# anenbergb/Co-DETR-TensorRT

Measured on AMD Instinct MI355X. Metric: images/sec, Co-DINO Swin-L 1920x1280 fp16 (p50 ms/image alongside), higher is better.
Workload: dtype f16

## Files before the change

co-detr-tensorrt_amd/codetr/_cabi.py:

```python
import ctypes
import os

import torch

_HERE = os.path.dirname(os.path.abspath(__file__))
LIB_PATH = os.path.join(_HERE, "libcodetr_hip.so")
ABI_VERSION = 53

_i64, _i32, _vp, _cp = ctypes.c_int64, ctypes.c_int, ctypes.c_void_p, ctypes.c_char_p

_MSDA_ARGS = [_vp, _vp, _vp, _vp, _vp, _vp, _i64, _i64, _i32, _i32, _i32, _i64, _i32, _i64, _vp]
SIGNATURES = {
    "codetr_hip_abi_version": (_i32, []),
    "codetr_hip_strerror": (_cp, [_i32]),
    "codetr_msda_forward_f16": (_i32, _MSDA_ARGS),
    "codetr_msda_forward_bf16": (_i32, _MSDA_ARGS),
    "codetr_msda_forward_f32": (_i32, _MSDA_ARGS),
    "codetr_msda_forward_f64": (_i32, _MSDA_ARGS),
    "codetr_msda_backward_f16": (_i32, [_vp, _vp, _vp, _vp, _vp, _vp, _vp, _i64, _i64, _i32, _i32, _i32, _i64, _i32, _i64,
                                        _vp, _vp, _vp]),
    "codetr_msda_backward_f32": (_i32, [_vp, _vp, _vp, _vp, _vp, _vp, _vp, _i64, _i64, _i32, _i32, _i32, _i64, _i32, _i64,
                                        _vp, _vp, _vp]),
    "codetr_msda_backward_f64": (_i32, [_vp, _vp, _vp, _vp, _vp, _vp, _vp, _i64, _i64, _i32, _i32, _i32, _i64, _i32, _i64,
                                        _vp, _vp, _vp]),
    "codetr_msda_variant": (_cp, [_i32, _i32, _i32, _i32, _i32]),
    "codetr_msda_fused_forward_f16": (_i32, [_vp, _vp, _vp, _vp, _vp, _i64, _vp, _i64, _vp, _i32, _i32, _i64, _i64,
                                             _i32, _i32, _i32, _i64, _i32, _vp]),
    "codetr_msda_fused_forward_bf16": (_i32, [_vp, _vp, _vp, _vp, _vp, _i64, _vp, _i64, _vp, _i32, _i32, _i64, _i64,
                                              _i32, _i32, _i32, _i64, _i32, _vp]),
    "codetr_msda_fused_forward_ref32_f16": (_i32, [_vp, _vp, _vp, _vp, _vp, _i64, _vp, _i64, _vp, _i32, _i32, _i64, _i64,
                                                   _i32, _i32, _i32, _i64, _i32, _vp]),
    "codetr_msda_fused_forward_ref32_bf16": (_i32, [_vp, _vp, _vp, _vp, _vp, _i64, _vp, _i64, _vp, _i32, _i32, _i64, _i64,
                                                    _i32, _i32, _i32, _i64, _i32, _vp]),
    "codetr_msda_encoder_forward_packed_f16": (_i32, [_vp, _vp, _vp, _vp, _i64, _vp, _i64, _i64, _i32, _i32, _i32, _i32,
                                                      _vp, _i32, _i32, _i32, _i32, _vp]),
    "codetr_msda_encoder_forward_packed_bf16": (_i32, [_vp, _vp, _vp, _vp, _i64, _vp, _i64, _i64, _i32, _i32, _i32, _i32,
                                                       _vp, _i32, _i32, _i32, _i32, _vp]),
    "codetr_linear_bf16_f16out": (_i32, [_vp, _vp, _vp, _vp, _vp, _vp, _i64, _i64, _i64, _i64, _i32]),
    "codetr_encoder_projections_f16": (_i32, [_vp, _vp, _vp, _vp, _vp, _vp, _vp, _vp, _i64, _i64, _i64, _i64, _i64, _i32]),
    "codetr_encoder_projections_bf16": (_i32, [_vp, _vp, _vp, _vp, _vp, _vp, _vp, _vp, _i64, _i64, _i64, _i64, _i64, _i32]),
    "codetr_encoder_projections_posgen_f16": (_i32, [_vp, _vp] + [_vp] * 10 + [_vp, _i32, _vp, ctypes.c_float, ctypes.c_float, ctypes.c_float,
                                                              ctypes.c_float, _i32, _vp, _vp, _vp, _vp, _vp, _i64, _i64, _i64, _i64, _i64, _i64, _i32]),
    "codetr_encoder_projections_posgen_bf16": (_i32, [_vp, _vp] + [_vp] * 10 + [_vp, _i32, _vp, ctypes.c_float, ctypes.c_float, ctypes.c_float,
                                                              ctypes.c_float, _i32, _vp, _vp, _vp, _vp, _vp, _i64, _i64, _i64, _i64, _i64, _i64, _i32]),
    "codetr_msda_encoder_packed_lds_bytes": (_i64, [_vp, _i32, _i32, _i32, _vp, _i32, _i32, _i32]),
    "codetr_msda_pack_projection_index": (_i32, [_i32, _i32, _i32, _vp]),
    "codetr_mx_scale_bytes": (_i64, [_i64, _i64]),
    "codetr_linear_fp8mx": (_i32, [_vp, _vp, _vp, _vp, _vp, _vp, _vp, _vp, _vp, _i64, _i64, _i64, _i32]),
    "codetr_cast_fp8mx_f16": (_i32, [_vp, _vp, _vp, _vp, _i64, _i64]),
    "codetr_layernorm_fp8mx_f16": (_i32, [_vp, _vp, _vp, _vp, _vp, _vp, _i64, _i64, ctypes.c_float]),
    "codetr_window_attention_fp8mx_f16": (_i32, [_vp, _vp, _vp, _vp, _vp, _vp, _i64, _i64, _i64, _i32, _i32, _i32, _i32]),
    "codetr_mha_attention_f16": (_i32, [_vp, _vp, _vp, _vp, _vp, _i64, _i64, _i64, _i32, _i32, _i64, _i64, _i64, _i64]),
    "codetr_mha_attention_bf16": (_i32, [_vp, _vp, _vp, _vp, _vp, _i64, _i64, _i64, _i32, _i32, _i64, _i64, _i64, _i64]),
    "codetr_linear_ln_f16": (_i32, [_vp, _vp, _vp, _vp, ctypes.c_float, _vp, _vp, _vp, _i64, _i64, _i64, _i32]),
    "codetr_linear_ln_bf16": (_i32, [_vp, _vp, _vp, _vp, ctypes.c_float, _vp, _vp, _vp, _i64, _i64, _i64, _i32]),
    "codetr_linear_xadd_f16": (_i32, [_vp, _vp, _vp, _vp, _vp, _vp, _i64, _i64, _i64]),
    "codetr_linear_xadd_bf16": (_i32, [_vp, _vp, _vp, _vp, _vp, _vp, _i64, _i64, _i64]),
    "codetr_im2col_tokens_b16": (_i32, [_vp, _vp, _i64, _i64, _i64, _i64, _i32, _i32, _i32, _vp]),
    "codetr_conv_tokens_f16": (_i32, [_vp, _vp, _vp, _vp, _vp, _vp, _i64, _i64, _i64, _i64, _i64, _i32, _i32, _i32, _i32]),
    "codetr_conv_tokens_bf16": (_i32, [_vp, _vp, _vp, _vp, _vp, _vp, _i64, _i64, _i64, _i64, _i64, _i32, _i32, _i32, _i32]),
# ... 11 lines not shown
    "codetr_sigmoid_f16": (_i32, [_vp, _vp, _vp, _i64]),
    "codetr_sigmoid_bf16": (_i32, [_vp, _vp, _vp, _i64]),
    "codetr_gather_rows_b16": (_i32, [_vp, _vp, _vp, _vp, _i64, _i64, _i64, _i64]),
    "codetr_decode_boxes_f16": (_i32, [_vp, _vp, _vp, _vp, _vp, _i64, _i64, _i64, _i32, ctypes.c_float, ctypes.c_float]),
    "codetr_decode_boxes_bf16": (_i32, [_vp, _vp, _vp, _vp, _vp, _i64, _i64, _i64, _i32, ctypes.c_float, ctypes.c_float]),
    "codetr_valid_ratios_f16": (_i32, [_vp, _vp, _vp, _vp, _vp, _i64, _i32]),
    "codetr_valid_ratios_bf16": (_i32, [_vp, _vp, _vp, _vp, _vp, _i64, _i32]),
    "codetr_linear_fp8": (_i32, [_vp, _vp, _vp, _vp, ctypes.c_float, _vp, _vp, _vp, _i32, ctypes.c_float, _i64, _i64, _i64,
                                 _i32]),
    "codetr_cast_fp8_f16": (_i32, [_vp, _vp, _vp, _i64, ctypes.c_float]),
    "codetr_layernorm_fp8_f16": (_i32, [_vp, _vp, _vp, _vp, _vp, _i64, _i64, ctypes.c_float, ctypes.c_float]),
    "codetr_linear_f16": (_i32, [_vp, _vp, _vp, _vp, _vp, _vp, _vp, _i64, _i64, _i64, _i32, _i64, _i32]),
    "codetr_linear_bf16": (_i32, [_vp, _vp, _vp, _vp, _vp, _vp, _vp, _i64, _i64, _i64, _i32, _i64, _i32]),
    "codetr_query_sine_embed_f16": (_i32, [_vp, _vp, _vp, _vp, _i64, _i64, _i32, _i32, _i32, ctypes.c_float, _i32, _vp, _vp,
                                           _vp]),
    "codetr_query_sine_embed_bf16": (_i32, [_vp, _vp, _vp, _vp, _i64, _i64, _i32, _i32, _i32, ctypes.c_float, _i32, _vp, _vp,
                                           _vp]),
    "codetr_encoder_geometry_f16": (_i32, [_vp, _vp, _vp, _i64, _i32, _vp, _vp, _vp, _vp, _vp]),
    "codetr_encoder_geometry_bf16": (_i32, [_vp, _vp, _vp, _i64, _i32, _vp, _vp, _vp, _vp, _vp]),
    "codetr_row_max_f16": (_i32, [_vp, _vp, _vp, _i64, _i64]),
    "codetr_row_max_bf16": (_i32, [_vp, _vp, _vp, _i64, _i64]),
    "codetr_preprocess_u8_f16": (_i32, [_vp, _vp, _i64, _i64, _i64, _i64, _i64, _i64, _vp, _vp, _vp, _vp, _vp]),
    "codetr_preprocess_u8_f32": (_i32, [_vp, _vp, _i64, _i64, _i64, _i64, _i64, _i64, _vp, _vp, _vp, _vp, _vp]),
    "codetr_batched_nms_f32": (_i32, [_vp, _vp, _vp, _i64, ctypes.c_float, _vp]),
    "codetr_preprocess_batch_u8_f16": (_i32, [_vp, _vp, _i64, _i64, _vp, _i64, _i64, _vp, _vp, _vp, ctypes.c_float, _vp, _vp]),
    "codetr_preprocess_batch_u8_bf16": (_i32, [_vp, _vp, _i64, _i64, _vp, _i64, _i64, _vp, _vp, _vp, ctypes.c_float, _vp, _vp]),
    "codetr_preprocess_batch_u8_f32": (_i32, [_vp, _vp, _i64, _i64, _vp, _i64, _i64, _vp, _vp, _vp, ctypes.c_float, _vp, _vp]),
    "codetr_postprocess_detections_f16": (_i32, [_vp, _vp, _vp, _vp, _vp, _i64, _i64, _i32, ctypes.c_float, _i32,
                                                 ctypes.c_float, _vp, _vp, _vp, _vp]),
    "codetr_postprocess_detections_bf16": (_i32, [_vp, _vp, _vp, _vp, _vp, _i64, _i64, _i32, ctypes.c_float, _i32,
                                                  ctypes.c_float, _vp, _vp, _vp, _vp]),
    "codetr_postprocess_detections_f32": (_i32, [_vp, _vp, _vp, _vp, _vp, _i64, _i64, _i32, ctypes.c_float, _i32,
                                                 ctypes.c_float, _vp, _vp, _vp, _vp]),
    "codetr_patch_merge_layernorm_f16": (_i32, [_vp, _vp, _vp, _vp, _vp, _i64, _i64, _i64, _i64, ctypes.c_float]),
    "codetr_patch_merge_layernorm_bf16": (_i32, [_vp, _vp, _vp, _vp, _vp, _i64, _i64, _i64, _i64, ctypes.c_float]),
    "codetr_mask_pyramid": (_i32, [_vp, _vp, _i64, _i64, _i64, _i32, _vp, _vp, _vp, _vp, _vp, _i32]),
    "codetr_linear_splitk_plan": (_i32, [_i64, _i64, _i64, _vp]),
    "codetr_linear_splitk_f16": (_i32, [_vp, _vp, _vp, _vp, _vp, _vp, _vp, _i64, _i64, _i64, _i32, _i32, _vp, _i64]),
    "codetr_linear_splitk_bf16": (_i32, [_vp, _vp, _vp, _vp, _vp, _vp, _vp, _i64, _i64, _i64, _i32, _i32, _vp, _i64]),
    "codetr_linear_sk_workspace_bytes": (_i64, []),
    "codetr_linear_sk_supported": (_i32, [_i64, _i64, _i64]),
    "codetr_linear_sk_preferred": (_i32, [_i64, _i64, _i64, _i32, _i32]),
    "codetr_linear_sk_f16": (_i32, [_vp, _vp, _vp, _vp, _vp, _vp, _i64, _i64, _i64, _i32, _vp, _i64, _i32]),
    "codetr_msda_op4_supported": (_i32, [_i32, _i64, _i64, _i32, _i32, _i32, _i64, _i32]),
    "codetr_msda_op4_forward_f16": (_i32, [_vp, _vp, _vp, _vp, _vp, _vp, _i64, _i64, _i32, _i32, _i32, _i64, _i32, _vp]),
    "codetr_msda_op4_forward_bf16": (_i32, [_vp, _vp, _vp, _vp, _vp, _vp, _i64, _i64, _i32, _i32, _i32, _i64, _i32, _vp]),
    "codetr_swin_mlp_supported": (_i32, [_i64, _i64, _i64]),
    "codetr_swin_mlp_f16": (_i32, [_vp, _vp, _vp, _vp, ctypes.c_float, _vp, _vp, _vp, _vp, _vp, _i64, _i64]),
    "codetr_swin_mlp_bf16": (_i32, [_vp, _vp, _vp, _vp, ctypes.c_float, _vp, _vp, _vp, _vp, _vp, _i64, _i64]),
    "codetr_linear_pp_supported": (_i32, [_i64, _i64, _i64]),
    "codetr_linear_pp_preferred": (_i32, [_i64, _i64, _i64, _i32, _i32]),
    "codetr_linear_pp_f16": (_i32, [_vp, _vp, _vp, _vp, _vp, _vp, _i64, _i64, _i64, _i32, _i32]),
    "codetr_linear_pp_bf16": (_i32, [_vp, _vp, _vp, _vp, _vp, _vp, _i64, _i64, _i64, _i32, _i32]),
    "codetr_linear_sk_bf16": (_i32, [_vp, _vp, _vp, _vp, _vp, _vp, _i64, _i64, _i64, _i32, _vp, _i64, _i32]),
    "codetr_decoder_layer_supported": (_i32, [_i32] * 7),
    "codetr_decoder_layer_blob_halfs": (_i64, [_i32] * 4),
    "codetr_decoder_layer_f16": (_i32, [_vp] * 18 + [_i64, _i64, _i64, _i32, _i32, _i32, ctypes.c_float, ctypes.c_float]),
    "codetr_decoder_layer_bf16": (_i32, [_vp] * 18 + [_i64, _i64, _i64, _i32, _i32, _i32, ctypes.c_float, ctypes.c_float]),
    "codetr_layernorm_f16": (_i32, [_vp, _vp, _vp, _vp, _vp, _i64, _i64, ctypes.c_float]),
    "codetr_layernorm_bf16": (_i32, [_vp, _vp, _vp, _vp, _vp, _i64, _i64, ctypes.c_float]),
    "codetr_groupnorm_tokens_workspace_bytes": (_i64, [_i64, _i64, _i64]),
    "codetr_groupnorm_tokens_f16": (_i32, [_vp, _vp, _vp, _vp, _vp, _i64, _vp, _i64, _i64, _i64, _i32,
                                           ctypes.c_float]),
    "codetr_groupnorm_tokens_bf16": (_i32, [_vp, _vp, _vp, _vp, _vp, _i64, _vp, _i64, _i64, _i64, _i32,
                                           ctypes.c_float]),
    "codetr_sine_pos_tokens_f16": (_i32, [_vp, _vp, _vp, _vp, _vp, _i64, _i64, _i64, _i64, _i32, ctypes.c_float,
                                          ctypes.c_float, ctypes.c_float, ctypes.c_float, _i32]),
    "codetr_sine_pos_tokens_bf16": (_i32, [_vp, _vp, _vp, _vp, _vp, _i64, _i64, _i64, _i64, _i32, ctypes.c_float,
                                          ctypes.c_float, ctypes.c_float, ctypes.c_float, _i32]),
    "codetr_ffn_relu_f16": (_i32, [_vp, _vp, _vp, _vp, _vp, _vp, _vp, _i64, _i64, _i64]),
    "codetr_ffn_relu_ln_f16": (_i32, [_vp, _vp, _vp, _vp, _vp, _vp, _vp, _i64, _i64, _i64, _vp, _vp, ctypes.c_float,
                                      _vp, _vp]),
    "codetr_ffn_relu_ln2_f16": (_i32, [_vp, _vp, _vp, _vp, _vp, _vp, _vp, _i64, _i64, _i64, _vp, _vp, ctypes.c_float,
                                       _vp, _vp, ctypes.c_float, _vp, _vp]),
    "codetr_ffn_relu_ln2_bf16": (_i32, [_vp, _vp, _vp, _vp, _vp, _vp, _vp, _i64, _i64, _i64, _vp, _vp, ctypes.c_float,
                                       _vp, _vp, ctypes.c_float, _vp, _vp]),
    "codetr_ffn_pack_w2_f16": (_i32, [_vp, _vp, _vp, _i64, _i64]),
    "codetr_ffn_oproj_relu_ln2_f16": (_i32, [_vp, _vp, _vp, _vp, _vp, _vp, _vp, _vp, _vp, _vp, _i64, _i64, _i64, _vp, _vp,
                                             ctypes.c_float, _vp, _vp, ctypes.c_float, _vp, _vp]),
    "codetr_ffn_oproj_relu_ln2_bf16": (_i32, [_vp, _vp, _vp, _vp, _vp, _vp, _vp, _vp, _vp, _vp, _i64, _i64, _i64, _vp, _vp,
                                              ctypes.c_float, _vp, _vp, ctypes.c_float, _vp, _vp]),
    "codetr_ffn_oproj_w1_index": (_i32, [_i64, _vp]),
    "codetr_ffn_fp8": (_i32, [_vp, _vp, _vp, _vp, _vp, _vp, _vp, _vp, _vp, _i64, _i64, _i64, ctypes.c_float, ctypes.c_float,
                              _vp, _vp, ctypes.c_float, _vp, _vp, ctypes.c_float, _vp, _vp]),
    "codetr_window_attention_f16": (_i32, [_vp, _vp, _vp, _vp, _vp, _i64, _i64, _i64, _i32, _i32, _i32, _i32]),
    "codetr_window_attention_bf16": (_i32, [_vp, _vp, _vp, _vp, _vp, _i64, _i64, _i64, _i32, _i32, _i32, _i32]),
    "codetr_window_attention_ex": (_i32, [_vp, _vp, _vp, _vp, _vp, _vp, ctypes.c_float, _i64, _i64, _i64, _i32, _i32, _i32, _i32,
                                          _i32, _i32, _i32]),
    "codetr_window_attention_bias_index": (_i32, [_i32, _vp]),
    "codetr_window_attention_fp8out_f16": (_i32, [_vp, _vp, _vp, _vp, _vp, ctypes.c_float, _i64, _i64, _i64, _i32, _i32,
                                                  _i32, _i32]),
}

_lib = None

CALLS = {"encoder_projections_posgen": 0, "msda": 0, "msda_fused": 0, "linear": 0, "layernorm": 0, "window_attention": 0, "groupnorm_tokens": 0,
         "sine_pos_tokens": 0, "ffn_fused": 0, "ffn_oproj_fused": 0, "linear_splitk": 0, "linear_sk": 0, "mask_pyramid": 0,
         "query_sine_embed": 0, "encoder_geometry": 0, "row_max": 0, "preprocess": 0, "batched_nms": 0,
         "preprocess_batch": 0, "postprocess_detections": 0,
         "msda_backward": 0, "patch_merge_layernorm": 0, "msda_encoder": 0, "msda_encoder_packed": 0, "patch_im2col": 0, "mha_attention": 0, "topk": 0,
         "linear_pp": 0, "swin_mlp": 0, "linear_tile128": 0, "linear_tile256": 0, "linear_xs": 0, "linear_ln": 0, "linear_xadd": 0, "encoder_projections": 0,
         "linear_fp8": 0, "cast_fp8": 0, "layernorm_fp8": 0, "small_ops": 0, "ffn_fp8": 0, "decoder_layer": 0,
         "conv_tokens": 0, "conv_im2col_nchw": 0, "maxpool_tokens": 0}


RECORDER = None
_QUERIES = {"codetr_hip_abi_version", "codetr_hip_strerror", "codetr_msda_variant", "codetr_linear_variant",
            "codetr_topk_chunks", "codetr_linear_splitk_plan", "codetr_groupnorm_tokens_workspace_bytes",
            "codetr_linear_sk_workspace_bytes", "codetr_linear_sk_supported", "codetr_linear_sk_preferred",
            "codetr_linear_pp_supported", "codetr_linear_pp_preferred", "codetr_msda_op4_supported", "codetr_swin_mlp_supported",
            "codetr_msda_encoder_packed_lds_bytes", "codetr_msda_pack_projection_index", "codetr_window_attention_bias_index",
            "codetr_mx_scale_bytes", "codetr_decoder_layer_supported",
            "codetr_decoder_layer_blob_halfs"}


class _RecordingLib:
    def __init__(self, lib):
        self._lib = lib

    def __getattr__(self, name):
        fn = getattr(self._lib, name)
        if name in _QUERIES or name not in SIGNATURES:
            return fn

        def launch(*args):
            rc = fn(*args)
            if RECORDER is not None and rc == 0:
                RECORDER.append((name, args))
            return rc

        return launch


_rec_lib = None


def load():
    global _lib, _rec_lib
    if _lib is not None:
        if RECORDER is None:
            return _lib
        if _rec_lib is None:
            _rec_lib = _RecordingLib(_lib)
        return _rec_lib
    if not os.path.isfile(LIB_PATH):
        raise ImportError(
            f"HIP extension not found at {LIB_PATH}; build it with "
            "`python -c 'import __graft_entry__ as g; g.build()'` or `make -C co-detr-tensorrt_amd/csrc`"
        )
    lib = ctypes.CDLL(LIB_PATH)
    for name, (res, args) in SIGNATURES.items():
        try:
            fn = getattr(lib, name)
        except AttributeError as e:
# ... 98 lines not shown
        v = _SK_PREFERRED[key] = bool(load().codetr_linear_sk_preferred(M, N, K, _ACT[act], 1 if has_residual else 0))
    return v


_SK_WORKSPACE = {}


def linear_sk_workspace(device):
    key = (device.index, torch.cuda.current_stream(device).cuda_stream)
    ws = _SK_WORKSPACE.get(key)
    if ws is None:
        with torch.cuda.device(device):
            ws = _SK_WORKSPACE[key] = torch.zeros(load().codetr_linear_sk_workspace_bytes(), dtype=torch.uint8, device=device)
    return ws


def linear_sk(x2d, weight, bias, residual2d, act, out2d, flags=0):
    lib = load()
    CALLS["linear"] += 1
    CALLS["linear_sk"] += 1
    M, K = x2d.shape
    N = weight.shape[0]
    ws = linear_sk_workspace(x2d.device) if flags & 0x40 else None
    fn = lib.codetr_linear_sk_f16 if x2d.dtype == torch.float16 else lib.codetr_linear_sk_bf16
    rc = fn(current_stream_ptr(x2d.device), x2d.data_ptr(), weight.data_ptr(),
            bias.data_ptr() if bias is not None else None,
            residual2d.data_ptr() if residual2d is not None else None, out2d.data_ptr(), M, N, K, _ACT[act],
            ws.data_ptr() if ws is not None else None, ws.numel() if ws is not None else 0, flags)
    check(rc, "codetr_linear_sk")
    return out2d


def swin_mlp(x2d, ln_w, ln_b, eps, w1, b1, w2_packed, b2, out2d):
    CALLS["swin_mlp"] += 1
    lib = load()
    fn = lib.codetr_swin_mlp_bf16 if x2d.dtype == torch.bfloat16 else lib.codetr_swin_mlp_f16
    rc = fn(current_stream_ptr(x2d.device), x2d.data_ptr(), ln_w.data_ptr(), ln_b.data_ptr(), float(eps), w1.data_ptr(),
            b1.data_ptr(), w2_packed.data_ptr(), b2.data_ptr(), out2d.data_ptr(), x2d.shape[0], x2d.shape[1])
    check(rc, "codetr_swin_mlp")
    return out2d


_PP_PREFERRED = {}


def linear_pp_preferred(M, N, K, act=None, has_residual=False) -> bool:
    key = (M, N, K, act, bool(has_residual))
    v = _PP_PREFERRED.get(key)
    if v is None:
        v = _PP_PREFERRED[key] = bool(load().codetr_linear_pp_preferred(M, N, K, _ACT[act], 1 if has_residual else 0))
    return v


def linear_pp(x2d, weight, bias, residual2d, act, out2d, flags=0):
    lib = load()
    CALLS["linear"] += 1
    CALLS["linear_pp"] += 1
    M, K = x2d.shape
    N = weight.shape[0]
    fn = lib.codetr_linear_pp_f16 if x2d.dtype == torch.float16 else lib.codetr_linear_pp_bf16
    rc = fn(current_stream_ptr(x2d.device), x2d.data_ptr(), weight.data_ptr(),
            bias.data_ptr() if bias is not None else None,
            residual2d.data_ptr() if residual2d is not None else None, out2d.data_ptr(), M, N, K, _ACT[act], flags)
    check(rc, "codetr_linear_pp")
    return out2d


def query_sine_embed(ref, valid_ratios, pos_feat, temperature=10000.0, apply_sigmoid=True, valid_ratios32=None):
    CALLS["query_sine_embed"] += 1
    B, Nq, d = ref.shape
    L = valid_ratios.shape[1]
    ref_in = torch.empty((B, Nq, L, d), dtype=ref.dtype, device=ref.device)
    ref_in32 = torch.empty((B, Nq, L, d), dtype=torch.float32, device=ref.device) if valid_ratios32 is not None else None
    embed = torch.empty((B, Nq, d * pos_feat), dtype=ref.dtype, device=ref.device)
    fn = load().codetr_query_sine_embed_bf16 if ref.dtype == torch.bfloat16 else load().codetr_query_sine_embed_f16
    rc = fn(current_stream_ptr(ref.device), ref.data_ptr(), valid_ratios.data_ptr(),
                                            valid_ratios32.data_ptr() if valid_ratios32 is not None else None, B, Nq,
                                            d, L, pos_feat, float(temperature), 1 if apply_sigmoid else 0,
                                            ref_in.data_ptr(), ref_in32.data_ptr() if ref_in32 is not None else None,
                                            embed.data_ptr())
    check(rc, "codetr_query_sine_embed_f16")
    return ref_in, embed, ref_in32


_MSDA_BWD = {torch.float16: "codetr_msda_backward_f16", torch.float32: "codetr_msda_backward_f32",
             torch.float64: "codetr_msda_backward_f64"}


def msda_backward(value, spatial_shapes, level_start_index, sampling_loc, attn_weight, grad_output, grad_value,
                  grad_sampling_loc, grad_attn_weight, im2col_step):
    if value.dtype not in _MSDA_BWD:
        raise RuntimeError(f"multi_scale_deformable_attention_backward: unsupported dtype {value.dtype} (f16 / f32 / f64)")
    CALLS["msda_backward"] += 1
    B, S, M, D = value.shape
    Nq, L, P = sampling_loc.shape[1], sampling_loc.shape[3], sampling_loc.shape[4]
    rc = getattr(load(), _MSDA_BWD[value.dtype])(
        current_stream_ptr(value.device), value.data_ptr(), spatial_shapes.data_ptr(), level_start_index.data_ptr(),
        sampling_loc.data_ptr(), attn_weight.data_ptr(), grad_output.data_ptr(), B, S, M, D, L, Nq, P, int(im2col_step),
        grad_value.data_ptr(), grad_sampling_loc.data_ptr(), grad_attn_weight.data_ptr())
    if rc == -2:
        step = min(B, int(im2col_step))
        raise RuntimeError(f"batch({B}) must divide im2col_step({step})")
    check(rc, "codetr_msda_backward")


def encoder_geometry(valid_ratios, mask_flat, shapes):
    CALLS["encoder_geometry"] += 1
    B, S = mask_flat.shape
    L = len(shapes)
    dev = mask_flat.device
    dt = valid_ratios.dtype
    ref = torch.empty((B, S, 2), dtype=dt, device=dev)
    ref_lvl = torch.empty((B, S, L, 2), dtype=dt, device=dev)
    prop = torch.empty((B, S, 4), dtype=dt, device=dev)
    state = torch.empty((B, S), dtype=torch.uint8, device=dev)
    hw = (ctypes.c_int64 * (2 * L))(*[int(v) for s in shapes for v in s])
    fn = load().codetr_encoder_geometry_bf16 if valid_ratios.dtype == torch.bfloat16 else load().codetr_encoder_geometry_f16
# ... 703 lines not shown
```

co-detr-tensorrt_amd/codetr/_kernel_names.py:

```python
KERNEL_NAMES = (
    "add_kernel",
    "batched_nms_kernel",
    "cast_fp8_kernel",
    "cast_fp8mx_kernel",
    "conv_im2col_nchw_kernel",
    "conv_tokens_kernel",
    "decode_boxes_kernel",
    "decoder_layer_kernel",
    "encoder_geometry_kernel",
    "ffn_fp8_kernel",
    "ffn_fused_kernel",
    "gather_rows_kernel",
    "gn_apply_kernel",
    "gn_finalize_kernel",
    "gn_partial_kernel",
    "im2col_tokens_kernel",
    "layernorm_fp8_kernel",
    "layernorm_fp8mx_kernel",
    "layernorm_kernel",
    "level_cums_kernel",
    "level_mask_kernel",
    "linear_256_fp8_kernel",
    "linear_256_kernel",
    "linear_kernel",
    "linear_pp_kernel",
    "linear_sk_kernel",
    "linear_xs_kernel",
    "maxpool_tokens_kernel",
    "mha_attention_kernel",
    "msda_backward_generic_kernel",
    "msda_backward_kernel",
    "msda_encoder_v4_kernel",
    "msda_fused_headmajor_kernel",
    "msda_op4_kernel",
    "msda_scalar_kernel",
    "msda_tiled_kernel",
    "pack_w2_kernel",
    "patch_im2col_k4_kernel",
    "postprocess_kernel",
    "preprocess_batch_kernel",
    "preprocess_kernel",
    "query_sine_embed_kernel",
    "row_max_kernel",
    "sigmoid_kernel",
    "sine_pos_kernel",
    "splitk_reduce_kernel",
    "swin_mlp_kernel",
    "topk_kernel",
    "topk_reg_kernel",
    "valid_ratios_kernel",
    "window_attention_kernel",
)
```

co-detr-tensorrt_amd/codetr/hip_ops.py:

```python

import collections

import torch
import torch.nn.functional as F

from . import _cabi

NATIVE = {"msda", "linear(f16/bf16, K%64==0)", "layer_norm(f16/bf16)", "swin_window_attention(f16, head_dim 32)",
          "msda_fused(softmax + sampling locations in-kernel)", "groupnorm_tokens(f16, 8 ch/group)",
          "sine_pos_tokens(f16, + level_embed)", "ffn_fused(f16, 256 -> hidden -> 256, ReLU, + identity)",
          "mask_pyramid(level masks + running valid counts + valid ratios)",
          "query_sine_embed(f16: sigmoid x valid ratios + sine embedding of the decoder reference boxes)",
          "encoder_geometry(f16: reference points, proposals, keep/drop state)", "row_max(f16)",
          "preprocess_image(u8 -> f16/f32, cv2-exact resize + pad + normalise + mask)", "batched_nms(f32)",
          "preprocess_batch(u8 -> f16/bf16/f32, <= 32 images of any size per launch, stacked + padded)",
          "postprocess_detections(f16/bf16/f32: threshold + sort + per-class NMS + rescale, one workgroup per image)",
          "patch_merge_layernorm(f16: Swin 2x2 gather + LayerNorm)",
          "msda_encoder_packed(f16/bf16: LDS-staged gather for the encoder's self-attention, csrc/msda_encoder4.hip)",
          "patch_embed(f16/bf16: 4x4 patch gather + GEMM)",
          "mha_attention(f16/bf16: dense softmax attention, head_dim 32, <= 1024 keys)",
          "topk(f16/bf16 rows, k <= 1024: radix select + bitonic sort)",
          "im2col_tokens(16-bit token-major maps)",
          "resnet50(f16/bf16: implicit-GEMM conv_tokens, stem window gather + GEMM, maxpool_tokens, BN folded)",
          "small_ops(f16: add, sigmoid, gather_rows, decode_boxes, valid_ratios)",
          "linear_fp8(e4m3 x e4m3, K%128==0) + layer_norm_fp8 + cast_fp8", "ffn_fp8(fused FFN, both products e4m3)"}


LINEAR_PROFILE = None
KERNEL_PROFILE = None


def _timed(name, meta, launch, device):
    if KERNEL_PROFILE is None:
        return launch()
    st = torch.cuda.current_stream(device)
    e0, e1 = torch.cuda.Event(enable_timing=True), torch.cuda.Event(enable_timing=True)
    e0.record(st)
    r = launch()
    e1.record(st)
    KERNEL_PROFILE.setdefault(name, []).append((e0, e1, meta))
    return r


def _gpu(x, what):
    if not x.is_cuda:
        raise RuntimeError(
            f"codetr.hip_ops.{what}: got a {x.device.type} tensor; this package computes on MI355X only "
            "(the CPU formulation is the oracle in oracle/, not a fallback)"
        )


LINEAR_PP = True


def _persistent_ok(mk, head_major, out, x2, w, r2, bias):
    return (mk is None and not head_major and out.data_ptr() % 16 == 0 and x2.data_ptr() % 16 == 0
            and w.data_ptr() % 16 == 0 and (r2 is None or r2.data_ptr() % 16 == 0)
            and (bias is None or bias.data_ptr() % 16 == 0))


def linear(x, weight, bias=None, act=None, residual=None, row_mask=None, head_major=None):
    _gpu(x, "linear")
    if _cabi.linear_supported(x, weight):
        K = x.shape[-1]
        N = weight.shape[0]
        x2 = x.reshape(-1, K)
        if not x2.is_contiguous():
            x2 = x2.contiguous()
        w = weight if weight.is_contiguous() else weight.contiguous()
        r2 = None
        if residual is not None:
            r2 = residual.reshape(-1, N)
            if not r2.is_contiguous():
                r2 = r2.contiguous()
        mk = None
        if row_mask is not None:
            mk = row_mask.reshape(-1)
            if mk.dtype != torch.bool and mk.dtype != torch.uint8:
                mk = mk != 0
            mk = mk.contiguous()
        hm_rows = hm_hd = 0
        if head_major:
            if x.dim() != 3 or residual is not None:
                raise ValueError("head_major needs a [B, S, K] input and no residual")
            hm_rows, hm_hd = x.shape[1], int(head_major)
        out = torch.empty((x2.shape[0], N), dtype=x.dtype, device=x.device)
        if x2.shape[0] > 0:
            with torch.cuda.device(x.device):
                res_act = act == "relu_res"
                splits, ws_bytes = (1, 0) if (head_major or res_act) else _cabi.linear_splitk_plan(x2.shape[0], N, K)
                if res_act:
                    launch = lambda: _cabi.linear(x2, w, bias, r2, act, out, mk, hm_rows, hm_hd)
                elif splits > 1:
                    ws = torch.empty(ws_bytes, dtype=torch.uint8, device=x.device)
                    launch = lambda: _cabi.linear_splitk(x2, w, bias, r2, act, out, splits, ws, mk)
                elif (LINEAR_PP and _persistent_ok(mk, head_major, out, x2, w, r2, bias)
                      and _cabi.linear_pp_preferred(x2.shape[0], N, K, act, r2 is not None)):
                    launch = lambda: _cabi.linear_pp(x2, w, bias, r2, act, out)
                elif (_persistent_ok(mk, head_major, out, x2, w, r2, bias)
                      and _cabi.linear_sk_preferred(x2.shape[0], N, K, act, r2 is not None)):
                    launch = lambda: _cabi.linear_sk(x2, w, bias, r2, act, out)
                else:
                    launch = lambda: _cabi.linear(x2, w, bias, r2, act, out, mk, hm_rows, hm_hd)
                if LINEAR_PROFILE is None:
                    launch()
                else:
                    st = torch.cuda.current_stream(x.device)
                    e0, e1 = torch.cuda.Event(enable_timing=True), torch.cuda.Event(enable_timing=True)
                    e0.record(st)
                    launch()
                    e1.record(st)
                    LINEAR_PROFILE.append((e0, e1, 2.0 * x2.shape[0] * N * K, x2.shape[0], N, K))
        if head_major:
            return out.view(x.shape[0], N // hm_hd, hm_rows, hm_hd)
        return out.view(*x.shape[:-1], N)
    if head_major:
        raise RuntimeError("head_major output exists only on the native linear (f16/bf16, K % 64 == 0)")
    y = F.linear(x, weight, bias)
    if act == "relu_res":
        if row_mask is not None:
            y = y.masked_fill(row_mask[..., None], 0.0)
        return F.relu(y + residual if residual is not None else y)
    if act == "relu":
        y = F.relu(y, inplace=True)
    elif act == "gelu":
        y = F.gelu(y)
    elif act is not None:
        raise ValueError(act)
    if row_mask is not None:
        y = y.masked_fill(row_mask[..., None], 0.0)
    if residual is not None:
        y = y + residual
    return y


LN_GEMM = True


def linear_ln_supported(x, norm_weight, weight):
    return (LN_GEMM and x.is_cuda and norm_weight is not None and norm_weight.dtype == x.dtype and weight.dtype == x.dtype
            and not torch.is_grad_enabled() and norm_weight.shape[0] == x.shape[-1]
            and _cabi.linear_xadd_supported(x.numel() // max(x.shape[-1], 1), weight.shape[0], x.shape[-1], x.dtype))


def linear_ln(x, norm_weight, norm_bias, eps, weight, bias=None, act=None):
    _gpu(x, "linear_ln")
    if linear_ln_supported(x, norm_weight, weight):
        K, N = x.shape[-1], weight.shape[0]
        x2 = x.reshape(-1, K)
        x2 = x2 if x2.is_contiguous() else x2.contiguous()
        w = weight if weight.is_contiguous() else weight.contiguous()
        out = torch.empty((x2.shape[0], N), dtype=x.dtype, device=x.device)
        ok = [False]

        def launch():
            ok[0] = _cabi.linear_ln(x2, norm_weight, norm_bias, eps, w, bias, act, out)

        with torch.cuda.device(x.device):
            if LINEAR_PROFILE is None:
                launch()
            else:
                st = torch.cuda.current_stream(x.device)
                e0, e1 = torch.cuda.Event(enable_timing=True), torch.cuda.Event(enable_timing=True)
                e0.record(st)
                launch()
                e1.record(st)
                if ok[0]:
                    LINEAR_PROFILE.append((e0, e1, 2.0 * x2.shape[0] * N * K, x2.shape[0], N, K))
        if ok[0]:
            return out.view(*x.shape[:-1], N)
    return linear(layer_norm(x, norm_weight, norm_bias, eps), weight, bias, act=act)


XADD = True
XADD_MIN_ROWS = 0


def linear_xadd_supported(x, x_add, weight):
    return (XADD and x.is_cuda and x_add is not None and x_add.shape == x.shape and x_add.dtype == x.dtype
            and weight.dtype == x.dtype and not torch.is_grad_enabled()
            and x.numel() // max(x.shape[-1], 1) >= XADD_MIN_ROWS
            and _cabi.linear_xadd_supported(x.numel() // max(x.shape[-1], 1), weight.shape[0], x.shape[-1], x.dtype))


def linear_xadd(x, x_add, weight, bias=None):
    _gpu(x, "linear_xadd")
    if linear_xadd_supported(x, x_add, weight):
        K, N = x.shape[-1], weight.shape[0]
        x2, a2 = x.reshape(-1, K), x_add.reshape(-1, K)
        x2 = x2 if x2.is_contiguous() else x2.contiguous()
        a2 = a2 if a2.is_contiguous() else a2.contiguous()
        w = weight if weight.is_contiguous() else weight.contiguous()
        out = torch.empty((x2.shape[0], N), dtype=x.dtype, device=x.device)
        ok = [False]

        def launch():
            ok[0] = _cabi.linear_xadd(x2, a2, w, bias, out)

        with torch.cuda.device(x.device):
# ... 480 lines not shown
        return linear(cols, weight_kkc, bias, act=act, residual=r).view(B, Ho, Wo, Cout)
    x4d = x4d if x4d.is_contiguous() else x4d.contiguous()
    if residual is not None and not residual.is_contiguous():
        residual = residual.contiguous()
    out = torch.empty((B, Ho, Wo, Cout), dtype=x4d.dtype, device=x4d.device)
    with torch.cuda.device(x4d.device):
        _timed("conv_tokens", {"M": B * Ho * Wo, "N": Cout, "K": k * k * C},
               lambda: _cabi.conv_tokens(x4d, weight_kkc, bias, residual, k, stride, pad, act, out), x4d.device)
    return out


def stem_conv_tokens(x, weight_pad, bias, k, stride, pad):
    _gpu(x, "stem_conv_tokens")
    B, C, H, W = x.shape
    Cout, kpad = weight_pad.shape
    Ho, Wo = (H + 2 * pad - k) // stride + 1, (W + 2 * pad - k) // stride + 1
    cols = torch.empty((B * Ho * Wo, kpad), dtype=x.dtype, device=x.device)
    with torch.cuda.device(x.device):
        _cabi.conv_im2col_nchw(x if x.is_contiguous() else x.contiguous(), k, stride, pad, kpad, cols)
    return linear(cols, weight_pad, bias, act="relu").view(B, Ho, Wo, Cout)


def maxpool_tokens(x4d):
    _gpu(x4d, "maxpool_tokens")
    B, H, W, C = x4d.shape
    out = torch.empty((B, (H - 1) // 2 + 1, (W - 1) // 2 + 1, C), dtype=x4d.dtype, device=x4d.device)
    with torch.cuda.device(x4d.device):
        _cabi.maxpool_tokens(x4d if x4d.is_contiguous() else x4d.contiguous(), out)
    return out




def topk(x, k, want_values=True):
    _gpu(x, "topk")
    x2 = x.reshape(-1, x.shape[-1])
    if not torch.is_grad_enabled():
        x2 = x2 if x2.is_contiguous() else x2.contiguous()
        if _cabi.topk_supported(x2, k):
            idx = torch.empty((x2.shape[0], k), dtype=torch.int64, device=x.device)
            val = torch.empty((x2.shape[0], k), dtype=x.dtype, device=x.device) if want_values else None
            with torch.cuda.device(x.device):
                _cabi.topk(x2, k, val, idx)
            shape = (*x.shape[:-1], k)
            return (val.view(shape) if val is not None else None), idx.view(shape)
    v, i = torch.topk(x, k, dim=-1)
    return v, i


MSDA_ENCODER = True
MSDA_FP32_REF = True


_SWITCH_DEFAULTS = {"ENC_POSGEN": True, "WINDOW_BIAS_LANE": True, "LINEAR_PP": True, "SWIN_MLP": True, "SWIN_MLP_MIN_ROWS": 32768, "LN_GEMM": True, "XADD": True, "XADD_MIN_ROWS": 0, "MERGE_LN": True, "MSDA_ENCODER": True,
                    "MSDA_FP32_REF": True, "FP8_MIN_TILES": 96,
                    "R50_NATIVE": True, "R50_CONV_IM2COL": False}


def nondefault_switches():
    import sys

    from . import multi_scale_deformable_attention as msda_mod
    from . import transformer as tr_mod

    me = sys.modules[__name__]
    out = [k for k, v in _SWITCH_DEFAULTS.items() if getattr(me, k) != v]
    if msda_mod.HEAD_MAJOR_VALUE:
        out.append("HEAD_MAJOR_VALUE")
    out += [k for k in ("DEC_FUSED", "DEC_VPROJ") if not getattr(tr_mod, k)]
    return sorted(out)


MSDA_V4 = True
MSDA_V4_THREADS = 512
MSDA_V4_REGION = (16, 16)
MSDA_V4_LDS_BUDGET = 64 * 1024
MSDA_V4_MARGIN_CAP = 40.0
MSDA_V4_HEAD_MAJOR = True
ENC_PROJ_FUSED = True
_SWITCH_DEFAULTS.update({"MSDA_V4": True, "MSDA_V4_THREADS": 512, "MSDA_V4_REGION": (16, 16),
                         "MSDA_V4_LDS_BUDGET": 64 * 1024, "MSDA_V4_MARGIN_CAP": 40.0,
                         "MSDA_V4_HEAD_MAJOR": True, "ENC_PROJ_FUSED": True, "FFN_OPROJ": True})


def msda_encoder_packed_supported(dtype, head_dim, num_levels, num_points):
    return (MSDA_V4 and MSDA_ENCODER and dtype in (torch.float16, torch.bfloat16) and head_dim == 32 and num_levels == 5
            and num_points == 4)


def value_projection_f16(x, weight, bias, row_mask, head_dim):
    _gpu(x, "value_projection_f16")
    if not (x.dtype == torch.bfloat16 and weight.dtype == torch.bfloat16 and x.dim() == 3):
        return None
    B, S, K = x.shape
    N = weight.shape[0]
    x2 = x.reshape(-1, K)
    x2 = x2 if x2.is_contiguous() else x2.contiguous()
    w = weight if weight.is_contiguous() else weight.contiguous()
    mk = None
    if row_mask is not None:
        mk = row_mask.reshape(-1)
        if mk.dtype != torch.bool and mk.dtype != torch.uint8:
            mk = mk != 0
        mk = mk.contiguous()
    out = torch.empty((B * S, N), dtype=torch.float16, device=x.device)
    with torch.cuda.device(x.device):
        ok = _cabi.linear_bf16_f16out(x2, w, bias, out, mk, S, int(head_dim))
# ... 366 lines not shown
```

co-detr-tensorrt_amd/codetr/swin.py:

```python
import warnings
from collections import OrderedDict

import torch
import torch.nn as nn
import torch.nn.functional as F

from . import hip_ops
from .transformer_layers import FFN, build_norm


def to_2tuple(x):
    return tuple(x) if isinstance(x, (tuple, list)) else (x, x)


class PatchEmbed(nn.Module):

    def __init__(self, in_channels=3, embed_dims=768, conv_type="Conv2d", kernel_size=16, stride=16, padding="corner",
                 dilation=1, bias=True, norm_cfg=None, input_size=None, init_cfg=None):
        super().__init__()
        if padding != "corner" or dilation != 1:
            raise NotImplementedError("PatchEmbed: only 'corner' padding, dilation 1 (what Swin uses)")
        self.embed_dims = embed_dims
        self.kernel_size, self.stride = to_2tuple(kernel_size), to_2tuple(stride or kernel_size)
        self.projection = nn.Conv2d(in_channels, embed_dims, self.kernel_size, self.stride, bias=bias)
        self.norm = build_norm(norm_cfg, embed_dims) if norm_cfg is not None else None

    def forward(self, x):
        H, W = x.shape[-2:]
        kh, kw = self.kernel_size
        sh, sw = self.stride
        if hip_ops.patch_embed_supported(x, self.projection.weight, self.stride):
            x, hw = hip_ops.patch_embed(x, self.projection.weight, self.projection.bias)
            if self.norm is not None:
                x = hip_ops.layer_norm(x, self.norm.weight, self.norm.bias, self.norm.eps)
            return x, hw
        ph = max((-(-H // sh) - 1) * sh + kh - H, 0)
        pw = max((-(-W // sw) - 1) * sw + kw - W, 0)
        if ph or pw:
            x = F.pad(x, (0, pw, 0, ph))
        x = hip_ops.conv2d(x, self.projection.weight, self.projection.bias, stride=self.stride)
        hw = (x.shape[2], x.shape[3])
        x = x.flatten(2).transpose(1, 2)
        if self.norm is not None:
            x = hip_ops.layer_norm(x, self.norm.weight, self.norm.bias, self.norm.eps)
        return x, hw


class PatchMerging(nn.Module):

    def __init__(self, in_channels, out_channels, kernel_size=2, stride=None, padding="corner", dilation=1, bias=False,
                 norm_cfg=dict(type="LN"), init_cfg=None):
        super().__init__()
        if to_2tuple(kernel_size) != (2, 2) or to_2tuple(stride or kernel_size) != (2, 2) or padding != "corner":
            raise NotImplementedError("PatchMerging: only the 2x2 / stride-2 / corner-padded form Swin uses")
        self.in_channels, self.out_channels = in_channels, out_channels
        self.norm = build_norm(norm_cfg, 4 * in_channels) if norm_cfg is not None else None
        self.reduction = nn.Linear(4 * in_channels, out_channels, bias=bias)

    def forward(self, x, input_size):
        B, L, C = x.shape
        H, W = input_size
        if L != H * W:
            raise AssertionError("input feature has wrong size")
        x = x.view(B, H, W, C)
        if H % 2 or W % 2:
            x = F.pad(x, (0, 0, 0, W % 2, 0, H % 2))
        H2, W2 = (H + 1) // 2, (W + 1) // 2
        if x.is_cuda and not torch.is_grad_enabled():
            nw, nb, rw = self._permuted_params(C)
            if (self.norm is not None and isinstance(self.norm, nn.LayerNorm)
                    and hip_ops.patch_merge_layernorm_supported(x, C)):
                x = hip_ops.patch_merge_layernorm(x.reshape(B, -1, C), (2 * H2, 2 * W2), nw, nb, self.norm.eps)
                return hip_ops.linear(x, rw, self.reduction.bias), (H2, W2)
            x = x.view(B, H2, 2, W2, 2, C).permute(0, 1, 3, 2, 4, 5).reshape(B, H2 * W2, 4 * C)
            if self.norm is not None:
                x = hip_ops.layer_norm(x, nw, nb, self.norm.eps)
            return hip_ops.linear(x, rw, self.reduction.bias), (H2, W2)
        x = x.view(B, H2, 2, W2, 2, C).permute(0, 1, 3, 5, 2, 4).reshape(B, H2 * W2, 4 * C)
        if self.norm is not None:
            x = hip_ops.layer_norm(x, self.norm.weight, self.norm.bias, self.norm.eps)
        return hip_ops.linear(x, self.reduction.weight, self.reduction.bias), (H2, W2)

    def _permuted_params(self, C):
        ps = [self.reduction.weight] + ([self.norm.weight, self.norm.bias] if self.norm is not None else [])

        def build():
            idx = (torch.arange(C, device=ps[0].device)[None, :] * 4 + torch.arange(4, device=ps[0].device)[:, None]).reshape(-1)
            rw = self.reduction.weight.detach()[:, idx].contiguous()
            nw = self.norm.weight.detach()[idx].contiguous() if self.norm is not None else None
            nb = self.norm.bias.detach()[idx].contiguous() if self.norm is not None else None
            return nw, nb, rw

        return hip_ops.derived(ps, "_codetr_perm", build)


class WindowMSA(nn.Module):
    def __init__(self, embed_dims, num_heads, window_size, qkv_bias=True, qk_scale=None, attn_drop_rate=0.0,
                 proj_drop_rate=0.0, init_cfg=None):
        super().__init__()
        self.embed_dims, self.window_size, self.num_heads = embed_dims, to_2tuple(window_size), num_heads
        head_dim = embed_dims // num_heads
        if qk_scale is not None and qk_scale != head_dim ** -0.5:
            raise NotImplementedError("custom qk_scale")
        self.scale = head_dim ** -0.5
        Wh, Ww = self.window_size
        self.relative_position_bias_table = nn.Parameter(torch.zeros((2 * Wh - 1) * (2 * Ww - 1), num_heads))
        coords = torch.stack(torch.meshgrid(torch.arange(Wh), torch.arange(Ww), indexing="ij")).flatten(1)
        rel = coords[:, :, None] - coords[:, None, :]
        index = (rel[0] + Wh - 1) * (2 * Ww - 1) + (rel[1] + Ww - 1)
        self.register_buffer("relative_position_index", index.contiguous())
        self.qkv = nn.Linear(embed_dims, embed_dims * 3, bias=qkv_bias)
        self.proj = nn.Linear(embed_dims, embed_dims)

    def init_weights(self):
        nn.init.trunc_normal_(self.relative_position_bias_table, std=0.02)

    def relative_position_bias(self):
        t = self.relative_position_bias_table
        N = self.window_size[0] * self.window_size[1]
        return hip_ops.derived((t,), "_codetr_rel_bias", lambda: t[self.relative_position_index.view(-1)].view(N, N, -1)
                               .permute(2, 0, 1).contiguous().detach())

    def forward(self, x, mask=None):
        qkv = hip_ops.linear(x, self.qkv.weight, self.qkv.bias)
        o = hip_ops.window_attention(qkv, self.relative_position_bias(), mask, self.num_heads)
        return hip_ops.linear(o, self.proj.weight, self.proj.bias)


_MASK_CACHE = {}


def shifted_window_mask(Hp, Wp, ws, shift, dtype, device):
    key = (Hp, Wp, ws, shift, dtype, str(device))
    m = _MASK_CACHE.get(key)
    if m is None:
        region = torch.zeros(Hp, Wp, dtype=torch.float32)
        cnt = 0
        for hs in (slice(0, -ws), slice(-ws, -shift), slice(-shift, None)):
            for wsl in (slice(0, -ws), slice(-ws, -shift), slice(-shift, None)):
                region[hs, wsl] = cnt
                cnt += 1
        r = region.view(Hp // ws, ws, Wp // ws, ws).permute(0, 2, 1, 3).reshape(-1, ws * ws)
        diff = r[:, None, :] - r[:, :, None]
        m = torch.where(diff != 0, torch.tensor(-100.0), torch.tensor(0.0)).to(device=device, dtype=dtype)
        _MASK_CACHE[key] = m
    return m


class ShiftWindowMSA(nn.Module):
    def __init__(self, embed_dims, num_heads, window_size, shift_size=0, qkv_bias=True, qk_scale=None,
                 attn_drop_rate=0, proj_drop_rate=0, dropout_layer=dict(type="DropPath", drop_prob=0.0), init_cfg=None):
        super().__init__()
        self.window_size, self.shift_size = window_size, shift_size
        if not 0 <= shift_size < window_size:
            raise AssertionError("shift_size must be in [0, window_size)")
        self.w_msa = WindowMSA(embed_dims, num_heads, to_2tuple(window_size), qkv_bias, qk_scale, attn_drop_rate,
                               proj_drop_rate)

    def takes_norm(self, query, hw_shape):
        return hip_ops.swin_window_attention_supported(query, self.w_msa.embed_dims, self.w_msa.num_heads, self.window_size)

    def forward(self, query, hw_shape, identity=None, pre_norm=None):
        B, L, C = query.shape
        H, W = hw_shape
        if L != H * W:
            raise AssertionError("input feature has wrong size")
        ws, sh = self.window_size, self.shift_size
        m = self.w_msa
        if hip_ops.swin_window_attention_supported(query, C, m.num_heads, ws):
            if pre_norm is not None:
                qkv = hip_ops.linear_ln(query, pre_norm[0], pre_norm[1], pre_norm[2], m.qkv.weight, m.qkv.bias)
            else:
                qkv = hip_ops.linear(query, m.qkv.weight, m.qkv.bias)
            o = hip_ops.swin_window_attention(qkv, m.qkv.bias, m.relative_position_bias(), hw_shape, m.num_heads, ws, sh)
            return hip_ops.linear(o, m.proj.weight, m.proj.bias, residual=identity)
        x = query.view(B, H, W, C)
        pad_r, pad_b = (-W) % ws, (-H) % ws
        if pad_r or pad_b:
            x = F.pad(x, (0, 0, 0, pad_r, 0, pad_b))
        Hp, Wp = H + pad_b, W + pad_r
        mask = None
        if sh > 0:
            x = torch.roll(x, shifts=(-sh, -sh), dims=(1, 2))
            mask = shifted_window_mask(Hp, Wp, ws, sh, query.dtype, query.device)
        win = x.view(B, Hp // ws, ws, Wp // ws, ws, C).permute(0, 1, 3, 2, 4, 5).reshape(-1, ws * ws, C)
        win = self.w_msa(win, mask)
        x = win.view(B, Hp // ws, Wp // ws, ws, ws, C).permute(0, 1, 3, 2, 4, 5).reshape(B, Hp, Wp, C)
        if sh > 0:
            x = torch.roll(x, shifts=(sh, sh), dims=(1, 2))
        if pad_r or pad_b:
            x = x[:, :H, :W, :]
        x = x.reshape(B, H * W, C)
        return x if identity is None else x + identity


class SwinBlock(nn.Module):
    def __init__(self, embed_dims, num_heads, feedforward_channels, window_size=7, shift=False, qkv_bias=True,
                 qk_scale=None, drop_rate=0.0, attn_drop_rate=0.0, drop_path_rate=0.0, act_cfg=dict(type="GELU"),
                 norm_cfg=dict(type="LN"), with_cp=False, init_cfg=None):
        super().__init__()
        self.norm1 = build_norm(norm_cfg, embed_dims)
        self.attn = ShiftWindowMSA(embed_dims, num_heads, window_size, window_size // 2 if shift else 0, qkv_bias,
                                   qk_scale, attn_drop_rate, drop_rate)
        self.norm2 = build_norm(norm_cfg, embed_dims)
        self.ffn = FFN(embed_dims=embed_dims, feedforward_channels=feedforward_channels, num_fcs=2, ffn_drop=drop_rate,
                       act_cfg=act_cfg, add_identity=True)

    def forward(self, x, hw_shape):
        n1, n2 = self.norm1, self.norm2
        mode = getattr(self, "fp8_mode", None)
        if mode is not None and x.is_cuda and x.dtype == torch.float16 and self.attn.takes_norm(x, hw_shape):
            rows = x.shape[0] * x.shape[1]
            if mode == "calibrate":
                return self._forward_fp8_calibrate(x, hw_shape)
            if mode == "run" and all(hip_ops.linear_fp8_supported(rows, w) for w in self._fp8_weights()):
                return self._forward_fp8(x, hw_shape)
            if mode == "mx":
                ops = getattr(self, "fp8_ops", None) or ("qkv", "proj", "fc1", "fc2")
                ws = dict(zip(("qkv", "proj", "fc1", "fc2"), self._fp8_weights()))
                if ops and all(hip_ops.linear_fp8_supported(rows, ws[o]) for o in ops):
                    return self._forward_fp8mx(x, hw_shape)
        if (isinstance(n1, nn.LayerNorm) and self.attn.takes_norm(x, hw_shape)
                and hip_ops.linear_ln_supported(x, n1.weight, self.attn.w_msa.qkv.weight)):
            x = self.attn(x, hw_shape, identity=x, pre_norm=(n1.weight, n1.bias, n1.eps))
        else:
            h = hip_ops.layer_norm(x, n1.weight, n1.bias, n1.eps)
            x = self.attn(h, hw_shape, identity=x)
        fc1, fc2 = self.ffn.layers[0][0], self.ffn.layers[1]
        if (isinstance(n2, nn.LayerNorm) and self.ffn.add_identity and fc1.bias is not None and fc2.bias is not None
                and hip_ops.swin_mlp_supported(x, n2.weight, fc1.weight, fc2.weight, self.ffn.act)):
            return hip_ops.swin_mlp(x, n2.weight, n2.bias, n2.eps, fc1.weight, fc1.bias, fc2.weight, fc2.bias)
        if (isinstance(n2, nn.LayerNorm) and self.ffn.add_identity
                and hip_ops.linear_ln_supported(x, n2.weight, fc1.weight)):
            h = hip_ops.linear_ln(x, n2.weight, n2.bias, n2.eps, fc1.weight, fc1.bias, act=self.ffn.act)
            return hip_ops.linear(h, fc2.weight, fc2.bias, residual=x)
        h = hip_ops.layer_norm(x, n2.weight, n2.bias, n2.eps)
        return self.ffn(h, identity=x)


    def _fp8_weights(self):
        m = self.attn.w_msa
        return (m.qkv.weight, m.proj.weight, self.ffn.layers[0][0].weight, self.ffn.layers[1].weight)

    def _forward_fp8_calibrate(self, x, hw_shape):
        n1, n2, m = self.norm1, self.norm2, self.attn.w_msa
        fc1, fc2 = self.ffn.layers[0][0], self.ffn.layers[1]
        amax = self.__dict__.setdefault("_fp8_amax", {})

        def rec(key, t):
            v = t.detach().abs().amax().float()
            amax[key] = v if key not in amax else torch.maximum(amax[key], v)

        h = hip_ops.layer_norm(x, n1.weight, n1.bias, n1.eps)
        rec("ln1", h)
        qkv = hip_ops.linear(h, m.qkv.weight, m.qkv.bias)
        o = hip_ops.swin_window_attention(qkv, m.qkv.bias, m.relative_position_bias(), hw_shape, m.num_heads,
                                          self.attn.window_size, self.attn.shift_size)
        rec("attn", o)
        x = hip_ops.linear(o, m.proj.weight, m.proj.bias, residual=x)
        h = hip_ops.layer_norm(x, n2.weight, n2.bias, n2.eps)
        rec("ln2", h)
        g = hip_ops.linear(h, fc1.weight, fc1.bias, act=self.ffn.act)
        rec("act", g)
        return hip_ops.linear(g, fc2.weight, fc2.bias, residual=x)

    def _forward_fp8(self, x, hw_shape):
        n1, n2, m = self.norm1, self.norm2, self.attn.w_msa
        fc1, fc2 = self.ffn.layers[0][0], self.ffn.layers[1]
        sc = self._fp8_scales
        h8 = hip_ops.layer_norm_fp8(x, n1.weight, n1.bias, n1.eps, sc["ln1"])
        qkv = hip_ops.linear_fp8(h8, sc["ln1"], m.qkv.weight, m.qkv.bias)
        o8 = hip_ops.swin_window_attention(qkv, m.qkv.bias, m.relative_position_bias(), hw_shape, m.num_heads,
                                           self.attn.window_size, self.attn.shift_size, out_scale=sc["attn"])
        x = hip_ops.linear_fp8(o8, sc["attn"], m.proj.weight, m.proj.bias, residual=x)
        h8 = hip_ops.layer_norm_fp8(x, n2.weight, n2.bias, n2.eps, sc["ln2"])
        g8 = hip_ops.linear_fp8(h8, sc["ln2"], fc1.weight, fc1.bias, act=self.ffn.act, out_scale=sc["act"])
        return hip_ops.linear_fp8(g8, sc["act"], fc2.weight, fc2.bias, residual=x)


    def _forward_fp8mx(self, x, hw_shape):
        n1, n2, m = self.norm1, self.norm2, self.attn.w_msa
        fc1, fc2 = self.ffn.layers[0][0], self.ffn.layers[1]
        ops = getattr(self, "fp8_ops", None) or ("qkv", "proj", "fc1", "fc2")
        if "qkv" in ops:
            h8, hs = hip_ops.layer_norm_fp8mx(x, n1.weight, n1.bias, n1.eps)
            qkv = hip_ops.linear_fp8mx(h8, hs, m.qkv.weight, m.qkv.bias)
        elif hip_ops.linear_ln_supported(x, n1.weight, m.qkv.weight):
            qkv = hip_ops.linear_ln(x, n1.weight, n1.bias, n1.eps, m.qkv.weight, m.qkv.bias)
# ... 172 lines not shown
```

co-detr-tensorrt_amd/csrc/gemm_pp.hip:

```cpp
#include <hip/hip_runtime.h>
#include <stdint.h>

#include <type_traits>

#include "codetr_hip.h"
#include "device_prims.h"

namespace {

#ifndef CODETR_PP_ABL
#define CODETR_PP_ABL 0
#endif
constexpr int kAbl = CODETR_PP_ABL;
#ifdef CODETR_PP_STAMPS
__device__ unsigned long long* g_pp_stamps = nullptr;
#define PP_T(i) const unsigned long long pp_t##i = __builtin_readcyclecounter()
#define PP_ACC(k, a, b) pp_acc[k] += pp_t##b - pp_t##a
#define PP_STAMPS_OUT()                                                                    \
  if (lane == 0 && g_pp_stamps) {                                                          \
    pp_acc[7] = __builtin_readcyclecounter() - pp_k0;                                      \
    unsigned long long* o = g_pp_stamps + ((size_t)blockIdx.x * 8 + wave) * 8;             \
    for (int i = 0; i < 8; ++i) o[i] = pp_acc[i];                                          \
  }
#else
#define PP_T(i)
#define PP_ACC(k, a, b)
#define PP_STAMPS_OUT()
#endif
typedef unsigned u32x2v __attribute__((__vector_size__(2 * sizeof(unsigned))));

constexpr int kSlot = 32768;
constexpr int kOpBytes = 16384;
constexpr int kBiasBytes = 32768;

struct PpArgs {
  const unsigned char* X;
  const unsigned char* W;
  const unsigned short* bias;
  const unsigned short* R;
  unsigned short* Y;
  int M, N, K;
  int tiles_n, T, nk;
  int G;
  int rounds;
  int rem;
};

__device__ __forceinline__ int key64(int row) {
  const int q = (row >> 2) & 3;
  return q ^ ((q & 1) << 1);
}

__device__ __forceinline__ void seg_barrier() {
  __builtin_amdgcn_sched_barrier(0);
  __builtin_amdgcn_s_barrier();
  __builtin_amdgcn_sched_barrier(0);
}

__device__ __forceinline__ int item_tile(const PpArgs& a, int w, int idx) {
  const int D = a.rounds * a.G;
  if (w < a.rem) {
    if (idx == 0) return D + w;
    --idx;
  }
  if (idx >= a.rounds) return -1;
  return (w & 7) * (D >> 3) + idx * (a.G >> 3) + (w >> 3);
}

template <class T, int ACT, bool HAS_BIAS, bool HAS_RES, bool BIAS_LDS = true>
__device__ __forceinline__ bool pp_epilogue(f32x4 (&acc)[4][8], const PpArgs& a, int tile, int grp, int wn, int lane,
                                            const unsigned char* bias_lds) {
  const int fa = lane & 15;
  const int tm = tile / a.tiles_n, tn = tile - tm * a.tiles_n;
  const int m0 = tm * 256 + grp * 128, n0 = tn * 256 + wn * 64;
  const int g = lane >> 4, nl = 4 * fa;
  const int mleft = a.M - m0, nleft = a.N - n0;
  const unsigned rowb = (unsigned)a.N * 2u;
  const unsigned span = (mleft > 0 && nleft > 0) ? (unsigned)(mleft < 128 ? mleft : 128) * rowb : 0u;
  const unsigned voff = nl < nleft ? (unsigned)(4 * g) * rowb + (unsigned)nl * 2u : 0x80000000u;
  const int mrem = mleft - 4 * g;
  const __amdgpu_buffer_rsrc_t rres = __builtin_amdgcn_make_buffer_rsrc(
      const_cast<unsigned char*>(reinterpret_cast<const unsigned char*>(a.R)) + ((size_t)m0 * a.N + n0) * 2, 0,
      HAS_RES ? span : 0u, 0x00020000);
  uint2 rr[8][4];
  auto load_res = [&](int j0, int j1) {
#pragma unroll
    for (int j = j0; j < j1; ++j)
#pragma unroll
      for (int r = 0; r < 4; ++r) {
        const u32x2v t2 = __builtin_amdgcn_raw_buffer_load_b64(rres, j * 16 + r < mrem ? voff : 0x80000000u,
                                                                 (unsigned)(j * 16 + r) * rowb, 0);
        rr[j][r] = uint2{t2[0], t2[1]};
      }
  };
  const bool stored = a.M > m0 && a.N > n0;
  if (stored) {
    float bias4[4] = {0.f, 0.f, 0.f, 0.f};
    if (HAS_BIAS) {
      const int nb = n0 + nl < a.N ? n0 + nl : 0;
      const uint2 b2 = BIAS_LDS ? *reinterpret_cast<const uint2*>(bias_lds + nb * 2)
                                : *reinterpret_cast<const uint2*>(a.bias + nb);
      bias4[0] = T::to_f32((unsigned short)(b2.x & 0xffffu));
      bias4[1] = T::to_f32((unsigned short)(b2.x >> 16));
      bias4[2] = T::to_f32((unsigned short)(b2.y & 0xffffu));
      bias4[3] = T::to_f32((unsigned short)(b2.y >> 16));
    }
    const __amdgpu_buffer_rsrc_t ry = __builtin_amdgcn_make_buffer_rsrc(
        reinterpret_cast<unsigned char*>(a.Y) + ((size_t)m0 * a.N + n0) * 2, 0, span, 0x00020000);
    if (HAS_RES) load_res(0, 4);
#pragma unroll
    for (int j = 0; j < 8; ++j) {
      if (HAS_RES && j == 2) load_res(4, 8);
#pragma unroll
      for (int r = 0; r < 4; ++r) {
        float x[4];
#pragma unroll
        for (int i = 0; i < 4; ++i) x[i] = acc[i][j][r] + bias4[i];
        if (ACT == 1) {
#pragma unroll
          for (int i = 0; i < 4; ++i) x[i] = x[i] < 0.f ? 0.f : x[i];
        }
        if (ACT == 2) {
          const f32x2 g01 = gelu_erf2(f32x2{x[0], x[1]}), g23 = gelu_erf2(f32x2{x[2], x[3]});
          x[0] = g01.x; x[1] = g01.y; x[2] = g23.x; x[3] = g23.y;
        }
        uint2 o = {T::pack2(x[0], x[1]), T::pack2(x[2], x[3])};
        if (HAS_RES) {
          const uint2 q = rr[j][r];
          const float y0 = T::to_f32((unsigned short)(o.x & 0xffffu)) + T::to_f32((unsigned short)(q.x & 0xffffu));
          const float y1 = T::to_f32((unsigned short)(o.x >> 16)) + T::to_f32((unsigned short)(q.x >> 16));
          const float y2 = T::to_f32((unsigned short)(o.y & 0xffffu)) + T::to_f32((unsigned short)(q.y & 0xffffu));
          const float y3 = T::to_f32((unsigned short)(o.y >> 16)) + T::to_f32((unsigned short)(q.y >> 16));
          o = uint2{T::pack2(y0, y1), T::pack2(y2, y3)};
        }
        if (!(kAbl & 16))
          __builtin_amdgcn_raw_buffer_store_b64(u32x2v{o.x, o.y}, ry, j * 16 + r < mrem ? voff : 0x80000000u,
                                                (unsigned)(j * 16 + r) * rowb, 0);
      }
    }
  }
  return stored;
}

template <class T, int ACT, bool HAS_BIAS, bool HAS_RES, int NS, int PH>
__global__ __launch_bounds__(512) __attribute__((amdgpu_waves_per_eu(2, 2))) void linear_pp_kernel(const PpArgs a) {
  __shared__ __attribute__((aligned(16))) unsigned char lds[NS * kSlot + (HAS_BIAS ? kBiasBytes : 0)];
  using frag = typename T::frag;
  constexpr int PP = 4;
  constexpr int VMN = PP * (NS - 2);

  const int tid = threadIdx.x, lane = tid & 63;
  const int wave = __builtin_amdgcn_readfirstlane(tid >> 6);
  const int grp = wave >> 2, wn = wave & 3;
  const int wg = blockIdx.x;
  const int K = a.K, K2 = K * 2;
  const int nh = 2 * a.nk;
  const unsigned lds0 = (unsigned)(uintptr_t)((__attribute__((address_space(3))) unsigned char*)lds);

#ifdef CODETR_PP_STAMPS
  unsigned long long pp_acc[8] = {0, 0, 0, 0, 0, 0, 0, 0};
  const unsigned long long pp_k0 = __builtin_readcyclecounter();
#endif
  int c_idx = 0;
  int c_tile = item_tile(a, wg, 0);
  if (c_tile < 0) return;

  unsigned voffW[2], voffX[2];
  const unsigned char* Wp = a.W;
  const unsigned char* Xp = a.X;
  int p_idx = 0, p_tile = c_tile, p_h = 0;
  auto prod_set_tile = [&]() {
    const int tm = p_tile / a.tiles_n, tn = p_tile - tm * a.tiles_n;
    const int m0 = tm * 256, n0 = tn * 256;
    const int nmax = a.N - 1 - n0, mmax = a.M - 1 - m0;
    int ln = lane;
    asm volatile("" : "+v"(ln));
#pragma unroll
    for (int q = 0; q < 2; ++q) {
      const int r = (wave + 8 * q) * 16 + (ln >> 2);
      const int rw = (r & 192) + 4 * (r & 15) + ((r >> 4) & 3);
      const unsigned co = (unsigned)((((ln & 3) ^ key64(r)) * 16));
      const int rn = rw < nmax ? rw : nmax, rm = r < mmax ? r : mmax;
      voffW[q] = (unsigned)rn * (unsigned)K2 + co;
      voffX[q] = (unsigned)rm * (unsigned)K2 + co;
    }
    Wp = a.W + (size_t)n0 * K * 2;
    Xp = a.X + (size_t)m0 * K * 2;
    p_h = 0;
  };
  prod_set_tile();
  auto produce_piece = [&](int g, int slot) {
    const unsigned dst = lds0 + (unsigned)slot * kSlot + (unsigned)wave * 1024u;
    if (g < 2) lds_dma16(Wp, voffW[g], dst + (unsigned)g * 8192u);
    else lds_dma16(Xp, voffX[g - 2], dst + kOpBytes + (unsigned)(g - 2) * 8192u);
  };
  auto produce_advance = [&]() {
    if (p_tile < 0) return;
    ++p_h;
    if (p_h < nh) {
      Wp += 64;
      Xp += 64;
      return;
    }
    p_tile = item_tile(a, wg, ++p_idx);
    if (p_tile >= 0) prod_set_tile();
  };

  const int fa = lane & 15, fc = lane >> 4;
  const unsigned offA = (unsigned)((wn * 64 + fa) * 64 + ((fc ^ key64(fa)) * 16));
  const unsigned offB = (unsigned)(kOpBytes + (grp * 128 + fa) * 64 + ((fc ^ key64(fa)) * 16));

  f32x4 acc[4][8];
  frag fw[4], fx[8];

  if (HAS_BIAS) {
    for (int i = tid; i * 8 < a.N; i += 512)
      *reinterpret_cast<u32x4*>(lds + NS * kSlot + i * 16) = *reinterpret_cast<const u32x4*>(a.bias + i * 8);
  }
#pragma unroll
  for (int s = 0; s < NS - 1; ++s) {
#pragma unroll
    for (int g = 0; g < PP; ++g) produce_piece(g, s);
    produce_advance();
  }
  wait_vmcnt<VMN>();
  asm volatile("s_waitcnt lgkmcnt(0)" ::: "memory");
  seg_barrier();
  int post = 0;
  int ws = 0;

  auto load_seg = [&](int part) {
    PP_T(0);
    const unsigned char* rbase = lds + ws * kSlot;
    const int fs = ws == 0 ? NS - 1 : ws - 1;
    if (!(kAbl & 4)) {
      if (part == 0) {
#pragma unroll
        for (int i = 0; i < 4; ++i) fw[i] = *reinterpret_cast<const frag*>(rbase + offA + i * 1024);
      }
#pragma unroll
      for (int j = 0; j < 8; ++j)
        if (PH == 1 || (j >> 2) == part) fx[j] = *reinterpret_cast<const frag*>(rbase + offB + j * 1024);
    }
    if (!(kAbl & 1)) {
#pragma unroll
      for (int g = 0; g < PP; ++g)
        if (PH == 1 || (g >> 1) == part) produce_piece(g, fs);
    }
    if (part == PH - 1) produce_advance();
    PP_T(1);
    if (part == PH - 1) {
      if (post > 0) {
        wait_vmcnt<VMN + 32>();
        --post;
      } else {
        wait_vmcnt<VMN>();
      }
    }
    PP_T(2);
    asm volatile("s_waitcnt lgkmcnt(0)" ::: "memory");
    PP_T(3);
    seg_barrier();
    PP_T(4);
    PP_ACC(0, 0, 1); PP_ACC(1, 1, 2); PP_ACC(2, 2, 3); PP_ACC(3, 3, 4);
  };
  auto mfma_seg = [&](int part, bool firstk) {
    PP_T(5);
    __builtin_amdgcn_s_setprio(1);
#pragma unroll
    for (int i = 0; i < 4; ++i)
#pragma unroll
      for (int j = 0; j < 8; ++j) {
        if (PH == 2 && (j >> 2) != part) continue;
        if (kAbl & 2) asm volatile("" ::"v"(fw[i]), "v"(fx[j]));
        else if (firstk) acc[i][j] = T::mfma(fx[j], fw[i], f32x4{0.f, 0.f, 0.f, 0.f});
        else acc[i][j] = T::mfma(fx[j], fw[i], acc[i][j]);
      }
    __builtin_amdgcn_s_setprio(0);
    PP_T(6);
    seg_barrier();
    PP_T(7);
    PP_ACC(4, 5, 6); PP_ACC(5, 6, 7);
  };

  while (c_tile >= 0) {
    if (grp == 1) seg_barrier();
#pragma unroll
    for (int part = 0; part < PH; ++part) {
      load_seg(part);
      mfma_seg(part, true);
    }
    ws = ws + 1 == NS ? 0 : ws + 1;
    for (int h = 1; h < nh; ++h) {
#pragma unroll
      for (int part = 0; part < PH; ++part) {
        load_seg(part);
        mfma_seg(part, false);
      }
      ws = ws + 1 == NS ? 0 : ws + 1;
    }
    if (grp == 0) seg_barrier();

    PP_T(8);
    const bool stored = pp_epilogue<T, ACT, HAS_BIAS, HAS_RES>(acc, a, c_tile, grp, wn, lane, lds + NS * kSlot);
    PP_T(9);
    PP_ACC(6, 8, 9);
    post = stored && !(kAbl & 16) ? NS - 2 : 0;
    c_tile = item_tile(a, wg, ++c_idx);
  }
  wait_vmcnt<0>();
  PP_STAMPS_OUT();
}

int device_cus() {
  static int cus[64] = {0};
  int dev = 0;
  if (hipGetDevice(&dev) != hipSuccess || dev < 0 || dev >= 64) return 256;
  if (cus[dev] == 0) {
    int n = 0;
    if (hipDeviceGetAttribute(&n, hipDeviceAttributeMultiprocessorCount, dev) != hipSuccess || n <= 0) n = 256;
    cus[dev] = n;
  }
  return cus[dev];
}

bool pp_supported(int64_t M, int64_t N, int64_t K) {
  return M > 0 && N > 0 && K >= 128 && K % 64 == 0 && N % 8 == 0 && M <= 0x7fffffffLL && N <= 16384 &&
         255 * K * 2 + 64 < 0x7fffffffLL;
}

template <class T, int ACT>
int launch_pp_act(hipStream_t st, const PpArgs& a, bool has_bias, bool has_res) {
  const dim3 grid((unsigned)a.G), block(512);
#define CODETR_PP(HB, HR) hipLaunchKernelGGL((linear_pp_kernel<T, ACT, HB, HR, 4, 1>), grid, block, 0, st, a)
  if (has_bias && has_res) CODETR_PP(true, true);
  else if (has_bias) CODETR_PP(true, false);
  else if (has_res) CODETR_PP(false, true);
  else CODETR_PP(false, false);
#undef CODETR_PP
  const hipError_t err = hipGetLastError();
  return err == hipSuccess ? 0 : (int)err;
}

template <class T>
int launch_pp(hipStream_t st, const void* X, const void* W, const void* bias, const void* R, void* Y, int64_t M, int64_t N,
              int64_t K, int act, int flags) {
  if (!X || !W || !Y || M <= 0 || N <= 0 || K <= 0) return CODETR_E_BADARG;
  if (act < 0 || act > 2 || !pp_supported(M, N, K)) return CODETR_E_UNSUPPORTED;
  if ((reinterpret_cast<uintptr_t>(X) | reinterpret_cast<uintptr_t>(W) | reinterpret_cast<uintptr_t>(Y) |
       reinterpret_cast<uintptr_t>(R) | reinterpret_cast<uintptr_t>(bias)) & 15)
    return CODETR_E_BADARG;
  const int64_t tiles_m = (M + 255) / 256, tiles_n = (N + 255) / 256, T_ = tiles_m * tiles_n;
  if (T_ > 0x3fffffff) return CODETR_E_TOO_LARGE;
  int G = device_cus() / 8 * 8;
  if (G <= 0) return CODETR_E_BADARG;
  PpArgs a;
  a.X = static_cast<const unsigned char*>(X);
  a.W = static_cast<const unsigned char*>(W);
  a.bias = static_cast<const unsigned short*>(bias);
  a.R = static_cast<const unsigned short*>(R);
  a.Y = static_cast<unsigned short*>(Y);
  a.M = (int)M; a.N = (int)N; a.K = (int)K;
  a.tiles_n = (int)tiles_n; a.T = (int)T_; a.nk = (int)(K / 64);
  a.G = G;
  a.rounds = (int)(T_ / G);
  a.rem = (int)(T_ - (int64_t)a.rounds * G);
  const bool hb = bias != nullptr, hr = R != nullptr;
  if ((int64_t)256 * K * 2 > 0x7fffffffLL) return CODETR_E_TOO_LARGE;
  if (flags != 0) return CODETR_E_UNSUPPORTED;
  switch (act) {
    case 0: return launch_pp_act<T, 0>(st, a, hb, hr);
    case 1: return launch_pp_act<T, 1>(st, a, hb, hr);
    default: return launch_pp_act<T, 2>(st, a, hb, hr);
  }
}

}

extern "C" {

int codetr_linear_pp_supported(int64_t M, int64_t N, int64_t K) { return pp_supported(M, N, K) ? 1 : 0; }

int codetr_linear_pp_preferred(int64_t M, int64_t N, int64_t K, int act, int has_residual) {
  (void)act;
  (void)has_residual;
  if (!pp_supported(M, N, K) || K < 768 || N < 384) return 0;
  const int64_t tn = (N + 255) / 256, tiles = ((M + 255) / 256) * tn;
  return tiles >= 200 && N * 8 >= tn * 256 * 7 ? 1 : 0;
}

int codetr_linear_pp_f16(void* stream, const void* x_dev, const void* w_dev, const void* bias_dev, const void* residual_dev,
                         void* y_dev, int64_t M, int64_t N, int64_t K, int act, int flags) {
  return launch_pp<HalfT>(static_cast<hipStream_t>(stream), x_dev, w_dev, bias_dev, residual_dev, y_dev, M, N, K, act, flags);
}

int codetr_linear_pp_bf16(void* stream, const void* x_dev, const void* w_dev, const void* bias_dev, const void* residual_dev,
                          void* y_dev, int64_t M, int64_t N, int64_t K, int act, int flags) {
#if CODETR_PP_ABL
  return CODETR_E_UNSUPPORTED;
#endif
  return launch_pp<BFloatT>(static_cast<hipStream_t>(stream), x_dev, w_dev, bias_dev, residual_dev, y_dev, M, N, K, act, flags);
}

}
```

co-detr-tensorrt_amd/csrc/layernorm.hip:

```cpp
#include <hip/hip_runtime.h>
#include <stdint.h>

#include "codetr_hip.h"
#include "device_prims.h"

namespace {

constexpr int kThreads = 256;

struct LnHalf {
  __device__ static float up(short b) {
    _Float16 h;
    __builtin_memcpy(&h, &b, 2);
    return (float)h;
  }
  __device__ static short down(float v) {
    _Float16 h = (_Float16)v;
    short b;
    __builtin_memcpy(&b, &h, 2);
    return b;
  }
};
struct LnBf16 {
  __device__ static float up(short b) { return bf16_to_f32((unsigned short)b); }
// ... 37 lines not shown
    int mb = 0, my = 0, mx = 0;
    if (MERGE) {
      mb = (int)(row / ((int64_t)mg.H2 * mg.W2));
      const int rr = (int)(row - (int64_t)mb * mg.H2 * mg.W2);
      my = rr / mg.W2;
      mx = rr - my * mg.W2;
    }
    s16x8 v[NCH];
    float s = 0.f;
#pragma unroll
    for (int c = 0; c < NCH; ++c) {
      const int ch = sub + c * G;
      if (ch < nchunks) {
        if (MERGE) {
          const int cpc = mg.Cs >> 3, k = ch / cpc, within = ch - k * cpc;
          const int sy = 2 * my + (k >> 1), sx = 2 * mx + (k & 1);
          v[c] = s16x8{0, 0, 0, 0, 0, 0, 0, 0};
          if (sy < mg.H && sx < mg.W)
            v[c] = *reinterpret_cast<const s16x8*>(x + (((int64_t)mb * mg.H + sy) * mg.W + sx) * mg.Cs + within * 8);
        } else {
          v[c] = *reinterpret_cast<const s16x8*>(xr + ch * 8);
        }
#pragma unroll
        for (int e = 0; e < 8; ++e) s += T::up(v[c][e]);
      }
    }
    const float mean = group_sum<G>(s) * inv_c;
    float q = 0.f;
#pragma unroll
    for (int c = 0; c < NCH; ++c) {
      const int ch = sub + c * G;
      if (ch < nchunks) {
#pragma unroll
        for (int e = 0; e < 8; ++e) {
          const float d = T::up(v[c][e]) - mean;
          q = fmaf(d, d, q);
        }
      }
    }
    const float rstd = rsqrtf(group_sum<G>(q) * inv_c + eps);
    short* yr = y + row * C;
#pragma unroll
    for (int c = 0; c < NCH; ++c) {
      const int ch = sub + c * G;
      if (ch < nchunks) {
        s16x8 o;
#pragma unroll
        for (int e = 0; e < 8; ++e)
          o[e] = T::down(fmaf((T::up(v[c][e]) - mean) * rstd, T::up(gw[c][e]), T::up(gb[c][e])));
        *reinterpret_cast<s16x8*>(yr + ch * 8) = o;
      }
    }
  }
}

template <class T, int G, int NCH, bool MERGE = false>
int launch_cfg(hipStream_t st, const void* x, const void* g, const void* b, void* y, int64_t rows, int C, float eps,
               MergeGeom mg = MergeGeom{}) {
  constexpr int RPB = kThreads / G;
  int64_t blocks = (rows + RPB - 1) / RPB;
  if (blocks > 256 * 16) blocks = 256 * 16;
  hipLaunchKernelGGL((layernorm_kernel<T, G, NCH, MERGE>), dim3((unsigned)blocks), dim3(kThreads), 0, st,
                     static_cast<const short*>(x), static_cast<const short*>(g), static_cast<const short*>(b),
                     static_cast<short*>(y), rows, C, eps, mg);
  const hipError_t err = hipGetLastError();
  return err == hipSuccess ? 0 : (int)err;
}

template <class T>
int launch_merge(hipStream_t st, const void* x, const void* g, const void* b, void* y, int64_t B, int64_t H, int64_t W,
                 int64_t Cs, float eps) {
  if (!x || !g || !b || !y || B <= 0 || H <= 0 || W <= 0 || Cs <= 0) return CODETR_E_BADARG;
  const int64_t C = 4 * Cs;
  if (Cs % 8 != 0 || C > 4096) return CODETR_E_UNSUPPORTED;
  if (H > 0x7fffffffLL || W > 0x7fffffffLL) return CODETR_E_TOO_LARGE;
  MergeGeom mg{(int)H, (int)W, (int)Cs, (int)((H + 1) / 2), (int)((W + 1) / 2)};
  const int64_t rows = B * mg.H2 * mg.W2;
  const int nch = (int)(C / 8);
  if (nch <= 32) return launch_cfg<T, 32, 1, true>(st, x, g, b, y, rows, (int)C, eps, mg);
  if (nch <= 64) return launch_cfg<T, 64, 1, true>(st, x, g, b, y, rows, (int)C, eps, mg);
  if (nch <= 128) return launch_cfg<T, 64, 2, true>(st, x, g, b, y, rows, (int)C, eps, mg);
  if (nch <= 192) return launch_cfg<T, 64, 3, true>(st, x, g, b, y, rows, (int)C, eps, mg);
  if (nch <= 256) return launch_cfg<T, 64, 4, true>(st, x, g, b, y, rows, (int)C, eps, mg);
  if (nch <= 384) return launch_cfg<T, 64, 6, true>(st, x, g, b, y, rows, (int)C, eps, mg);
  return launch_cfg<T, 64, 8, true>(st, x, g, b, y, rows, (int)C, eps, mg);
}

template <class T>
int launch(hipStream_t st, const void* x, const void* g, const void* b, void* y, int64_t rows, int64_t C, float eps) {
  if (!x || !g || !b || !y || rows <= 0 || C <= 0) return CODETR_E_BADARG;
  if (C % 8 != 0 || C > 4096) return CODETR_E_UNSUPPORTED;
  const int nch = (int)(C / 8);
  if (nch <= 32) return launch_cfg<T, 32, 1>(st, x, g, b, y, rows, (int)C, eps);
  if (nch <= 64) return launch_cfg<T, 64, 1>(st, x, g, b, y, rows, (int)C, eps);
  if (nch <= 128) return launch_cfg<T, 64, 2>(st, x, g, b, y, rows, (int)C, eps);
  if (nch <= 192) return launch_cfg<T, 64, 3>(st, x, g, b, y, rows, (int)C, eps);
  if (nch <= 256) return launch_cfg<T, 64, 4>(st, x, g, b, y, rows, (int)C, eps);
  if (nch <= 384) return launch_cfg<T, 64, 6>(st, x, g, b, y, rows, (int)C, eps);
  return launch_cfg<T, 64, 8>(st, x, g, b, y, rows, (int)C, eps);
}

}

extern "C" {

int codetr_layernorm_f16(void* stream, const void* x_dev, const void* gamma_dev, const void* beta_dev, void* y_dev,
                         int64_t rows, int64_t C, float eps) {
  return launch<LnHalf>(static_cast<hipStream_t>(stream), x_dev, gamma_dev, beta_dev, y_dev, rows, C, eps);
}

int codetr_layernorm_bf16(void* stream, const void* x_dev, const void* gamma_dev, const void* beta_dev, void* y_dev,
                          int64_t rows, int64_t C, float eps) {
  return launch<LnBf16>(static_cast<hipStream_t>(stream), x_dev, gamma_dev, beta_dev, y_dev, rows, C, eps);
}

int codetr_patch_merge_layernorm_f16(void* stream, const void* x_dev, const void* gamma_dev, const void* beta_dev,
                                     void* y_dev, int64_t B, int64_t H, int64_t W, int64_t C, float eps) {
  return launch_merge<LnHalf>(static_cast<hipStream_t>(stream), x_dev, gamma_dev, beta_dev, y_dev, B, H, W, C, eps);
}

int codetr_patch_merge_layernorm_bf16(void* stream, const void* x_dev, const void* gamma_dev, const void* beta_dev,
                                      void* y_dev, int64_t B, int64_t H, int64_t W, int64_t C, float eps) {
  return launch_merge<LnBf16>(static_cast<hipStream_t>(stream), x_dev, gamma_dev, beta_dev, y_dev, B, H, W, C, eps);
}

}
```

include/codetr_hip.h:

```cpp
#ifndef CODETR_HIP_H_
#define CODETR_HIP_H_

#include <stdint.h>

#ifdef __cplusplus
extern "C" {
#endif

#define CODETR_E_BADARG (-1)
#define CODETR_E_IM2COL_STEP (-2)
#define CODETR_E_TOO_LARGE (-3)
#define CODETR_E_UNSUPPORTED (-4)

#define CODETR_HIP_ABI_VERSION 53
int codetr_hip_abi_version(void);
const char *codetr_hip_strerror(int code);

int codetr_msda_forward_f16(void *stream, const void *value_dev, const int64_t *spatial_shapes_dev,
                            const int64_t *level_start_dev, const void *loc_dev, const void *weight_dev,
                            int64_t B, int64_t S, int M, int D, int L, int64_t Nq, int P, int64_t im2col_step,
                            void *out_dev);
int codetr_msda_forward_bf16(void *stream, const void *value_dev, const int64_t *spatial_shapes_dev,
                             const int64_t *level_start_dev, const void *loc_dev, const void *weight_dev,
                             int64_t B, int64_t S, int M, int D, int L, int64_t Nq, int P, int64_t im2col_step,
                             void *out_dev);
int codetr_msda_forward_f32(void *stream, const void *value_dev, const int64_t *spatial_shapes_dev,
                            const int64_t *level_start_dev, const void *loc_dev, const void *weight_dev,
                            int64_t B, int64_t S, int M, int D, int L, int64_t Nq, int P, int64_t im2col_step,
                            void *out_dev);
int codetr_msda_forward_f64(void *stream, const void *value_dev, const int64_t *spatial_shapes_dev,
                            const int64_t *level_start_dev, const void *loc_dev, const void *weight_dev,
                            int64_t B, int64_t S, int M, int D, int L, int64_t Nq, int P, int64_t im2col_step,
                            void *out_dev);

int codetr_msda_op4_supported(int elem_bytes, int64_t B, int64_t S, int M, int D, int L, int64_t Nq, int P);
int codetr_msda_op4_forward_f16(void *stream, const void *value_dev, const int64_t *spatial_shapes_dev,
                                const int64_t *level_start_dev, const void *loc_dev, const void *weight_dev, int64_t B,
                                int64_t S, int M, int D, int L, int64_t Nq, int P, void *out_dev);
int codetr_msda_op4_forward_bf16(void *stream, const void *value_dev, const int64_t *spatial_shapes_dev,
                                 const int64_t *level_start_dev, const void *loc_dev, const void *weight_dev, int64_t B,
                                 int64_t S, int M, int D, int L, int64_t Nq, int P, void *out_dev);

int codetr_msda_fused_forward_f16(void *stream, const void *value_dev, const int64_t *spatial_shapes_dev,
                                  const int64_t *level_start_dev, const void *offsets_dev, int64_t offsets_row_stride,
                                  const void *logits_dev, int64_t logits_row_stride, const void *ref_dev, int ref_dim,
                                  int value_head_major, int64_t B, int64_t S, int M, int D, int L, int64_t Nq, int P,
                                  void *out_dev);
int codetr_msda_fused_forward_bf16(void *stream, const void *value_dev, const int64_t *spatial_shapes_dev,
                                   const int64_t *level_start_dev, const void *offsets_dev, int64_t offsets_row_stride,
                                   const void *logits_dev, int64_t logits_row_stride, const void *ref_dev, int ref_dim,
                                   int value_head_major, int64_t B, int64_t S, int M, int D, int L, int64_t Nq, int P,
                                   void *out_dev);
int codetr_msda_fused_forward_ref32_f16(void *stream, const void *value_dev, const int64_t *spatial_shapes_dev,
                                        const int64_t *level_start_dev, const void *offsets_dev,
                                        int64_t offsets_row_stride, const void *logits_dev, int64_t logits_row_stride,
                                        const void *ref_dev, int ref_dim, int value_head_major, int64_t B, int64_t S,
                                        int M, int D, int L, int64_t Nq, int P, void *out_dev);
int codetr_msda_fused_forward_ref32_bf16(void *stream, const void *value_dev, const int64_t *spatial_shapes_dev,
                                         const int64_t *level_start_dev, const void *offsets_dev,
                                         int64_t offsets_row_stride, const void *logits_dev, int64_t logits_row_stride,
                                         const void *ref_dev, int ref_dim, int value_head_major, int64_t B, int64_t S,
                                         int M, int D, int L, int64_t Nq, int P, void *out_dev);

int codetr_msda_encoder_forward_packed_f16(void *stream, const void *value_dev, const int64_t *level_shapes_host,
                                           const void *packed_dev, int64_t packed_row_stride,
                                           const float *valid_counts_dev, int64_t B, int64_t S, int M, int D, int L, int P,
                                           const int8_t *windows_host, int region_w, int region_h, int threads,
// ... 105 lines not shown
                                      const void *rel_bias_dev, void *out8_dev, void *out_scales_dev, int64_t B, int64_t H,
                                      int64_t W, int num_heads, int head_dim, int window_size, int shift);

int codetr_add_f16(void *stream, const void *a_dev, const void *b_dev, void *out_dev, int64_t n, int64_t a_period);
int codetr_add_bf16(void *stream, const void *a_dev, const void *b_dev, void *out_dev, int64_t n, int64_t a_period);
int codetr_sigmoid_f16(void *stream, const void *x_dev, void *out_dev, int64_t n);
int codetr_sigmoid_bf16(void *stream, const void *x_dev, void *out_dev, int64_t n);
int codetr_gather_rows_b16(void *stream, const void *src_dev, const int64_t *idx_dev, void *out_dev, int64_t B, int64_t S,
                           int64_t K, int64_t C);
int codetr_decode_boxes_f16(void *stream, const void *coords_unact_dev, const int64_t *idx_dev, void *boxes_dev,
                            int64_t *labels_dev, int64_t B, int64_t Nq, int64_t K, int num_classes, float img_w,
                            float img_h);
int codetr_decode_boxes_bf16(void *stream, const void *coords_unact_dev, const int64_t *idx_dev, void *boxes_dev,
                            int64_t *labels_dev, int64_t B, int64_t Nq, int64_t K, int num_classes, float img_w,
                            float img_h);
int codetr_valid_ratios_f16(void *stream, const float *counts_dev, const void *level_wh_f16_dev, void *out_dev,
                            float *out32_dev, int64_t B, int L);
int codetr_valid_ratios_bf16(void *stream, const float *counts_dev, const void *level_wh_bf16_dev, void *out_dev,
                            float *out32_dev, int64_t B, int L);

int codetr_linear_splitk_plan(int64_t M, int64_t N, int64_t K, int64_t *workspace_bytes);
int codetr_linear_splitk_f16(void *stream, const void *x_dev, const void *w_dev, const void *bias_dev,
                             const void *residual_dev, const void *row_mask_dev, void *y_dev, int64_t M, int64_t N,
                             int64_t K, int act, int splits, void *workspace_dev, int64_t workspace_bytes);
int codetr_linear_splitk_bf16(void *stream, const void *x_dev, const void *w_dev, const void *bias_dev,
                              const void *residual_dev, const void *row_mask_dev, void *y_dev, int64_t M, int64_t N,
                              int64_t K, int act, int splits, void *workspace_dev, int64_t workspace_bytes);

int64_t codetr_linear_sk_workspace_bytes(void);
int codetr_linear_sk_supported(int64_t M, int64_t N, int64_t K);
int codetr_linear_sk_preferred(int64_t M, int64_t N, int64_t K, int act, int has_residual);
int codetr_linear_sk_f16(void *stream, const void *x_dev, const void *w_dev, const void *bias_dev,
                         const void *residual_dev, void *y_dev, int64_t M, int64_t N, int64_t K, int act,
                         void *workspace_dev, int64_t workspace_bytes, int flags);
int codetr_linear_sk_bf16(void *stream, const void *x_dev, const void *w_dev, const void *bias_dev,
                          const void *residual_dev, void *y_dev, int64_t M, int64_t N, int64_t K, int act,
                          void *workspace_dev, int64_t workspace_bytes, int flags);

int codetr_swin_mlp_supported(int64_t M, int64_t C, int64_t hidden);
int codetr_swin_mlp_f16(void *stream, const void *x_dev, const void *ln_gamma_dev, const void *ln_beta_dev, float ln_eps,
                        const void *w1_dev, const void *b1_dev, const void *w2_packed_dev, const void *b2_dev, void *y_dev,
                        int64_t M, int64_t C);
int codetr_swin_mlp_bf16(void *stream, const void *x_dev, const void *ln_gamma_dev, const void *ln_beta_dev, float ln_eps,
                         const void *w1_dev, const void *b1_dev, const void *w2_packed_dev, const void *b2_dev, void *y_dev,
                         int64_t M, int64_t C);

int codetr_linear_pp_supported(int64_t M, int64_t N, int64_t K);
int codetr_linear_pp_preferred(int64_t M, int64_t N, int64_t K, int act, int has_residual);
int codetr_linear_pp_f16(void *stream, const void *x_dev, const void *w_dev, const void *bias_dev,
                         const void *residual_dev, void *y_dev, int64_t M, int64_t N, int64_t K, int act, int flags);
int codetr_linear_pp_bf16(void *stream, const void *x_dev, const void *w_dev, const void *bias_dev,
                          const void *residual_dev, void *y_dev, int64_t M, int64_t N, int64_t K, int act, int flags);

int codetr_mask_pyramid(void *stream, const void *img_mask_dev, int64_t B, int64_t H_img, int64_t W_img,
                        int num_levels, const int64_t *level_shapes_host, void *mask_flat_dev, float *ycum_dev,
                        float *xcum_dev, float *valid_counts_dev, int mask_elem_bytes);

int codetr_query_sine_embed_f16(void *stream, const void *ref_dev, const void *valid_ratios_dev,
                                const float *valid_ratios32_dev, int64_t B, int64_t Nq, int ref_dim, int num_levels,
                                int pos_feat, float temperature, int apply_sigmoid, void *ref_in_dev,
                                float *ref_in32_dev, void *embed_dev);
int codetr_query_sine_embed_bf16(void *stream, const void *ref_dev, const void *valid_ratios_dev,
                                const float *valid_ratios32_dev, int64_t B, int64_t Nq, int ref_dim, int num_levels,
                                int pos_feat, float temperature, int apply_sigmoid, void *ref_in_dev,
                                float *ref_in32_dev, void *embed_dev);

int codetr_encoder_geometry_f16(void *stream, const void *valid_ratios_dev, const void *mask_flat_dev, int64_t B,
                                int num_levels, const int64_t *level_shapes_host, void *reference_points_dev,
                                void *reference_by_level_dev, void *proposals_dev, void *row_state_dev);
int codetr_encoder_geometry_bf16(void *stream, const void *valid_ratios_dev, const void *mask_flat_dev, int64_t B,
                                int num_levels, const int64_t *level_shapes_host, void *reference_points_dev,
                                void *reference_by_level_dev, void *proposals_dev, void *row_state_dev);

int codetr_row_max_f16(void *stream, const void *x_dev, void *out_dev, int64_t rows, int64_t C);
int codetr_row_max_bf16(void *stream, const void *x_dev, void *out_dev, int64_t rows, int64_t C);

int codetr_preprocess_u8_f16(void *stream, const void *src_dev, int64_t H_src, int64_t W_src, int64_t H_resized,
                             int64_t W_resized, int64_t H_pad, int64_t W_pad, const float *mean_host,
                             const float *std_host, const int *pad_value_host, void *dst_dev, void *mask_dev);
int codetr_preprocess_u8_f32(void *stream, const void *src_dev, int64_t H_src, int64_t W_src, int64_t H_resized,
                             int64_t W_resized, int64_t H_pad, int64_t W_pad, const float *mean_host,
                             const float *std_host, const int *pad_value_host, void *dst_dev, void *mask_dev);
int codetr_batched_nms_f32(void *stream, const float *boxes_sorted_dev, const int64_t *labels_sorted_dev, int64_t N,
                           float iou_threshold, void *keep_dev);

#define CODETR_PREPROCESS_BATCH_MAX 32
#define CODETR_POSTPROCESS_MAX_Q 1024
int codetr_preprocess_batch_u8_f16(void *stream, const void *src_dev, int64_t src_bytes, int64_t N,
                                   const int64_t *images_host, int64_t H, int64_t W, const float *mean_host,
                                   const float *std_host, const int *pad_value_host, float pad_fill, void *dst_dev,
                                   void *mask_dev);
int codetr_preprocess_batch_u8_bf16(void *stream, const void *src_dev, int64_t src_bytes, int64_t N,
                                    const int64_t *images_host, int64_t H, int64_t W, const float *mean_host,
                                    const float *std_host, const int *pad_value_host, float pad_fill, void *dst_dev,
                                    void *mask_dev);
int codetr_preprocess_batch_u8_f32(void *stream, const void *src_dev, int64_t src_bytes, int64_t N,
                                   const int64_t *images_host, int64_t H, int64_t W, const float *mean_host,
                                   const float *std_host, const int *pad_value_host, float pad_fill, void *dst_dev,
                                   void *mask_dev);
int codetr_postprocess_detections_f16(void *stream, const void *boxes_dev, const void *scores_dev,
                                      const int64_t *labels_dev, const void *divisor_dev, int64_t N, int64_t Q,
                                      int apply_threshold, float score_threshold, int apply_nms, float iou_threshold,
                                      void *boxes_out_dev, void *scores_out_dev, int64_t *labels_out_dev,
                                      int *count_dev);
int codetr_postprocess_detections_bf16(void *stream, const void *boxes_dev, const void *scores_dev,
                                       const int64_t *labels_dev, const void *divisor_dev, int64_t N, int64_t Q,
// ... 136 lines not shown
```

runner/dispatch_gen.inc:

```
static const int kPlanAbi = 53;
static int call_codetr_msda_forward_f16(void* fn, const Arg* a) { typedef int (*F)(const void*, const void*, const void*, const void*, const void*, const void*, long long, long long, int, int, int, long long, int, long long, const void*); return ((F)fn)((const void*)a[0].p, (const void*)a[1].p, (const void*)a[2].p, (const void*)a[3].p, (const void*)a[4].p, (const void*)a[5].p, (long long)a[6].i, (long long)a[7].i, (int)a[8].i, (int)a[9].i, (int)a[10].i, (long long)a[11].i, (int)a[12].i, (long long)a[13].i, (const void*)a[14].p); }
static int call_codetr_msda_forward_bf16(void* fn, const Arg* a) { typedef int (*F)(const void*, const void*, const void*, const void*, const void*, const void*, long long, long long, int, int, int, long long, int, long long, const void*); return ((F)fn)((const void*)a[0].p, (const void*)a[1].p, (const void*)a[2].p, (const void*)a[3].p, (const void*)a[4].p, (const void*)a[5].p, (long long)a[6].i, (long long)a[7].i, (int)a[8].i, (int)a[9].i, (int)a[10].i, (long long)a[11].i, (int)a[12].i, (long long)a[13].i, (const void*)a[14].p); }
static int call_codetr_msda_forward_f32(void* fn, const Arg* a) { typedef int (*F)(const void*, const void*, const void*, const void*, const void*, const void*, long long, long long, int, int, int, long long, int, long long, const void*); return ((F)fn)((const void*)a[0].p, (const void*)a[1].p, (const void*)a[2].p, (const void*)a[3].p, (const void*)a[4].p, (const void*)a[5].p, (long long)a[6].i, (long long)a[7].i, (int)a[8].i, (int)a[9].i, (int)a[10].i, (long long)a[11].i, (int)a[12].i, (long long)a[13].i, (const void*)a[14].p); }
static int call_codetr_msda_forward_f64(void* fn, const Arg* a) { typedef int (*F)(const void*, const void*, const void*, const void*, const void*, const void*, long long, long long, int, int, int, long long, int, long long, const void*); return ((F)fn)((const void*)a[0].p, (const void*)a[1].p, (const void*)a[2].p, (const void*)a[3].p, (const void*)a[4].p, (const void*)a[5].p, (long long)a[6].i, (long long)a[7].i, (int)a[8].i, (int)a[9].i, (int)a[10].i, (long long)a[11].i, (int)a[12].i, (long long)a[13].i, (const void*)a[14].p); }
static int call_codetr_msda_backward_f16(void* fn, const Arg* a) { typedef int (*F)(const void*, const void*, const void*, const void*, const void*, const void*, const void*, long long, long long, int, int, int, long long, int, long long, const void*, const void*, const void*); return ((F)fn)((const void*)a[0].p, (const void*)a[1].p, (const void*)a[2].p, (const void*)a[3].p, (const void*)a[4].p, (const void*)a[5].p, (const void*)a[6].p, (long long)a[7].i, (long long)a[8].i, (int)a[9].i, (int)a[10].i, (int)a[11].i, (long long)a[12].i, (int)a[13].i, (long long)a[14].i, (const void*)a[15].p, (const void*)a[16].p, (const void*)a[17].p); }
static int call_codetr_msda_backward_f32(void* fn, const Arg* a) { typedef int (*F)(const void*, const void*, const void*, const void*, const void*, const void*, const void*, long long, long long, int, int, int, long long, int, long long, const void*, const void*, const void*); return ((F)fn)((const void*)a[0].p, (const void*)a[1].p, (const void*)a[2].p, (const void*)a[3].p, (const void*)a[4].p, (const void*)a[5].p, (const void*)a[6].p, (long long)a[7].i, (long long)a[8].i, (int)a[9].i, (int)a[10].i, (int)a[11].i, (long long)a[12].i, (int)a[13].i, (long long)a[14].i, (const void*)a[15].p, (const void*)a[16].p, (const void*)a[17].p); }
static int call_codetr_msda_backward_f64(void* fn, const Arg* a) { typedef int (*F)(const void*, const void*, const void*, const void*, const void*, const void*, const void*, long long, long long, int, int, int, long long, int, long long, const void*, const void*, const void*); return ((F)fn)((const void*)a[0].p, (const void*)a[1].p, (const void*)a[2].p, (const void*)a[3].p, (const void*)a[4].p, (const void*)a[5].p, (const void*)a[6].p, (long long)a[7].i, (long long)a[8].i, (int)a[9].i, (int)a[10].i, (int)a[11].i, (long long)a[12].i, (int)a[13].i, (long long)a[14].i, (const void*)a[15].p, (const void*)a[16].p, (const void*)a[17].p); }
static int call_codetr_msda_fused_forward_f16(void* fn, const Arg* a) { typedef int (*F)(const void*, const void*, const void*, const void*, const void*, long long, const void*, long long, const void*, int, int, long long, long long, int, int, int, long long, int, const void*); return ((F)fn)((const void*)a[0].p, (const void*)a[1].p, (const void*)a[2].p, (const void*)a[3].p, (const void*)a[4].p, (long long)a[5].i, (const void*)a[6].p, (long long)a[7].i, (const void*)a[8].p, (int)a[9].i, (int)a[10].i, (long long)a[11].i, (long long)a[12].i, (int)a[13].i, (int)a[14].i, (int)a[15].i, (long long)a[16].i, (int)a[17].i, (const void*)a[18].p); }
static int call_codetr_msda_fused_forward_bf16(void* fn, const Arg* a) { typedef int (*F)(const void*, const void*, const void*, const void*, const void*, long long, const void*, long long, const void*, int, int, long long, long long, int, int, int, long long, int, const void*); return ((F)fn)((const void*)a[0].p, (const void*)a[1].p, (const void*)a[2].p, (const void*)a[3].p, (const void*)a[4].p, (long long)a[5].i, (const void*)a[6].p, (long long)a[7].i, (const void*)a[8].p, (int)a[9].i, (int)a[10].i, (long long)a[11].i, (long long)a[12].i, (int)a[13].i, (int)a[14].i, (int)a[15].i, (long long)a[16].i, (int)a[17].i, (const void*)a[18].p); }
static int call_codetr_msda_fused_forward_ref32_f16(void* fn, const Arg* a) { typedef int (*F)(const void*, const void*, const void*, const void*, const void*, long long, const void*, long long, const void*, int, int, long long, long long, int, int, int, long long, int, const void*); return ((F)fn)((const void*)a[0].p, (const void*)a[1].p, (const void*)a[2].p, (const void*)a[3].p, (const void*)a[4].p, (long long)a[5].i, (const void*)a[6].p, (long long)a[7].i, (const void*)a[8].p, (int)a[9].i, (int)a[10].i, (long long)a[11].i, (long long)a[12].i, (int)a[13].i, (int)a[14].i, (int)a[15].i, (long long)a[16].i, (int)a[17].i, (const void*)a[18].p); }
static int call_codetr_msda_fused_forward_ref32_bf16(void* fn, const Arg* a) { typedef int (*F)(const void*, const void*, const void*, const void*, const void*, long long, const void*, long long, const void*, int, int, long long, long long, int, int, int, long long, int, const void*); return ((F)fn)((const void*)a[0].p, (const void*)a[1].p, (const void*)a[2].p, (const void*)a[3].p, (const void*)a[4].p, (long long)a[5].i, (const void*)a[6].p, (long long)a[7].i, (const void*)a[8].p, (int)a[9].i, (int)a[10].i, (long long)a[11].i, (long long)a[12].i, (int)a[13].i, (int)a[14].i, (int)a[15].i, (long long)a[16].i, (int)a[17].i, (const void*)a[18].p); }
static int call_codetr_msda_encoder_forward_packed_f16(void* fn, const Arg* a) { typedef int (*F)(const void*, const void*, const void*, const void*, long long, const void*, long long, long long, int, int, int, int, const void*, int, int, int, int, const void*); return ((F)fn)((const void*)a[0].p, (const void*)a[1].p, (const void*)a[2].p, (const void*)a[3].p, (long long)a[4].i, (const void*)a[5].p, (long long)a[6].i, (long long)a[7].i, (int)a[8].i, (int)a[9].i, (int)a[10].i, (int)a[11].i, (const void*)a[12].p, (int)a[13].i, (int)a[14].i, (int)a[15].i, (int)a[16].i, (const void*)a[17].p); }
static int call_codetr_msda_encoder_forward_packed_bf16(void* fn, const Arg* a) { typedef int (*F)(const void*, const void*, const void*, const void*, long long, const void*, long long, long long, int, int, int, int, const void*, int, int, int, int, const void*); return ((F)fn)((const void*)a[0].p, (const void*)a[1].p, (const void*)a[2].p, (const void*)a[3].p, (long long)a[4].i, (const void*)a[5].p, (long long)a[6].i, (long long)a[7].i, (int)a[8].i, (int)a[9].i, (int)a[10].i, (int)a[11].i, (const void*)a[12].p, (int)a[13].i, (int)a[14].i, (int)a[15].i, (int)a[16].i, (const void*)a[17].p); }
static int call_codetr_linear_bf16_f16out(void* fn, const Arg* a) { typedef int (*F)(const void*, const void*, const void*, const void*, const void*, const void*, long long, long long, long long, long long, int); return ((F)fn)((const void*)a[0].p, (const void*)a[1].p, (const void*)a[2].p, (const void*)a[3].p, (const void*)a[4].p, (const void*)a[5].p, (long long)a[6].i, (long long)a[7].i, (long long)a[8].i, (long long)a[9].i, (int)a[10].i); }
static int call_codetr_encoder_projections_f16(void* fn, const Arg* a) { typedef int (*F)(const void*, const void*, const void*, const void*, const void*, const void*, const void*, const void*, long long, long long, long long, long long, long long, int); return ((F)fn)((const void*)a[0].p, (const void*)a[1].p, (const void*)a[2].p, (const void*)a[3].p, (const void*)a[4].p, (const void*)a[5].p, (const void*)a[6].p, (const void*)a[7].p, (long long)a[8].i, (long long)a[9].i, (long long)a[10].i, (long long)a[11].i, (long long)a[12].i, (int)a[13].i); }
static int call_codetr_encoder_projections_bf16(void* fn, const Arg* a) { typedef int (*F)(const void*, const void*, const void*, const void*, const void*, const void*, const void*, const void*, long long, long long, long long, long long, long long, int); return ((F)fn)((const void*)a[0].p, (const void*)a[1].p, (const void*)a[2].p, (const void*)a[3].p, (const void*)a[4].p, (const void*)a[5].p, (const void*)a[6].p, (const void*)a[7].p, (long long)a[8].i, (long long)a[9].i, (long long)a[10].i, (long long)a[11].i, (long long)a[12].i, (int)a[13].i); }
static int call_codetr_encoder_projections_posgen_f16(void* fn, const Arg* a) { typedef int (*F)(const void*, const void*, const void*, const void*, const void*, const void*, const void*, const void*, const void*, const void*, const void*, const void*, const void*, int, const void*, float, float, float, float, int, const void*, const void*, const void*, const void*, const void*, long long, long long, long long, long long, long long, long long, int); return ((F)fn)((const void*)a[0].p, (const void*)a[1].p, (const void*)a[2].p, (const void*)a[3].p, (const void*)a[4].p, (const void*)a[5].p, (const void*)a[6].p, (const void*)a[7].p, (const void*)a[8].p, (const void*)a[9].p, (const void*)a[10].p, (const void*)a[11].p, (const void*)a[12].p, (int)a[13].i, (const void*)a[14].p, (float)a[15].f, (float)a[16].f, (float)a[17].f, (float)a[18].f, (int)a[19].i, (const void*)a[20].p, (const void*)a[21].p, (const void*)a[22].p, (const void*)a[23].p, (const void*)a[24].p, (long long)a[25].i, (long long)a[26].i, (long long)a[27].i, (long long)a[28].i, (long long)a[29].i, (long long)a[30].i, (int)a[31].i); }
static int call_codetr_encoder_projections_posgen_bf16(void* fn, const Arg* a) { typedef int (*F)(const void*, const void*, const void*, const void*, const void*, const void*, const void*, const void*, const void*, const void*, const void*, const void*, const void*, int, const void*, float, float, float, float, int, const void*, const void*, const void*, const void*, const void*, long long, long long, long long, long long, long long, long long, int); return ((F)fn)((const void*)a[0].p, (const void*)a[1].p, (const void*)a[2].p, (const void*)a[3].p, (const void*)a[4].p, (const void*)a[5].p, (const void*)a[6].p, (const void*)a[7].p, (const void*)a[8].p, (const void*)a[9].p, (const void*)a[10].p, (const void*)a[11].p, (const void*)a[12].p, (int)a[13].i, (const void*)a[14].p, (float)a[15].f, (float)a[16].f, (float)a[17].f, (float)a[18].f, (int)a[19].i, (const void*)a[20].p, (const void*)a[21].p, (const void*)a[22].p, (const void*)a[23].p, (const void*)a[24].p, (long long)a[25].i, (long long)a[26].i, (long long)a[27].i, (long long)a[28].i, (long long)a[29].i, (long long)a[30].i, (int)a[31].i); }
static int call_codetr_linear_fp8mx(void* fn, const Arg* a) { typedef int (*F)(const void*, const void*, const void*, const void*, const void*, const void*, const void*, const void*, const void*, long long, long long, long long, int); return ((F)fn)((const void*)a[0].p, (const void*)a[1].p, (const void*)a[2].p, (const void*)a[3].p, (const void*)a[4].p, (const void*)a[5].p, (const void*)a[6].p, (const void*)a[7].p, (const void*)a[8].p, (long long)a[9].i, (long long)a[10].i, (long long)a[11].i, (int)a[12].i); }
static int call_codetr_cast_fp8mx_f16(void* fn, const Arg* a) { typedef int (*F)(const void*, const void*, const void*, const void*, long long, long long); return ((F)fn)((const void*)a[0].p, (const void*)a[1].p, (const void*)a[2].p, (const void*)a[3].p, (long long)a[4].i, (long long)a[5].i); }
static int call_codetr_layernorm_fp8mx_f16(void* fn, const Arg* a) { typedef int (*F)(const void*, const void*, const void*, const void*, const void*, const void*, long long, long long, float); return ((F)fn)((const void*)a[0].p, (const void*)a[1].p, (const void*)a[2].p, (const void*)a[3].p, (const void*)a[4].p, (const void*)a[5].p, (long long)a[6].i, (long long)a[7].i, (float)a[8].f); }
static int call_codetr_window_attention_fp8mx_f16(void* fn, const Arg* a) { typedef int (*F)(const void*, const void*, const void*, const void*, const void*, const void*, long long, long long, long long, int, int, int, int); return ((F)fn)((const void*)a[0].p, (const void*)a[1].p, (const void*)a[2].p, (const void*)a[3].p, (const void*)a[4].p, (const void*)a[5].p, (long long)a[6].i, (long long)a[7].i, (long long)a[8].i, (int)a[9].i, (int)a[10].i, (int)a[11].i, (int)a[12].i); }
static int call_codetr_mha_attention_f16(void* fn, const Arg* a) { typedef int (*F)(const void*, const void*, const void*, const void*, const void*, long long, long long, long long, int, int, long long, long long, long long, long long); return ((F)fn)((const void*)a[0].p, (const void*)a[1].p, (const void*)a[2].p, (const void*)a[3].p, (const void*)a[4].p, (long long)a[5].i, (long long)a[6].i, (long long)a[7].i, (int)a[8].i, (int)a[9].i, (long long)a[10].i, (long long)a[11].i, (long long)a[12].i, (long long)a[13].i); }
static int call_codetr_mha_attention_bf16(void* fn, const Arg* a) { typedef int (*F)(const void*, const void*, const void*, const void*, const void*, long long, long long, long long, int, int, long long, long long, long long, long long); return ((F)fn)((const void*)a[0].p, (const void*)a[1].p, (const void*)a[2].p, (const void*)a[3].p, (const void*)a[4].p, (long long)a[5].i, (long long)a[6].i, (long long)a[7].i, (int)a[8].i, (int)a[9].i, (long long)a[10].i, (long long)a[11].i, (long long)a[12].i, (long long)a[13].i); }
static int call_codetr_linear_ln_f16(void* fn, const Arg* a) { typedef int (*F)(const void*, const void*, const void*, const void*, float, const void*, const void*, const void*, long long, long long, long long, int); return ((F)fn)((const void*)a[0].p, (const void*)a[1].p, (const void*)a[2].p, (const void*)a[3].p, (float)a[4].f, (const void*)a[5].p, (const void*)a[6].p, (const void*)a[7].p, (long long)a[8].i, (long long)a[9].i, (long long)a[10].i, (int)a[11].i); }
static int call_codetr_linear_ln_bf16(void* fn, const Arg* a) { typedef int (*F)(const void*, const void*, const void*, const void*, float, const void*, const void*, const void*, long long, long long, long long, int); return ((F)fn)((const void*)a[0].p, (const void*)a[1].p, (const void*)a[2].p, (const void*)a[3].p, (float)a[4].f, (const void*)a[5].p, (const void*)a[6].p, (const void*)a[7].p, (long long)a[8].i, (long long)a[9].i, (long long)a[10].i, (int)a[11].i); }
static int call_codetr_linear_xadd_f16(void* fn, const Arg* a) { typedef int (*F)(const void*, const void*, const void*, const void*, const void*, const void*, long long, long long, long long); return ((F)fn)((const void*)a[0].p, (const void*)a[1].p, (const void*)a[2].p, (const void*)a[3].p, (const void*)a[4].p, (const void*)a[5].p, (long long)a[6].i, (long long)a[7].i, (long long)a[8].i); }
static int call_codetr_linear_xadd_bf16(void* fn, const Arg* a) { typedef int (*F)(const void*, const void*, const void*, const void*, const void*, const void*, long long, long long, long long); return ((F)fn)((const void*)a[0].p, (const void*)a[1].p, (const void*)a[2].p, (const void*)a[3].p, (const void*)a[4].p, (const void*)a[5].p, (long long)a[6].i, (long long)a[7].i, (long long)a[8].i); }
static int call_codetr_im2col_tokens_b16(void* fn, const Arg* a) { typedef int (*F)(const void*, const void*, long long, long long, long long, long long, int, int, int, const void*); return ((F)fn)((const void*)a[0].p, (const void*)a[1].p, (long long)a[2].i, (long long)a[3].i, (long long)a[4].i, (long long)a[5].i, (int)a[6].i, (int)a[7].i, (int)a[8].i, (const void*)a[9].p); }
static int call_codetr_conv_tokens_f16(void* fn, const Arg* a) { typedef int (*F)(const void*, const void*, const void*, const void*, const void*, const void*, long long, long long, long long, long long, long long, int, int, int, int); return ((F)fn)((const void*)a[0].p, (const void*)a[1].p, (const void*)a[2].p, (const void*)a[3].p, (const void*)a[4].p, (const void*)a[5].p, (long long)a[6].i, (long long)a[7].i, (long long)a[8].i, (long long)a[9].i, (long long)a[10].i, (int)a[11].i, (int)a[12].i, (int)a[13].i, (int)a[14].i); }
static int call_codetr_conv_tokens_bf16(void* fn, const Arg* a) { typedef int (*F)(const void*, const void*, const void*, const void*, const void*, const void*, long long, long long, long long, long long, long long, int, int, int, int); return ((F)fn)((const void*)a[0].p, (const void*)a[1].p, (const void*)a[2].p, (const void*)a[3].p, (const void*)a[4].p, (const void*)a[5].p, (long long)a[6].i, (long long)a[7].i, (long long)a[8].i, (long long)a[9].i, (long long)a[10].i, (int)a[11].i, (int)a[12].i, (int)a[13].i, (int)a[14].i); }
static int call_codetr_conv_im2col_nchw_b16(void* fn, const Arg* a) { typedef int (*F)(const void*, const void*, long long, int, long long, long long, int, int, int, int, const void*); return ((F)fn)((const void*)a[0].p, (const void*)a[1].p, (long long)a[2].i, (int)a[3].i, (long long)a[4].i, (long long)a[5].i, (int)a[6].i, (int)a[7].i, (int)a[8].i, (int)a[9].i, (const void*)a[10].p); }
static int call_codetr_maxpool_tokens_b16(void* fn, const Arg* a) { typedef int (*F)(const void*, const void*, long long, long long, long long, long long, int, int, int, int, const void*); return ((F)fn)((const void*)a[0].p, (const void*)a[1].p, (long long)a[2].i, (long long)a[3].i, (long long)a[4].i, (long long)a[5].i, (int)a[6].i, (int)a[7].i, (int)a[8].i, (int)a[9].i, (const void*)a[10].p); }
static int call_codetr_topk_chunked_f16(void* fn, const Arg* a) { typedef int (*F)(const void*, const void*, long long, long long, int, int, const void*, const void*, const void*, long long); return ((F)fn)((const void*)a[0].p, (const void*)a[1].p, (long long)a[2].i, (long long)a[3].i, (int)a[4].i, (int)a[5].i, (const void*)a[6].p, (const void*)a[7].p, (const void*)a[8].p, (long long)a[9].i); }
static int call_codetr_topk_chunked_bf16(void* fn, const Arg* a) { typedef int (*F)(const void*, const void*, long long, long long, int, int, const void*, const void*, const void*, long long); return ((F)fn)((const void*)a[0].p, (const void*)a[1].p, (long long)a[2].i, (long long)a[3].i, (int)a[4].i, (int)a[5].i, (const void*)a[6].p, (const void*)a[7].p, (const void*)a[8].p, (long long)a[9].i); }
static int call_codetr_topk_f16(void* fn, const Arg* a) { typedef int (*F)(const void*, const void*, long long, long long, int, const void*, const void*); return ((F)fn)((const void*)a[0].p, (const void*)a[1].p, (long long)a[2].i, (long long)a[3].i, (int)a[4].i, (const void*)a[5].p, (const void*)a[6].p); }
static int call_codetr_topk_bf16(void* fn, const Arg* a) { typedef int (*F)(const void*, const void*, long long, long long, int, const void*, const void*); return ((F)fn)((const void*)a[0].p, (const void*)a[1].p, (long long)a[2].i, (long long)a[3].i, (int)a[4].i, (const void*)a[5].p, (const void*)a[6].p); }
static int call_codetr_patch_im2col_b16(void* fn, const Arg* a) { typedef int (*F)(const void*, const void*, long long, int, long long, long long, int, int, const void*); return ((F)fn)((const void*)a[0].p, (const void*)a[1].p, (long long)a[2].i, (int)a[3].i, (long long)a[4].i, (long long)a[5].i, (int)a[6].i, (int)a[7].i, (const void*)a[8].p); }
static int call_codetr_add_f16(void* fn, const Arg* a) { typedef int (*F)(const void*, const void*, const void*, const void*, long long, long long); return ((F)fn)((const void*)a[0].p, (const void*)a[1].p, (const void*)a[2].p, (const void*)a[3].p, (long long)a[4].i, (long long)a[5].i); }
static int call_codetr_add_bf16(void* fn, const Arg* a) { typedef int (*F)(const void*, const void*, const void*, const void*, long long, long long); return ((F)fn)((const void*)a[0].p, (const void*)a[1].p, (const void*)a[2].p, (const void*)a[3].p, (long long)a[4].i, (long long)a[5].i); }
static int call_codetr_sigmoid_f16(void* fn, const Arg* a) { typedef int (*F)(const void*, const void*, const void*, long long); return ((F)fn)((const void*)a[0].p, (const void*)a[1].p, (const void*)a[2].p, (long long)a[3].i); }
static int call_codetr_sigmoid_bf16(void* fn, const Arg* a) { typedef int (*F)(const void*, const void*, const void*, long long); return ((F)fn)((const void*)a[0].p, (const void*)a[1].p, (const void*)a[2].p, (long long)a[3].i); }
static int call_codetr_gather_rows_b16(void* fn, const Arg* a) { typedef int (*F)(const void*, const void*, const void*, const void*, long long, long long, long long, long long); return ((F)fn)((const void*)a[0].p, (const void*)a[1].p, (const void*)a[2].p, (const void*)a[3].p, (long long)a[4].i, (long long)a[5].i, (long long)a[6].i, (long long)a[7].i); }
static int call_codetr_decode_boxes_f16(void* fn, const Arg* a) { typedef int (*F)(const void*, const void*, const void*, const void*, const void*, long long, long long, long long, int, float, float); return ((F)fn)((const void*)a[0].p, (const void*)a[1].p, (const void*)a[2].p, (const void*)a[3].p, (const void*)a[4].p, (long long)a[5].i, (long long)a[6].i, (long long)a[7].i, (int)a[8].i, (float)a[9].f, (float)a[10].f); }
static int call_codetr_decode_boxes_bf16(void* fn, const Arg* a) { typedef int (*F)(const void*, const void*, const void*, const void*, const void*, long long, long long, long long, int, float, float); return ((F)fn)((const void*)a[0].p, (const void*)a[1].p, (const void*)a[2].p, (const void*)a[3].p, (const void*)a[4].p, (long long)a[5].i, (long long)a[6].i, (long long)a[7].i, (int)a[8].i, (float)a[9].f, (float)a[10].f); }
static int call_codetr_valid_ratios_f16(void* fn, const Arg* a) { typedef int (*F)(const void*, const void*, const void*, const void*, const void*, long long, int); return ((F)fn)((const void*)a[0].p, (const void*)a[1].p, (const void*)a[2].p, (const void*)a[3].p, (const void*)a[4].p, (long long)a[5].i, (int)a[6].i); }
static int call_codetr_valid_ratios_bf16(void* fn, const Arg* a) { typedef int (*F)(const void*, const void*, const void*, const void*, const void*, long long, int); return ((F)fn)((const void*)a[0].p, (const void*)a[1].p, (const void*)a[2].p, (const void*)a[3].p, (const void*)a[4].p, (long long)a[5].i, (int)a[6].i); }
static int call_codetr_linear_fp8(void* fn, const Arg* a) { typedef int (*F)(const void*, const void*, const void*, const void*, float, const void*, const void*, const void*, int, float, long long, long long, long long, int); return ((F)fn)((const void*)a[0].p, (const void*)a[1].p, (const void*)a[2].p, (const void*)a[3].p, (float)a[4].f, (const void*)a[5].p, (const void*)a[6].p, (const void*)a[7].p, (int)a[8].i, (float)a[9].f, (long long)a[10].i, (long long)a[11].i, (long long)a[12].i, (int)a[13].i); }
static int call_codetr_cast_fp8_f16(void* fn, const Arg* a) { typedef int (*F)(const void*, const void*, const void*, long long, float); return ((F)fn)((const void*)a[0].p, (const void*)a[1].p, (const void*)a[2].p, (long long)a[3].i, (float)a[4].f); }
static int call_codetr_layernorm_fp8_f16(void* fn, const Arg* a) { typedef int (*F)(const void*, const void*, const void*, const void*, const void*, long long, long long, float, float); return ((F)fn)((const void*)a[0].p, (const void*)a[1].p, (const void*)a[2].p, (const void*)a[3].p, (const void*)a[4].p, (long long)a[5].i, (long long)a[6].i, (float)a[7].f, (float)a[8].f); }
static int call_codetr_linear_f16(void* fn, const Arg* a) { typedef int (*F)(const void*, const void*, const void*, const void*, const void*, const void*, const void*, long long, long long, long long, int, long long, int); return ((F)fn)((const void*)a[0].p, (const void*)a[1].p, (const void*)a[2].p, (const void*)a[3].p, (const void*)a[4].p, (const void*)a[5].p, (const void*)a[6].p, (long long)a[7].i, (long long)a[8].i, (long long)a[9].i, (int)a[10].i, (long long)a[11].i, (int)a[12].i); }
static int call_codetr_linear_bf16(void* fn, const Arg* a) { typedef int (*F)(const void*, const void*, const void*, const void*, const void*, const void*, const void*, long long, long long, long long, int, long long, int); return ((F)fn)((const void*)a[0].p, (const void*)a[1].p, (const void*)a[2].p, (const void*)a[3].p, (const void*)a[4].p, (const void*)a[5].p, (const void*)a[6].p, (long long)a[7].i, (long long)a[8].i, (long long)a[9].i, (int)a[10].i, (long long)a[11].i, (int)a[12].i); }
static int call_codetr_query_sine_embed_f16(void* fn, const Arg* a) { typedef int (*F)(const void*, const void*, const void*, const void*, long long, long long, int, int, int, float, int, const void*, const void*, const void*); return ((F)fn)((const void*)a[0].p, (const void*)a[1].p, (const void*)a[2].p, (const void*)a[3].p, (long long)a[4].i, (long long)a[5].i, (int)a[6].i, (int)a[7].i, (int)a[8].i, (float)a[9].f, (int)a[10].i, (const void*)a[11].p, (const void*)a[12].p, (const void*)a[13].p); }
static int call_codetr_query_sine_embed_bf16(void* fn, const Arg* a) { typedef int (*F)(const void*, const void*, const void*, const void*, long long, long long, int, int, int, float, int, const void*, const void*, const void*); return ((F)fn)((const void*)a[0].p, (const void*)a[1].p, (const void*)a[2].p, (const void*)a[3].p, (long long)a[4].i, (long long)a[5].i, (int)a[6].i, (int)a[7].i, (int)a[8].i, (float)a[9].f, (int)a[10].i, (const void*)a[11].p, (const void*)a[12].p, (const void*)a[13].p); }
static int call_codetr_encoder_geometry_f16(void* fn, const Arg* a) { typedef int (*F)(const void*, const void*, const void*, long long, int, const void*, const void*, const void*, const void*, const void*); return ((F)fn)((const void*)a[0].p, (const void*)a[1].p, (const void*)a[2].p, (long long)a[3].i, (int)a[4].i, (const void*)a[5].p, (const void*)a[6].p, (const void*)a[7].p, (const void*)a[8].p, (const void*)a[9].p); }
static int call_codetr_encoder_geometry_bf16(void* fn, const Arg* a) { typedef int (*F)(const void*, const void*, const void*, long long, int, const void*, const void*, const void*, const void*, const void*); return ((F)fn)((const void*)a[0].p, (const void*)a[1].p, (const void*)a[2].p, (long long)a[3].i, (int)a[4].i, (const void*)a[5].p, (const void*)a[6].p, (const void*)a[7].p, (const void*)a[8].p, (const void*)a[9].p); }
static int call_codetr_row_max_f16(void* fn, const Arg* a) { typedef int (*F)(const void*, const void*, const void*, long long, long long); return ((F)fn)((const void*)a[0].p, (const void*)a[1].p, (const void*)a[2].p, (long long)a[3].i, (long long)a[4].i); }
static int call_codetr_row_max_bf16(void* fn, const Arg* a) { typedef int (*F)(const void*, const void*, const void*, long long, long long); return ((F)fn)((const void*)a[0].p, (const void*)a[1].p, (const void*)a[2].p, (long long)a[3].i, (long long)a[4].i); }
static int call_codetr_preprocess_u8_f16(void* fn, const Arg* a) { typedef int (*F)(const void*, const void*, long long, long long, long long, long long, long long, long long, const void*, const void*, const void*, const void*, const void*); return ((F)fn)((const void*)a[0].p, (const void*)a[1].p, (long long)a[2].i, (long long)a[3].i, (long long)a[4].i, (long long)a[5].i, (long long)a[6].i, (long long)a[7].i, (const void*)a[8].p, (const void*)a[9].p, (const void*)a[10].p, (const void*)a[11].p, (const void*)a[12].p); }
static int call_codetr_preprocess_u8_f32(void* fn, const Arg* a) { typedef int (*F)(const void*, const void*, long long, long long, long long, long long, long long, long long, const void*, const void*, const void*, const void*, const void*); return ((F)fn)((const void*)a[0].p, (const void*)a[1].p, (long long)a[2].i, (long long)a[3].i, (long long)a[4].i, (long long)a[5].i, (long long)a[6].i, (long long)a[7].i, (const void*)a[8].p, (const void*)a[9].p, (const void*)a[10].p, (const void*)a[11].p, (const void*)a[12].p); }
static int call_codetr_batched_nms_f32(void* fn, const Arg* a) { typedef int (*F)(const void*, const void*, const void*, long long, float, const void*); return ((F)fn)((const void*)a[0].p, (const void*)a[1].p, (const void*)a[2].p, (long long)a[3].i, (float)a[4].f, (const void*)a[5].p); }
static int call_codetr_preprocess_batch_u8_f16(void* fn, const Arg* a) { typedef int (*F)(const void*, const void*, long long, long long, const void*, long long, long long, const void*, const void*, const void*, float, const void*, const void*); return ((F)fn)((const void*)a[0].p, (const void*)a[1].p, (long long)a[2].i, (long long)a[3].i, (const void*)a[4].p, (long long)a[5].i, (long long)a[6].i, (const void*)a[7].p, (const void*)a[8].p, (const void*)a[9].p, (float)a[10].f, (const void*)a[11].p, (const void*)a[12].p); }
static int call_codetr_preprocess_batch_u8_bf16(void* fn, const Arg* a) { typedef int (*F)(const void*, const void*, long long, long long, const void*, long long, long long, const void*, const void*, const void*, float, const void*, const void*); return ((F)fn)((const void*)a[0].p, (const void*)a[1].p, (long long)a[2].i, (long long)a[3].i, (const void*)a[4].p, (long long)a[5].i, (long long)a[6].i, (const void*)a[7].p, (const void*)a[8].p, (const void*)a[9].p, (float)a[10].f, (const void*)a[11].p, (const void*)a[12].p); }
static int call_codetr_preprocess_batch_u8_f32(void* fn, const Arg* a) { typedef int (*F)(const void*, const void*, long long, long long, const void*, long long, long long, const void*, const void*, const void*, float, const void*, const void*); return ((F)fn)((const void*)a[0].p, (const void*)a[1].p, (long long)a[2].i, (long long)a[3].i, (const void*)a[4].p, (long long)a[5].i, (long long)a[6].i, (const void*)a[7].p, (const void*)a[8].p, (const void*)a[9].p, (float)a[10].f, (const void*)a[11].p, (const void*)a[12].p); }
static int call_codetr_postprocess_detections_f16(void* fn, const Arg* a) { typedef int (*F)(const void*, const void*, const void*, const void*, const void*, long long, long long, int, float, int, float, const void*, const void*, const void*, const void*); return ((F)fn)((const void*)a[0].p, (const void*)a[1].p, (const void*)a[2].p, (const void*)a[3].p, (const void*)a[4].p, (long long)a[5].i, (long long)a[6].i, (int)a[7].i, (float)a[8].f, (int)a[9].i, (float)a[10].f, (const void*)a[11].p, (const void*)a[12].p, (const void*)a[13].p, (const void*)a[14].p); }
static int call_codetr_postprocess_detections_bf16(void* fn, const Arg* a) { typedef int (*F)(const void*, const void*, const void*, const void*, const void*, long long, long long, int, float, int, float, const void*, const void*, const void*, const void*); return ((F)fn)((const void*)a[0].p, (const void*)a[1].p, (const void*)a[2].p, (const void*)a[3].p, (const void*)a[4].p, (long long)a[5].i, (long long)a[6].i, (int)a[7].i, (float)a[8].f, (int)a[9].i, (float)a[10].f, (const void*)a[11].p, (const void*)a[12].p, (const void*)a[13].p, (const void*)a[14].p); }
static int call_codetr_postprocess_detections_f32(void* fn, const Arg* a) { typedef int (*F)(const void*, const void*, const void*, const void*, const void*, long long, long long, int, float, int, float, const void*, const void*, const void*, const void*); return ((F)fn)((const void*)a[0].p, (const void*)a[1].p, (const void*)a[2].p, (const void*)a[3].p, (const void*)a[4].p, (long long)a[5].i, (long long)a[6].i, (int)a[7].i, (float)a[8].f, (int)a[9].i, (float)a[10].f, (const void*)a[11].p, (const void*)a[12].p, (const void*)a[13].p, (const void*)a[14].p); }
static int call_codetr_patch_merge_layernorm_f16(void* fn, const Arg* a) { typedef int (*F)(const void*, const void*, const void*, const void*, const void*, long long, long long, long long, long long, float); return ((F)fn)((const void*)a[0].p, (const void*)a[1].p, (const void*)a[2].p, (const void*)a[3].p, (const void*)a[4].p, (long long)a[5].i, (long long)a[6].i, (long long)a[7].i, (long long)a[8].i, (float)a[9].f); }
static int call_codetr_patch_merge_layernorm_bf16(void* fn, const Arg* a) { typedef int (*F)(const void*, const void*, const void*, const void*, const void*, long long, long long, long long, long long, float); return ((F)fn)((const void*)a[0].p, (const void*)a[1].p, (const void*)a[2].p, (const void*)a[3].p, (const void*)a[4].p, (long long)a[5].i, (long long)a[6].i, (long long)a[7].i, (long long)a[8].i, (float)a[9].f); }
static int call_codetr_mask_pyramid(void* fn, const Arg* a) { typedef int (*F)(const void*, const void*, long long, long long, long long, int, const void*, const void*, const void*, const void*, const void*, int); return ((F)fn)((const void*)a[0].p, (const void*)a[1].p, (long long)a[2].i, (long long)a[3].i, (long long)a[4].i, (int)a[5].i, (const void*)a[6].p, (const void*)a[7].p, (const void*)a[8].p, (const void*)a[9].p, (const void*)a[10].p, (int)a[11].i); }
static int call_codetr_linear_splitk_f16(void* fn, const Arg* a) { typedef int (*F)(const void*, const void*, const void*, const void*, const void*, const void*, const void*, long long, long long, long long, int, int, const void*, long long); return ((F)fn)((const void*)a[0].p, (const void*)a[1].p, (const void*)a[2].p, (const void*)a[3].p, (const void*)a[4].p, (const void*)a[5].p, (const void*)a[6].p, (long long)a[7].i, (long long)a[8].i, (long long)a[9].i, (int)a[10].i, (int)a[11].i, (const void*)a[12].p, (long long)a[13].i); }
static int call_codetr_linear_splitk_bf16(void* fn, const Arg* a) { typedef int (*F)(const void*, const void*, const void*, const void*, const void*, const void*, const void*, long long, long long, long long, int, int, const void*, long long); return ((F)fn)((const void*)a[0].p, (const void*)a[1].p, (const void*)a[2].p, (const void*)a[3].p, (const void*)a[4].p, (const void*)a[5].p, (const void*)a[6].p, (long long)a[7].i, (long long)a[8].i, (long long)a[9].i, (int)a[10].i, (int)a[11].i, (const void*)a[12].p, (long long)a[13].i); }
static int call_codetr_linear_sk_f16(void* fn, const Arg* a) { typedef int (*F)(const void*, const void*, const void*, const void*, const void*, const void*, long long, long long, long long, int, const void*, long long, int); return ((F)fn)((const void*)a[0].p, (const void*)a[1].p, (const void*)a[2].p, (const void*)a[3].p, (const void*)a[4].p, (const void*)a[5].p, (long long)a[6].i, (long long)a[7].i, (long long)a[8].i, (int)a[9].i, (const void*)a[10].p, (long long)a[11].i, (int)a[12].i); }
static int call_codetr_msda_op4_forward_f16(void* fn, const Arg* a) { typedef int (*F)(const void*, const void*, const void*, const void*, const void*, const void*, long long, long long, int, int, int, long long, int, const void*); return ((F)fn)((const void*)a[0].p, (const void*)a[1].p, (const void*)a[2].p, (const void*)a[3].p, (const void*)a[4].p, (const void*)a[5].p, (long long)a[6].i, (long long)a[7].i, (int)a[8].i, (int)a[9].i, (int)a[10].i, (long long)a[11].i, (int)a[12].i, (const void*)a[13].p); }
static int call_codetr_msda_op4_forward_bf16(void* fn, const Arg* a) { typedef int (*F)(const void*, const void*, const void*, const void*, const void*, const void*, long long, long long, int, int, int, long long, int, const void*); return ((F)fn)((const void*)a[0].p, (const void*)a[1].p, (const void*)a[2].p, (const void*)a[3].p, (const void*)a[4].p, (const void*)a[5].p, (long long)a[6].i, (long long)a[7].i, (int)a[8].i, (int)a[9].i, (int)a[10].i, (long long)a[11].i, (int)a[12].i, (const void*)a[13].p); }
static int call_codetr_swin_mlp_f16(void* fn, const Arg* a) { typedef int (*F)(const void*, const void*, const void*, const void*, float, const void*, const void*, const void*, const void*, const void*, long long, long long); return ((F)fn)((const void*)a[0].p, (const void*)a[1].p, (const void*)a[2].p, (const void*)a[3].p, (float)a[4].f, (const void*)a[5].p, (const void*)a[6].p, (const void*)a[7].p, (const void*)a[8].p, (const void*)a[9].p, (long long)a[10].i, (long long)a[11].i); }
static int call_codetr_swin_mlp_bf16(void* fn, const Arg* a) { typedef int (*F)(const void*, const void*, const void*, const void*, float, const void*, const void*, const void*, const void*, const void*, long long, long long); return ((F)fn)((const void*)a[0].p, (const void*)a[1].p, (const void*)a[2].p, (const void*)a[3].p, (float)a[4].f, (const void*)a[5].p, (const void*)a[6].p, (const void*)a[7].p, (const void*)a[8].p, (const void*)a[9].p, (long long)a[10].i, (long long)a[11].i); }
static int call_codetr_linear_pp_f16(void* fn, const Arg* a) { typedef int (*F)(const void*, const void*, const void*, const void*, const void*, const void*, long long, long long, long long, int, int); return ((F)fn)((const void*)a[0].p, (const void*)a[1].p, (const void*)a[2].p, (const void*)a[3].p, (const void*)a[4].p, (const void*)a[5].p, (long long)a[6].i, (long long)a[7].i, (long long)a[8].i, (int)a[9].i, (int)a[10].i); }
static int call_codetr_linear_pp_bf16(void* fn, const Arg* a) { typedef int (*F)(const void*, const void*, const void*, const void*, const void*, const void*, long long, long long, long long, int, int); return ((F)fn)((const void*)a[0].p, (const void*)a[1].p, (const void*)a[2].p, (const void*)a[3].p, (const void*)a[4].p, (const void*)a[5].p, (long long)a[6].i, (long long)a[7].i, (long long)a[8].i, (int)a[9].i, (int)a[10].i); }
static int call_codetr_linear_sk_bf16(void* fn, const Arg* a) { typedef int (*F)(const void*, const void*, const void*, const void*, const void*, const void*, long long, long long, long long, int, const void*, long long, int); return ((F)fn)((const void*)a[0].p, (const void*)a[1].p, (const void*)a[2].p, (const void*)a[3].p, (const void*)a[4].p, (const void*)a[5].p, (long long)a[6].i, (long long)a[7].i, (long long)a[8].i, (int)a[9].i, (const void*)a[10].p, (long long)a[11].i, (int)a[12].i); }
static int call_codetr_decoder_layer_f16(void* fn, const Arg* a) { typedef int (*F)(const void*, const void*, const void*, const void*, const void*, const void*, const void*, const void*, const void*, const void*, const void*, const void*, const void*, const void*, const void*, const void*, const void*, const void*, long long, long long, long long, int, int, int, float, float); return ((F)fn)((const void*)a[0].p, (const void*)a[1].p, (const void*)a[2].p, (const void*)a[3].p, (const void*)a[4].p, (const void*)a[5].p, (const void*)a[6].p, (const void*)a[7].p, (const void*)a[8].p, (const void*)a[9].p, (const void*)a[10].p, (const void*)a[11].p, (const void*)a[12].p, (const void*)a[13].p, (const void*)a[14].p, (const void*)a[15].p, (const void*)a[16].p, (const void*)a[17].p, (long long)a[18].i, (long long)a[19].i, (long long)a[20].i, (int)a[21].i, (int)a[22].i, (int)a[23].i, (float)a[24].f, (float)a[25].f); }
static int call_codetr_decoder_layer_bf16(void* fn, const Arg* a) { typedef int (*F)(const void*, const void*, const void*, const void*, const void*, const void*, const void*, const void*, const void*, const void*, const void*, const void*, const void*, const void*, const void*, const void*, const void*, const void*, long long, long long, long long, int, int, int, float, float); return ((F)fn)((const void*)a[0].p, (const void*)a[1].p, (const void*)a[2].p, (const void*)a[3].p, (const void*)a[4].p, (const void*)a[5].p, (const void*)a[6].p, (const void*)a[7].p, (const void*)a[8].p, (const void*)a[9].p, (const void*)a[10].p, (const void*)a[11].p, (const void*)a[12].p, (const void*)a[13].p, (const void*)a[14].p, (const void*)a[15].p, (const void*)a[16].p, (const void*)a[17].p, (long long)a[18].i, (long long)a[19].i, (long long)a[20].i, (int)a[21].i, (int)a[22].i, (int)a[23].i, (float)a[24].f, (float)a[25].f); }
static int call_codetr_layernorm_f16(void* fn, const Arg* a) { typedef int (*F)(const void*, const void*, const void*, const void*, const void*, long long, long long, float); return ((F)fn)((const void*)a[0].p, (const void*)a[1].p, (const void*)a[2].p, (const void*)a[3].p, (const void*)a[4].p, (long long)a[5].i, (long long)a[6].i, (float)a[7].f); }
static int call_codetr_layernorm_bf16(void* fn, const Arg* a) { typedef int (*F)(const void*, const void*, const void*, const void*, const void*, long long, long long, float); return ((F)fn)((const void*)a[0].p, (const void*)a[1].p, (const void*)a[2].p, (const void*)a[3].p, (const void*)a[4].p, (long long)a[5].i, (long long)a[6].i, (float)a[7].f); }
static int call_codetr_groupnorm_tokens_f16(void* fn, const Arg* a) { typedef int (*F)(const void*, const void*, const void*, const void*, const void*, long long, const void*, long long, long long, long long, int, float); return ((F)fn)((const void*)a[0].p, (const void*)a[1].p, (const void*)a[2].p, (const void*)a[3].p, (const void*)a[4].p, (long long)a[5].i, (const void*)a[6].p, (long long)a[7].i, (long long)a[8].i, (long long)a[9].i, (int)a[10].i, (float)a[11].f); }
static int call_codetr_groupnorm_tokens_bf16(void* fn, const Arg* a) { typedef int (*F)(const void*, const void*, const void*, const void*, const void*, long long, const void*, long long, long long, long long, int, float); return ((F)fn)((const void*)a[0].p, (const void*)a[1].p, (const void*)a[2].p, (const void*)a[3].p, (const void*)a[4].p, (long long)a[5].i, (const void*)a[6].p, (long long)a[7].i, (long long)a[8].i, (long long)a[9].i, (int)a[10].i, (float)a[11].f); }
static int call_codetr_sine_pos_tokens_f16(void* fn, const Arg* a) { typedef int (*F)(const void*, const void*, const void*, const void*, const void*, long long, long long, long long, long long, int, float, float, float, float, int); return ((F)fn)((const void*)a[0].p, (const void*)a[1].p, (const void*)a[2].p, (const void*)a[3].p, (const void*)a[4].p, (long long)a[5].i, (long long)a[6].i, (long long)a[7].i, (long long)a[8].i, (int)a[9].i, (float)a[10].f, (float)a[11].f, (float)a[12].f, (float)a[13].f, (int)a[14].i); }
static int call_codetr_sine_pos_tokens_bf16(void* fn, const Arg* a) { typedef int (*F)(const void*, const void*, const void*, const void*, const void*, long long, long long, long long, long long, int, float, float, float, float, int); return ((F)fn)((const void*)a[0].p, (const void*)a[1].p, (const void*)a[2].p, (const void*)a[3].p, (const void*)a[4].p, (long long)a[5].i, (long long)a[6].i, (long long)a[7].i, (long long)a[8].i, (int)a[9].i, (float)a[10].f, (float)a[11].f, (float)a[12].f, (float)a[13].f, (int)a[14].i); }
static int call_codetr_ffn_relu_f16(void* fn, const Arg* a) { typedef int (*F)(const void*, const void*, const void*, const void*, const void*, const void*, const void*, long long, long long, long long); return ((F)fn)((const void*)a[0].p, (const void*)a[1].p, (const void*)a[2].p, (const void*)a[3].p, (const void*)a[4].p, (const void*)a[5].p, (const void*)a[6].p, (long long)a[7].i, (long long)a[8].i, (long long)a[9].i); }
static int call_codetr_ffn_relu_ln_f16(void* fn, const Arg* a) { typedef int (*F)(const void*, const void*, const void*, const void*, const void*, const void*, const void*, long long, long long, long long, const void*, const void*, float, const void*, const void*); return ((F)fn)((const void*)a[0].p, (const void*)a[1].p, (const void*)a[2].p, (const void*)a[3].p, (const void*)a[4].p, (const void*)a[5].p, (const void*)a[6].p, (long long)a[7].i, (long long)a[8].i, (long long)a[9].i, (const void*)a[10].p, (const void*)a[11].p, (float)a[12].f, (const void*)a[13].p, (const void*)a[14].p); }
static int call_codetr_ffn_relu_ln2_f16(void* fn, const Arg* a) { typedef int (*F)(const void*, const void*, const void*, const void*, const void*, const void*, const void*, long long, long long, long long, const void*, const void*, float, const void*, const void*, float, const void*, const void*); return ((F)fn)((const void*)a[0].p, (const void*)a[1].p, (const void*)a[2].p, (const void*)a[3].p, (const void*)a[4].p, (const void*)a[5].p, (const void*)a[6].p, (long long)a[7].i, (long long)a[8].i, (long long)a[9].i, (const void*)a[10].p, (const void*)a[11].p, (float)a[12].f, (const void*)a[13].p, (const void*)a[14].p, (float)a[15].f, (const void*)a[16].p, (const void*)a[17].p); }
static int call_codetr_ffn_relu_ln2_bf16(void* fn, const Arg* a) { typedef int (*F)(const void*, const void*, const void*, const void*, const void*, const void*, const void*, long long, long long, long long, const void*, const void*, float, const void*, const void*, float, const void*, const void*); return ((F)fn)((const void*)a[0].p, (const void*)a[1].p, (const void*)a[2].p, (const void*)a[3].p, (const void*)a[4].p, (const void*)a[5].p, (const void*)a[6].p, (long long)a[7].i, (long long)a[8].i, (long long)a[9].i, (const void*)a[10].p, (const void*)a[11].p, (float)a[12].f, (const void*)a[13].p, (const void*)a[14].p, (float)a[15].f, (const void*)a[16].p, (const void*)a[17].p); }
static int call_codetr_ffn_pack_w2_f16(void* fn, const Arg* a) { typedef int (*F)(const void*, const void*, const void*, long long, long long); return ((F)fn)((const void*)a[0].p, (const void*)a[1].p, (const void*)a[2].p, (long long)a[3].i, (long long)a[4].i); }
static int call_codetr_ffn_oproj_relu_ln2_f16(void* fn, const Arg* a) { typedef int (*F)(const void*, const void*, const void*, const void*, const void*, const void*, const void*, const void*, const void*, const void*, long long, long long, long long, const void*, const void*, float, const void*, const void*, float, const void*, const void*); return ((F)fn)((const void*)a[0].p, (const void*)a[1].p, (const void*)a[2].p, (const void*)a[3].p, (const void*)a[4].p, (const void*)a[5].p, (const void*)a[6].p, (const void*)a[7].p, (const void*)a[8].p, (const void*)a[9].p, (long long)a[10].i, (long long)a[11].i, (long long)a[12].i, (const void*)a[13].p, (const void*)a[14].p, (float)a[15].f, (const void*)a[16].p, (const void*)a[17].p, (float)a[18].f, (const void*)a[19].p, (const void*)a[20].p); }
static int call_codetr_ffn_oproj_relu_ln2_bf16(void* fn, const Arg* a) { typedef int (*F)(const void*, const void*, const void*, const void*, const void*, const void*, const void*, const void*, const void*, const void*, long long, long long, long long, const void*, const void*, float, const void*, const void*, float, const void*, const void*); return ((F)fn)((const void*)a[0].p, (const void*)a[1].p, (const void*)a[2].p, (const void*)a[3].p, (const void*)a[4].p, (const void*)a[5].p, (const void*)a[6].p, (const void*)a[7].p, (const void*)a[8].p, (const void*)a[9].p, (long long)a[10].i, (long long)a[11].i, (long long)a[12].i, (const void*)a[13].p, (const void*)a[14].p, (float)a[15].f, (const void*)a[16].p, (const void*)a[17].p, (float)a[18].f, (const void*)a[19].p, (const void*)a[20].p); }
static int call_codetr_ffn_fp8(void* fn, const Arg* a) { typedef int (*F)(const void*, const void*, const void*, const void*, const void*, const void*, const void*, const void*, const void*, long long, long long, long long, float, float, const void*, const void*, float, const void*, const void*, float, const void*, const void*); return ((F)fn)((const void*)a[0].p, (const void*)a[1].p, (const void*)a[2].p, (const void*)a[3].p, (const void*)a[4].p, (const void*)a[5].p, (const void*)a[6].p, (const void*)a[7].p, (const void*)a[8].p, (long long)a[9].i, (long long)a[10].i, (long long)a[11].i, (float)a[12].f, (float)a[13].f, (const void*)a[14].p, (const void*)a[15].p, (float)a[16].f, (const void*)a[17].p, (const void*)a[18].p, (float)a[19].f, (const void*)a[20].p, (const void*)a[21].p); }
static int call_codetr_window_attention_f16(void* fn, const Arg* a) { typedef int (*F)(const void*, const void*, const void*, const void*, const void*, long long, long long, long long, int, int, int, int); return ((F)fn)((const void*)a[0].p, (const void*)a[1].p, (const void*)a[2].p, (const void*)a[3].p, (const void*)a[4].p, (long long)a[5].i, (long long)a[6].i, (long long)a[7].i, (int)a[8].i, (int)a[9].i, (int)a[10].i, (int)a[11].i); }
static int call_codetr_window_attention_bf16(void* fn, const Arg* a) { typedef int (*F)(const void*, const void*, const void*, const void*, const void*, long long, long long, long long, int, int, int, int); return ((F)fn)((const void*)a[0].p, (const void*)a[1].p, (const void*)a[2].p, (const void*)a[3].p, (const void*)a[4].p, (long long)a[5].i, (long long)a[6].i, (long long)a[7].i, (int)a[8].i, (int)a[9].i, (int)a[10].i, (int)a[11].i); }
static int call_codetr_window_attention_ex(void* fn, const Arg* a) { typedef int (*F)(const void*, const void*, const void*, const void*, const void*, const void*, float, long long, long long, long long, int, int, int, int, int, int, int); return ((F)fn)((const void*)a[0].p, (const void*)a[1].p, (const void*)a[2].p, (const void*)a[3].p, (const void*)a[4].p, (const void*)a[5].p, (float)a[6].f, (long long)a[7].i, (long long)a[8].i, (long long)a[9].i, (int)a[10].i, (int)a[11].i, (int)a[12].i, (int)a[13].i, (int)a[14].i, (int)a[15].i, (int)a[16].i); }
static int call_codetr_window_attention_fp8out_f16(void* fn, const Arg* a) { typedef int (*F)(const void*, const void*, const void*, const void*, const void*, float, long long, long long, long long, int, int, int, int); return ((F)fn)((const void*)a[0].p, (const void*)a[1].p, (const void*)a[2].p, (const void*)a[3].p, (const void*)a[4].p, (float)a[5].f, (long long)a[6].i, (long long)a[7].i, (long long)a[8].i, (int)a[9].i, (int)a[10].i, (int)a[11].i, (int)a[12].i); }
static const Entry kEntries[] = {
  {"codetr_msda_forward_f16", 15, call_codetr_msda_forward_f16},
  {"codetr_msda_forward_bf16", 15, call_codetr_msda_forward_bf16},
  {"codetr_msda_forward_f32", 15, call_codetr_msda_forward_f32},
  {"codetr_msda_forward_f64", 15, call_codetr_msda_forward_f64},
  {"codetr_msda_backward_f16", 18, call_codetr_msda_backward_f16},
  {"codetr_msda_backward_f32", 18, call_codetr_msda_backward_f32},
  {"codetr_msda_backward_f64", 18, call_codetr_msda_backward_f64},
  {"codetr_msda_fused_forward_f16", 19, call_codetr_msda_fused_forward_f16},
  {"codetr_msda_fused_forward_bf16", 19, call_codetr_msda_fused_forward_bf16},
  {"codetr_msda_fused_forward_ref32_f16", 19, call_codetr_msda_fused_forward_ref32_f16},
  {"codetr_msda_fused_forward_ref32_bf16", 19, call_codetr_msda_fused_forward_ref32_bf16},
  {"codetr_msda_encoder_forward_packed_f16", 18, call_codetr_msda_encoder_forward_packed_f16},
  {"codetr_msda_encoder_forward_packed_bf16", 18, call_codetr_msda_encoder_forward_packed_bf16},
  {"codetr_linear_bf16_f16out", 11, call_codetr_linear_bf16_f16out},
  {"codetr_encoder_projections_f16", 14, call_codetr_encoder_projections_f16},
  {"codetr_encoder_projections_bf16", 14, call_codetr_encoder_projections_bf16},
  {"codetr_encoder_projections_posgen_f16", 32, call_codetr_encoder_projections_posgen_f16},
  {"codetr_encoder_projections_posgen_bf16", 32, call_codetr_encoder_projections_posgen_bf16},
  {"codetr_linear_fp8mx", 13, call_codetr_linear_fp8mx},
  {"codetr_cast_fp8mx_f16", 6, call_codetr_cast_fp8mx_f16},
  {"codetr_layernorm_fp8mx_f16", 9, call_codetr_layernorm_fp8mx_f16},
  {"codetr_window_attention_fp8mx_f16", 13, call_codetr_window_attention_fp8mx_f16},
  {"codetr_mha_attention_f16", 14, call_codetr_mha_attention_f16},
  {"codetr_mha_attention_bf16", 14, call_codetr_mha_attention_bf16},
  {"codetr_linear_ln_f16", 12, call_codetr_linear_ln_f16},
  {"codetr_linear_ln_bf16", 12, call_codetr_linear_ln_bf16},
  {"codetr_linear_xadd_f16", 9, call_codetr_linear_xadd_f16},
  {"codetr_linear_xadd_bf16", 9, call_codetr_linear_xadd_bf16},
  {"codetr_im2col_tokens_b16", 10, call_codetr_im2col_tokens_b16},
  {"codetr_conv_tokens_f16", 15, call_codetr_conv_tokens_f16},
  {"codetr_conv_tokens_bf16", 15, call_codetr_conv_tokens_bf16},
  {"codetr_conv_im2col_nchw_b16", 11, call_codetr_conv_im2col_nchw_b16},
  {"codetr_maxpool_tokens_b16", 11, call_codetr_maxpool_tokens_b16},
  {"codetr_topk_chunked_f16", 10, call_codetr_topk_chunked_f16},
  {"codetr_topk_chunked_bf16", 10, call_codetr_topk_chunked_bf16},
  {"codetr_topk_f16", 7, call_codetr_topk_f16},
  {"codetr_topk_bf16", 7, call_codetr_topk_bf16},
  {"codetr_patch_im2col_b16", 9, call_codetr_patch_im2col_b16},
  {"codetr_add_f16", 6, call_codetr_add_f16},
  {"codetr_add_bf16", 6, call_codetr_add_bf16},
  {"codetr_sigmoid_f16", 4, call_codetr_sigmoid_f16},
  {"codetr_sigmoid_bf16", 4, call_codetr_sigmoid_bf16},
  {"codetr_gather_rows_b16", 8, call_codetr_gather_rows_b16},
  {"codetr_decode_boxes_f16", 11, call_codetr_decode_boxes_f16},
  {"codetr_decode_boxes_bf16", 11, call_codetr_decode_boxes_bf16},
  {"codetr_valid_ratios_f16", 7, call_codetr_valid_ratios_f16},
  {"codetr_valid_ratios_bf16", 7, call_codetr_valid_ratios_bf16},
  {"codetr_linear_fp8", 14, call_codetr_linear_fp8},
  {"codetr_cast_fp8_f16", 5, call_codetr_cast_fp8_f16},
  {"codetr_layernorm_fp8_f16", 9, call_codetr_layernorm_fp8_f16},
  {"codetr_linear_f16", 13, call_codetr_linear_f16},
  {"codetr_linear_bf16", 13, call_codetr_linear_bf16},
  {"codetr_query_sine_embed_f16", 14, call_codetr_query_sine_embed_f16},
  {"codetr_query_sine_embed_bf16", 14, call_codetr_query_sine_embed_bf16},
  {"codetr_encoder_geometry_f16", 10, call_codetr_encoder_geometry_f16},
  {"codetr_encoder_geometry_bf16", 10, call_codetr_encoder_geometry_bf16},
  {"codetr_row_max_f16", 5, call_codetr_row_max_f16},
  {"codetr_row_max_bf16", 5, call_codetr_row_max_bf16},
  {"codetr_preprocess_u8_f16", 13, call_codetr_preprocess_u8_f16},
  {"codetr_preprocess_u8_f32", 13, call_codetr_preprocess_u8_f32},
  {"codetr_batched_nms_f32", 6, call_codetr_batched_nms_f32},
  {"codetr_preprocess_batch_u8_f16", 13, call_codetr_preprocess_batch_u8_f16},
  {"codetr_preprocess_batch_u8_bf16", 13, call_codetr_preprocess_batch_u8_bf16},
  {"codetr_preprocess_batch_u8_f32", 13, call_codetr_preprocess_batch_u8_f32},
  {"codetr_postprocess_detections_f16", 15, call_codetr_postprocess_detections_f16},
  {"codetr_postprocess_detections_bf16", 15, call_codetr_postprocess_detections_bf16},
  {"codetr_postprocess_detections_f32", 15, call_codetr_postprocess_detections_f32},
  {"codetr_patch_merge_layernorm_f16", 10, call_codetr_patch_merge_layernorm_f16},
  {"codetr_patch_merge_layernorm_bf16", 10, call_codetr_patch_merge_layernorm_bf16},
  {"codetr_mask_pyramid", 12, call_codetr_mask_pyramid},
  {"codetr_linear_splitk_f16", 14, call_codetr_linear_splitk_f16},
  {"codetr_linear_splitk_bf16", 14, call_codetr_linear_splitk_bf16},
  {"codetr_linear_sk_f16", 13, call_codetr_linear_sk_f16},
  {"codetr_msda_op4_forward_f16", 14, call_codetr_msda_op4_forward_f16},
  {"codetr_msda_op4_forward_bf16", 14, call_codetr_msda_op4_forward_bf16},
  {"codetr_swin_mlp_f16", 12, call_codetr_swin_mlp_f16},
  {"codetr_swin_mlp_bf16", 12, call_codetr_swin_mlp_bf16},
  {"codetr_linear_pp_f16", 11, call_codetr_linear_pp_f16},
  {"codetr_linear_pp_bf16", 11, call_codetr_linear_pp_bf16},
  {"codetr_linear_sk_bf16", 13, call_codetr_linear_sk_bf16},
  {"codetr_decoder_layer_f16", 26, call_codetr_decoder_layer_f16},
  {"codetr_decoder_layer_bf16", 26, call_codetr_decoder_layer_bf16},
  {"codetr_layernorm_f16", 8, call_codetr_layernorm_f16},
  {"codetr_layernorm_bf16", 8, call_codetr_layernorm_bf16},
  {"codetr_groupnorm_tokens_f16", 12, call_codetr_groupnorm_tokens_f16},
  {"codetr_groupnorm_tokens_bf16", 12, call_codetr_groupnorm_tokens_bf16},
  {"codetr_sine_pos_tokens_f16", 15, call_codetr_sine_pos_tokens_f16},
  {"codetr_sine_pos_tokens_bf16", 15, call_codetr_sine_pos_tokens_bf16},
  {"codetr_ffn_relu_f16", 10, call_codetr_ffn_relu_f16},
  {"codetr_ffn_relu_ln_f16", 15, call_codetr_ffn_relu_ln_f16},
  {"codetr_ffn_relu_ln2_f16", 18, call_codetr_ffn_relu_ln2_f16},
  {"codetr_ffn_relu_ln2_bf16", 18, call_codetr_ffn_relu_ln2_bf16},
  {"codetr_ffn_pack_w2_f16", 5, call_codetr_ffn_pack_w2_f16},
  {"codetr_ffn_oproj_relu_ln2_f16", 21, call_codetr_ffn_oproj_relu_ln2_f16},
  {"codetr_ffn_oproj_relu_ln2_bf16", 21, call_codetr_ffn_oproj_relu_ln2_bf16},
  {"codetr_ffn_fp8", 22, call_codetr_ffn_fp8},
  {"codetr_window_attention_f16", 12, call_codetr_window_attention_f16},
  {"codetr_window_attention_bf16", 12, call_codetr_window_attention_bf16},
  {"codetr_window_attention_ex", 17, call_codetr_window_attention_ex},
  {"codetr_window_attention_fp8out_f16", 13, call_codetr_window_attention_fp8out_f16},
};
```

Measured before the change: 99.63.

## Fold LayerNorm into following GEMM using per-row stats from producer epilogue

Adds an LN-folded persistent GEMM path for Swin blocks. The LayerNorm gain is folded into pre-scaled weights, and the mean and variance correction is applied in the epilogue using per-row partial statistics. Those statistics are emitted by the previous linear's epilogue (proj, fc2, patch-merge reduction), with a standalone row_stats kernel as fallback. This aims to remove the separate normalization pass and its activation read/write before qkv and fc1. In exchange, the producing GEMMs do extra epilogue work, and the folded fp16 weights plus E[x^2]-style statistics may lose some numerical accuracy.

```diff
diff --git a/co-detr-tensorrt_amd/codetr/_cabi.py b/co-detr-tensorrt_amd/codetr/_cabi.py
--- a/co-detr-tensorrt_amd/codetr/_cabi.py
+++ b/co-detr-tensorrt_amd/codetr/_cabi.py
@@ -5,7 +5,7 @@
 
 _HERE = os.path.dirname(os.path.abspath(__file__))
 LIB_PATH = os.path.join(_HERE, "libcodetr_hip.so")
-ABI_VERSION = 53
+ABI_VERSION = 54
 
 _i64, _i32, _vp, _cp = ctypes.c_int64, ctypes.c_int, ctypes.c_void_p, ctypes.c_char_p
 
@@ -123,6 +123,12 @@
     "codetr_linear_pp_preferred": (_i32, [_i64, _i64, _i64, _i32, _i32]),
     "codetr_linear_pp_f16": (_i32, [_vp, _vp, _vp, _vp, _vp, _vp, _i64, _i64, _i64, _i32, _i32]),
     "codetr_linear_pp_bf16": (_i32, [_vp, _vp, _vp, _vp, _vp, _vp, _i64, _i64, _i64, _i32, _i32]),
+    "codetr_linear_pp_stats_f16": (_i32, [_vp, _vp, _vp, _vp, _vp, _vp, _vp, _i64, _i64, _i64]),
+    "codetr_linear_pp_stats_bf16": (_i32, [_vp, _vp, _vp, _vp, _vp, _vp, _vp, _i64, _i64, _i64]),
+    "codetr_row_stats_f16": (_i32, [_vp, _vp, _vp, _i64, _i64]),
+    "codetr_row_stats_bf16": (_i32, [_vp, _vp, _vp, _i64, _i64]),
+    "codetr_linear_pp_lnfold_f16": (_i32, [_vp, _vp, _vp, _i64, ctypes.c_float, _vp, _vp, _vp, _vp, _i64, _i64, _i64, _i32]),
+    "codetr_linear_pp_lnfold_bf16": (_i32, [_vp, _vp, _vp, _i64, ctypes.c_float, _vp, _vp, _vp, _vp, _i64, _i64, _i64, _i32]),
     "codetr_linear_sk_bf16": (_i32, [_vp, _vp, _vp, _vp, _vp, _vp, _i64, _i64, _i64, _i32, _vp, _i64, _i32]),
     "codetr_decoder_layer_supported": (_i32, [_i32] * 7),
     "codetr_decoder_layer_blob_halfs": (_i64, [_i32] * 4),
@@ -170,7 +176,7 @@
          "query_sine_embed": 0, "encoder_geometry": 0, "row_max": 0, "preprocess": 0, "batched_nms": 0,
          "preprocess_batch": 0, "postprocess_detections": 0,
          "msda_backward": 0, "patch_merge_layernorm": 0, "msda_encoder": 0, "msda_encoder_packed": 0, "patch_im2col": 0, "mha_attention": 0, "topk": 0,
-         "linear_pp": 0, "swin_mlp": 0, "linear_tile128": 0, "linear_tile256": 0, "linear_xs": 0, "linear_ln": 0, "linear_xadd": 0, "encoder_projections": 0,
+         "linear_pp": 0, "linear_lnfold": 0, "linear_pp_stats": 0, "row_stats": 0, "swin_mlp": 0, "linear_tile128": 0, "linear_tile256": 0, "linear_xs": 0, "linear_ln": 0, "linear_xadd": 0, "encoder_projections": 0,
          "linear_fp8": 0, "cast_fp8": 0, "layernorm_fp8": 0, "small_ops": 0, "ffn_fp8": 0, "decoder_layer": 0,
          "conv_tokens": 0, "conv_im2col_nchw": 0, "maxpool_tokens": 0}
 
@@ -375,6 +381,10 @@
     return v
 
 
+def linear_pp_supported(M, N, K) -> bool:
+    return bool(load().codetr_linear_pp_supported(M, N, K))
+
+
 def linear_pp(x2d, weight, bias, residual2d, act, out2d, flags=0):
     lib = load()
     CALLS["linear"] += 1
@@ -386,6 +396,43 @@
             bias.data_ptr() if bias is not None else None,
             residual2d.data_ptr() if residual2d is not None else None, out2d.data_ptr(), M, N, K, _ACT[act], flags)
     check(rc, "codetr_linear_pp")
+    return out2d
+
+
+def linear_pp_stats(x2d, weight, bias, residual2d, out2d, rec):
+    lib = load()
+    CALLS["linear"] += 1
+    CALLS["linear_pp"] += 1
+    CALLS["linear_pp_stats"] += 1
+    M, K = x2d.shape
+    N = weight.shape[0]
+    fn = lib.codetr_linear_pp_stats_f16 if x2d.dtype == torch.float16 else lib.codetr_linear_pp_stats_bf16
+    rc = fn(current_stream_ptr(x2d.device), x2d.data_ptr(), weight.data_ptr(),
+            bias.data_ptr() if bias is not None else None,
+            residual2d.data_ptr() if residual2d is not None else None, out2d.data_ptr(), rec.data_ptr(), M, N, K)
+    check(rc, "codetr_linear_pp_stats")
+    return out2d
+
+
+def row_stats(x2d, rec):
+    CALLS["row_stats"] += 1
+    rows, C = x2d.shape
+    fn = load().codetr_row_stats_f16 if x2d.dtype == torch.float16 else load().codetr_row_stats_bf16
+    check(fn(current_stream_ptr(x2d.device), x2d.data_ptr(), rec.data_ptr(), rows, C), "codetr_row_stats")
+    return rec
+
+
+def linear_pp_lnfold(x2d, rec, eps, w_scaled, s, c, act, out2d):
+    lib = load()
+    CALLS["linear"] += 1
+    CALLS["linear_pp"] += 1
+    CALLS["linear_lnfold"] += 1
+    M, K = x2d.shape
+    N = w_scaled.shape[0]
+    fn = lib.codetr_linear_pp_lnfold_f16 if x2d.dtype == torch.float16 else lib.codetr_linear_pp_lnfold_bf16
+    rc = fn(current_stream_ptr(x2d.device), x2d.data_ptr(), rec.data_ptr(), rec.shape[1], float(eps), w_scaled.data_ptr(),
+            s.data_ptr(), c.data_ptr(), out2d.data_ptr(), M, N, K, _ACT[act])
+    check(rc, "codetr_linear_pp_lnfold")
     return out2d
 
 
diff --git a/co-detr-tensorrt_amd/codetr/_kernel_names.py b/co-detr-tensorrt_amd/codetr/_kernel_names.py
--- a/co-detr-tensorrt_amd/codetr/_kernel_names.py
+++ b/co-detr-tensorrt_amd/codetr/_kernel_names.py
@@ -42,6 +42,7 @@
     "preprocess_kernel",
     "query_sine_embed_kernel",
     "row_max_kernel",
+    "row_stats_kernel",
     "sigmoid_kernel",
     "sine_pos_kernel",
     "splitk_reduce_kernel",
diff --git a/co-detr-tensorrt_amd/codetr/hip_ops.py b/co-detr-tensorrt_amd/codetr/hip_ops.py
--- a/co-detr-tensorrt_amd/codetr/hip_ops.py
+++ b/co-detr-tensorrt_amd/codetr/hip_ops.py
@@ -59,7 +59,7 @@
             and (bias is None or bias.data_ptr() % 16 == 0))
 
 
-def linear(x, weight, bias=None, act=None, residual=None, row_mask=None, head_major=None):
+def linear(x, weight, bias=None, act=None, residual=None, row_mask=None, head_major=None, ln_stats=False):
     _gpu(x, "linear")
     if _cabi.linear_supported(x, weight):
         K = x.shape[-1]
@@ -85,6 +85,7 @@
                 raise ValueError("head_major needs a [B, S, K] input and no residual")
             hm_rows, hm_hd = x.shape[1], int(head_major)
         out = torch.empty((x2.shape[0], N), dtype=x.dtype, device=x.device)
+        rec = None
         if x2.shape[0] > 0:
             with torch.cuda.device(x.device):
                 res_act = act == "relu_res"
@@ -96,7 +97,12 @@
                     launch = lambda: _cabi.linear_splitk(x2, w, bias, r2, act, out, splits, ws, mk)
                 elif (LINEAR_PP and _persistent_ok(mk, head_major, out, x2, w, r2, bias)
                       and _cabi.linear_pp_preferred(x2.shape[0], N, K, act, r2 is not None)):
-                    launch = lambda: _cabi.linear_pp(x2, w, bias, r2, act, out)
+                    if (ln_stats and act is None and ln_fold_width(x.dtype, N) and (bias is None) == (r2 is None)
+                            and not torch.is_grad_enabled()):
+                        rec = torch.empty((x2.shape[0], N // 64, 2), dtype=torch.float32, device=x.device)
+                        launch = lambda: _cabi.linear_pp_stats(x2, w, bias, r2, out, rec)
+                    else:
+                        launch = lambda: _cabi.linear_pp(x2, w, bias, r2, act, out)
                 elif (_persistent_ok(mk, head_major, out, x2, w, r2, bias)
                       and _cabi.linear_sk_preferred(x2.shape[0], N, K, act, r2 is not None)):
                     launch = lambda: _cabi.linear_sk(x2, w, bias, r2, act, out)
@@ -113,7 +119,10 @@
                     LINEAR_PROFILE.append((e0, e1, 2.0 * x2.shape[0] * N * K, x2.shape[0], N, K))
         if head_major:
             return out.view(x.shape[0], N // hm_hd, hm_rows, hm_hd)
-        return out.view(*x.shape[:-1], N)
+        y = out.view(*x.shape[:-1], N)
+        if rec is not None:
+            y._codetr_ln_rec = rec
+        return y
     if head_major:
         raise RuntimeError("head_major output exists only on the native linear (f16/bf16, K % 64 == 0)")
     y = F.linear(x, weight, bias)
@@ -137,14 +146,72 @@
 LN_GEMM = True
 
 
-def linear_ln_supported(x, norm_weight, weight):
+LN_FOLD = True
+
+
+def ln_fold_width(dtype, C):
+    return LN_FOLD and dtype in (torch.float16, torch.bfloat16) and C >= 768 and C % 64 == 0 and C <= 2048
+
+
+def linear_lnfold_supported(x, norm_weight, norm_bias, weight, act=None):
+    C, N = x.shape[-1], weight.shape[0]
+    return (x.is_cuda and ln_fold_width(x.dtype, C) and not torch.is_grad_enabled() and act in (None, "gelu")
+            and norm_weight is not None and norm_bias is not None and norm_weight.dtype == x.dtype
+            and weight.dtype == x.dtype and norm_weight.shape[0] == C and weight.shape[1] == C and N % 8 == 0
+            and x.numel() > 0 and _cabi.linear_pp_supported(x.numel() // C, N, C))
+
+
+def ln_fold_operands(norm_weight, norm_bias, weight, bias):
+    ps = [weight, norm_weight, norm_bias] + ([bias] if bias is not None else [])
+
+    def build():
+        w64 = weight.detach().double()
+        ws = (w64 * norm_weight.detach().double()[None, :]).to(weight.dtype).contiguous()
+        s = ws.double().sum(1).float().contiguous()
+        c = w64 @ norm_bias.detach().double()
+        if bias is not None:
+            c = c + bias.detach().double()
+        return ws, s, c.float().contiguous()
+
+    return derived(ps, "_codetr_ln_fold", build)
+
+
+def _linear_lnfold(x, norm_weight, norm_bias, eps, weight, bias, act):
+    K, N = x.shape[-1], weight.shape[0]
+    x2 = x.reshape(-1, K)
+    x2 = x2 if x2.is_contiguous() else x2.contiguous()
+    ws, s, c = ln_fold_operands(norm_weight, norm_bias, weight, bias)
+    out = torch.empty((x2.shape[0], N), dtype=x.dtype, device=x.device)
+    rec = getattr(x, "_codetr_ln_rec", None)
+    with torch.cuda.device(x.device):
+        if (rec is None or rec.device != x.device or rec.dim() != 3 or rec.shape[0] != x2.shape[0]
+                or K % rec.shape[1] != 0 or x2.data_ptr() != x.data_ptr()):
+            rec = _cabi.row_stats(x2, torch.empty((x2.shape[0], 1, 2), dtype=torch.float32, device=x.device))
+        launch = lambda: _cabi.linear_pp_lnfold(x2, rec, eps, ws, s, c, act, out)
+        if LINEAR_PROFILE is None:
+            launch()
+        else:
+            st = torch.cuda.current_stream(x.device)
+            e0, e1 = torch.cuda.Event(enable_timing=True), torch.cuda.Event(enable_timing=True)
+            e0.record(st)
+            launch()
+            e1.record(st)
+            LINEAR_PROFILE.append((e0, e1, 2.0 * x2.shape[0] * N * K, x2.shape[0], N, K))
+    return out.view(*x.shape[:-1], N)
+
+
+def linear_ln_supported(x, norm_weight, weight, fold=False, norm_bias=None):
+    if fold and linear_lnfold_supported(x, norm_weight, norm_bias, weight):
+        return True
     return (LN_GEMM and x.is_cuda and norm_weight is not None and norm_weight.dtype == x.dtype and weight.dtype == x.dtype
             and not torch.is_grad_enabled() and norm_weight.shape[0] == x.shape[-1]
             and _cabi.linear_xadd_supported(x.numel() // max(x.shape[-1], 1), weight.shape[0], x.shape[-1], x.dtype))
 
 
-def linear_ln(x, norm_weight, norm_bias, eps, weight, bias=None, act=None):
+def linear_ln(x, norm_weight, norm_bias, eps, weight, bias=None, act=None, fold=False):
     _gpu(x, "linear_ln")
+    if fold and linear_lnfold_supported(x, norm_weight, norm_bias, weight, act):
+        return _linear_lnfold(x, norm_weight, norm_bias, eps, weight, bias, act)
     if linear_ln_supported(x, norm_weight, weight):
         K, N = x.shape[-1], weight.shape[0]
         x2 = x.reshape(-1, K)
@@ -731,7 +798,7 @@
 MSDA_FP32_REF = True
 
 
-_SWITCH_DEFAULTS = {"ENC_POSGEN": True, "WINDOW_BIAS_LANE": True, "LINEAR_PP": True, "SWIN_MLP": True, "SWIN_MLP_MIN_ROWS": 32768, "LN_GEMM": True, "XADD": True, "XADD_MIN_ROWS": 0, "MERGE_LN": True, "MSDA_ENCODER": True,
+_SWITCH_DEFAULTS = {"ENC_POSGEN": True, "WINDOW_BIAS_LANE": True, "LINEAR_PP": True, "SWIN_MLP": True, "SWIN_MLP_MIN_ROWS": 32768, "LN_GEMM": True, "LN_FOLD": True, "XADD": True, "XADD_MIN_ROWS": 0, "MERGE_LN": True, "MSDA_ENCODER": True,
                     "MSDA_FP32_REF": True, "FP8_MIN_TILES": 96,
                     "R50_NATIVE": True, "R50_CONV_IM2COL": False}
 
diff --git a/co-detr-tensorrt_amd/codetr/swin.py b/co-detr-tensorrt_amd/codetr/swin.py
--- a/co-detr-tensorrt_amd/codetr/swin.py
+++ b/co-detr-tensorrt_amd/codetr/swin.py
@@ -71,11 +71,11 @@
             if (self.norm is not None and isinstance(self.norm, nn.LayerNorm)
                     and hip_ops.patch_merge_layernorm_supported(x, C)):
                 x = hip_ops.patch_merge_layernorm(x.reshape(B, -1, C), (2 * H2, 2 * W2), nw, nb, self.norm.eps)
-                return hip_ops.linear(x, rw, self.reduction.bias), (H2, W2)
+                return hip_ops.linear(x, rw, self.reduction.bias, ln_stats=True), (H2, W2)
             x = x.view(B, H2, 2, W2, 2, C).permute(0, 1, 3, 2, 4, 5).reshape(B, H2 * W2, 4 * C)
             if self.norm is not None:
                 x = hip_ops.layer_norm(x, nw, nb, self.norm.eps)
-            return hip_ops.linear(x, rw, self.reduction.bias), (H2, W2)
+            return hip_ops.linear(x, rw, self.reduction.bias, ln_stats=True), (H2, W2)
         x = x.view(B, H2, 2, W2, 2, C).permute(0, 1, 3, 5, 2, 4).reshape(B, H2 * W2, 4 * C)
         if self.norm is not None:
             x = hip_ops.layer_norm(x, self.norm.weight, self.norm.bias, self.norm.eps)
@@ -169,11 +169,11 @@
         m = self.w_msa
         if hip_ops.swin_window_attention_supported(query, C, m.num_heads, ws):
             if pre_norm is not None:
-                qkv = hip_ops.linear_ln(query, pre_norm[0], pre_norm[1], pre_norm[2], m.qkv.weight, m.qkv.bias)
+                qkv = hip_ops.linear_ln(query, pre_norm[0], pre_norm[1], pre_norm[2], m.qkv.weight, m.qkv.bias, fold=True)
             else:
                 qkv = hip_ops.linear(query, m.qkv.weight, m.qkv.bias)
             o = hip_ops.swin_window_attention(qkv, m.qkv.bias, m.relative_position_bias(), hw_shape, m.num_heads, ws, sh)
-            return hip_ops.linear(o, m.proj.weight, m.proj.bias, residual=identity)
+            return hip_ops.linear(o, m.proj.weight, m.proj.bias, residual=identity, ln_stats=True)
         x = query.view(B, H, W, C)
         pad_r, pad_b = (-W) % ws, (-H) % ws
         if pad_r or pad_b:
@@ -221,7 +221,7 @@
                 if ops and all(hip_ops.linear_fp8_supported(rows, ws[o]) for o in ops):
                     return self._forward_fp8mx(x, hw_shape)
         if (isinstance(n1, nn.LayerNorm) and self.attn.takes_norm(x, hw_shape)
-                and hip_ops.linear_ln_supported(x, n1.weight, self.attn.w_msa.qkv.weight)):
+                and hip_ops.linear_ln_supported(x, n1.weight, self.attn.w_msa.qkv.weight, fold=True, norm_bias=n1.bias)):
             x = self.attn(x, hw_shape, identity=x, pre_norm=(n1.weight, n1.bias, n1.eps))
         else:
             h = hip_ops.layer_norm(x, n1.weight, n1.bias, n1.eps)
@@ -231,9 +231,10 @@
                 and hip_ops.swin_mlp_supported(x, n2.weight, fc1.weight, fc2.weight, self.ffn.act)):
             return hip_ops.swin_mlp(x, n2.weight, n2.bias, n2.eps, fc1.weight, fc1.bias, fc2.weight, fc2.bias)
         if (isinstance(n2, nn.LayerNorm) and self.ffn.add_identity
-                and hip_ops.linear_ln_supported(x, n2.weight, fc1.weight)):
-            h = hip_ops.linear_ln(x, n2.weight, n2.bias, n2.eps, fc1.weight, fc1.bias, act=self.ffn.act)
-            return hip_ops.linear(h, fc2.weight, fc2.bias, residual=x)
+                and hip_ops.linear_ln_supported(x, n2.weight, fc1.weight, fold=self.ffn.act in (None, "gelu"),
+                                                norm_bias=n2.bias)):
+            h = hip_ops.linear_ln(x, n2.weight, n2.bias, n2.eps, fc1.weight, fc1.bias, act=self.ffn.act, fold=True)
+            return hip_ops.linear(h, fc2.weight, fc2.bias, residual=x, ln_stats=True)
         h = hip_ops.layer_norm(x, n2.weight, n2.bias, n2.eps)
         return self.ffn(h, identity=x)
 
diff --git a/co-detr-tensorrt_amd/csrc/gemm_pp.hip b/co-detr-tensorrt_amd/csrc/gemm_pp.hip
--- a/co-detr-tensorrt_amd/csrc/gemm_pp.hip
+++ b/co-detr-tensorrt_amd/csrc/gemm_pp.hip
@@ -5,6 +5,7 @@
 
 #include "codetr_hip.h"
 #include "device_prims.h"
+#include "ln_fold.h"
 
 namespace {
 
@@ -32,6 +33,7 @@
 constexpr int kSlot = 32768;
 constexpr int kOpBytes = 16384;
 constexpr int kBiasBytes = 32768;
+constexpr int kLnBytes = 8192;
 
 struct PpArgs {
   const unsigned char* X;
@@ -44,6 +46,12 @@
   int G;
   int rounds;
   int rem;
+  const float* ln_rec;
+  const float* ln_s;
+  const float* ln_c;
+  int ln_parts;
+  float ln_eps;
+  float* rec_out;
 };
 
 __device__ __forceinline__ int key64(int row) {
@@ -67,9 +75,9 @@
   return (w & 7) * (D >> 3) + idx * (a.G >> 3) + (w >> 3);
 }
 
-template <class T, int ACT, bool HAS_BIAS, bool HAS_RES, bool BIAS_LDS = true>
+template <class T, int ACT, bool HAS_BIAS, bool HAS_RES, bool LN = false, bool STATS = false, bool BIAS_LDS = true>
 __device__ __forceinline__ bool pp_epilogue(f32x4 (&acc)[4][8], const PpArgs& a, int tile, int grp, int wn, int lane,
-                                            const unsigned char* bias_lds) {
+                                            unsigned char* bias_lds) {
   const int fa = lane & 15;
   const int tm = tile / a.tiles_n, tn = tile - tm * a.tiles_n;
   const int m0 = tm * 256 + grp * 128, n0 = tn * 256 + wn * 64;
@@ -105,6 +113,28 @@
       bias4[2] = T::to_f32((unsigned short)(b2.y & 0xffffu));
       bias4[3] = T::to_f32((unsigned short)(b2.y >> 16));
     }
+    float s4[4] = {0.f, 0.f, 0.f, 0.f};
+    float2* lnst = reinterpret_cast<float2*>(bias_lds) + (grp * 4 + wn) * 128;
+    if (LN) {
+      const int nb = n0 + nl < a.N ? n0 + nl : 0;
+      const f32x4 sv = *reinterpret_cast<const f32x4*>(a.ln_s + nb), cv = *reinterpret_cast<const f32x4*>(a.ln_c + nb);
+#pragma unroll
+      for (int i = 0; i < 4; ++i) {
+        s4[i] = sv[i];
+        bias4[i] = cv[i];
+      }
+      const float cnt = (float)(a.K / a.ln_parts);
+#pragma unroll 1
+      for (int h = 0; h < 2; ++h) {
+        int row = m0 + lane + 64 * h;
+        row = row < a.M ? row : a.M - 1;
+        lnst[lane + 64 * h] =
+            ln_row_stats(reinterpret_cast<const float2*>(a.ln_rec) + (size_t)row * a.ln_parts, a.ln_parts, cnt, a.ln_eps);
+      }
+      asm volatile("s_waitcnt lgkmcnt(0)" ::: "memory");
+      __builtin_amdgcn_wave_barrier();
+    }
+    float rmean[2] = {0.f, 0.f}, rm2[2] = {0.f, 0.f};
     const __amdgpu_buffer_rsrc_t ry = __builtin_amdgcn_make_buffer_rsrc(
         reinterpret_cast<unsigned char*>(a.Y) + ((size_t)m0 * a.N + n0) * 2, 0, span, 0x00020000);
     if (HAS_RES) load_res(0, 4);
@@ -116,6 +146,11 @@
         float x[4];
 #pragma unroll
         for (int i = 0; i < 4; ++i) x[i] = acc[i][j][r] + bias4[i];
+        if (LN) {
+          const float2 mr = lnst[j * 16 + 4 * g + r];
+#pragma unroll
+          for (int i = 0; i < 4; ++i) x[i] = fmaf(mr.y, fmaf(-mr.x, s4[i], acc[i][j][r]), bias4[i]);
+        }
         if (ACT == 1) {
 #pragma unroll
           for (int i = 0; i < 4; ++i) x[i] = x[i] < 0.f ? 0.f : x[i];
@@ -133,18 +168,42 @@
           const float y3 = T::to_f32((unsigned short)(o.y >> 16)) + T::to_f32((unsigned short)(q.y >> 16));
           o = uint2{T::pack2(y0, y1), T::pack2(y2, y3)};
         }
+        if (STATS) {
+          const float v0 = T::to_f32((unsigned short)(o.x & 0xffffu)), v1 = T::to_f32((unsigned short)(o.x >> 16));
+          const float v2 = T::to_f32((unsigned short)(o.y & 0xffffu)), v3 = T::to_f32((unsigned short)(o.y >> 16));
+          const float mean = row16_sum((v0 + v1) + (v2 + v3)) * (1.0f / 64.0f);
+          const float d0 = v0 - mean, d1 = v1 - mean, d2 = v2 - mean, d3 = v3 - mean;
+          const float m2 = row16_sum(fmaf(d0, d0, d1 * d1) + fmaf(d2, d2, d3 * d3));
+          const bool mine = ((4 * j + r) & 15) == fa;
+          rmean[j >> 2] = mine ? mean : rmean[j >> 2];
+          rm2[j >> 2] = mine ? m2 : rm2[j >> 2];
+        }
         if (!(kAbl & 16))
           __builtin_amdgcn_raw_buffer_store_b64(u32x2v{o.x, o.y}, ry, j * 16 + r < mrem ? voff : 0x80000000u,
                                                 (unsigned)(j * 16 + r) * rowb, 0);
       }
     }
+    if (STATS) {
+      const unsigned parts = (unsigned)a.N >> 6;
+      const __amdgpu_buffer_rsrc_t rrec = __builtin_amdgcn_make_buffer_rsrc(
+          reinterpret_cast<unsigned char*>(a.rec_out) + ((size_t)m0 * parts + (unsigned)(n0 >> 6)) * 8, 0,
+          (unsigned)(mleft < 128 ? mleft : 128) * parts * 8u, 0x00020000);
+#pragma unroll
+      for (int h = 0; h < 2; ++h) {
+        const int rl = (h * 4 + (fa >> 2)) * 16 + 4 * g + (fa & 3);
+        __builtin_amdgcn_raw_buffer_store_b64(u32x2v{__float_as_uint(rmean[h]), __float_as_uint(rm2[h])}, rrec,
+                                              rl < mleft ? (unsigned)rl * parts * 8u : 0x80000000u, 0, 0);
+      }
+    }
   }
   return stored;
 }
 
-template <class T, int ACT, bool HAS_BIAS, bool HAS_RES, int NS, int PH>
+template <class T, int ACT, bool HAS_BIAS, bool HAS_RES, int NS, int PH, bool LN = false, bool STATS = false>
 __global__ __launch_bounds__(512) __attribute__((amdgpu_waves_per_eu(2, 2))) void linear_pp_kernel(const PpArgs a) {
-  __shared__ __attribute__((aligned(16))) unsigned char lds[NS * kSlot + (HAS_BIAS ? kBiasBytes : 0)];
+  static_assert(!(LN && HAS_BIAS), "the folded LayerNorm's c vector carries the bias");
+  __shared__ __attribute__((aligned(16))) unsigned char lds[NS * kSlot + (HAS_BIAS ? kBiasBytes : LN ? kLnBytes : 0)];
+  constexpr int kEpiStores = 32 + (STATS ? 2 : 0);
   using frag = typename T::frag;
   constexpr int PP = 4;
   constexpr int VMN = PP * (NS - 2);
@@ -251,7 +310,7 @@
     PP_T(1);
     if (part == PH - 1) {
       if (post > 0) {
-        wait_vmcnt<VMN + 32>();
+        wait_vmcnt<VMN + kEpiStores>();
         --post;
       } else {
         wait_vmcnt<VMN>();
@@ -302,7 +361,7 @@
     if (grp == 0) seg_barrier();
 
     PP_T(8);
-    const bool stored = pp_epilogue<T, ACT, HAS_BIAS, HAS_RES>(acc, a, c_tile, grp, wn, lane, lds + NS * kSlot);
+    const bool stored = pp_epilogue<T, ACT, HAS_BIAS, HAS_RES, LN, STATS>(acc, a, c_tile, grp, wn, lane, lds + NS * kSlot);
     PP_T(9);
     PP_ACC(6, 8, 9);
     post = stored && !(kAbl & 16) ? NS - 2 : 0;
@@ -342,9 +401,25 @@
   return err == hipSuccess ? 0 : (int)err;
 }
 
+struct PpLn {
+  const float* rec = nullptr;
+  const float* s = nullptr;
+  const float* c = nullptr;
+  int parts = 0;
+  float eps = 0.f;
+  float* rec_out = nullptr;
+};
+
+template <class T, int ACT, bool HB, bool HR, bool LN, bool STATS>
+int launch_pp_one(hipStream_t st, const PpArgs& a) {
+  hipLaunchKernelGGL((linear_pp_kernel<T, ACT, HB, HR, 4, 1, LN, STATS>), dim3((unsigned)a.G), dim3(512), 0, st, a);
+  const hipError_t err = hipGetLastError();
+  return err == hipSuccess ? 0 : (int)err;
+}
+
 template <class T>
 int launch_pp(hipStream_t st, const void* X, const void* W, const void* bias, const void* R, void* Y, int64_t M, int64_t N,
-              int64_t K, int act, int flags) {
+              int64_t K, int act, int flags, const PpLn& ln = PpLn{}) {
   if (!X || !W || !Y || M <= 0 || N <= 0 || K <= 0) return CODETR_E_BADARG;
   if (act < 0 || act > 2 || !pp_supported(M, N, K)) return CODETR_E_UNSUPPORTED;
   if ((reinterpret_cast<uintptr_t>(X) | reinterpret_cast<uintptr_t>(W) | reinterpret_cast<uintptr_t>(Y) |
@@ -368,6 +443,20 @@
   const bool hb = bias != nullptr, hr = R != nullptr;
   if ((int64_t)256 * K * 2 > 0x7fffffffLL) return CODETR_E_TOO_LARGE;
   if (flags != 0) return CODETR_E_UNSUPPORTED;
+  a.ln_rec = ln.rec; a.ln_s = ln.s; a.ln_c = ln.c; a.ln_parts = ln.parts; a.ln_eps = ln.eps; a.rec_out = ln.rec_out;
+  if (ln.rec) {
+    if (!ln.s || !ln.c || hb || hr || ln.rec_out) return CODETR_E_BADARG;
+    if (ln.parts <= 0 || K % ln.parts != 0 || N % 4 != 0 || act == 1) return CODETR_E_UNSUPPORTED;
+    if ((reinterpret_cast<uintptr_t>(ln.rec) & 7) || ((reinterpret_cast<uintptr_t>(ln.s) | reinterpret_cast<uintptr_t>(ln.c)) & 15))
+      return CODETR_E_BADARG;
+    return act == 0 ? launch_pp_one<T, 0, false, false, true, false>(st, a) : launch_pp_one<T, 2, false, false, true, false>(st, a);
+  }
+  if (ln.rec_out) {
+    if (reinterpret_cast<uintptr_t>(ln.rec_out) & 7) return CODETR_E_BADARG;
+    if (N % 64 != 0 || act != 0 || hb != hr) return CODETR_E_UNSUPPORTED;
+    if (M * (N / 64) * 8 > 0x7fffffffLL) return CODETR_E_TOO_LARGE;
+    return hb ? launch_pp_one<T, 0, true, true, false, true>(st, a) : launch_pp_one<T, 0, false, false, false, true>(st, a);
+  }
   switch (act) {
     case 0: return launch_pp_act<T, 0>(st, a, hb, hr);
     case 1: return launch_pp_act<T, 1>(st, a, hb, hr);
@@ -402,4 +491,51 @@
   return launch_pp<BFloatT>(static_cast<hipStream_t>(stream), x_dev, w_dev, bias_dev, residual_dev, y_dev, M, N, K, act, flags);
 }
 
-}
+#if !CODETR_PP_ABL
+int codetr_linear_pp_lnfold_f16(void* stream, const void* x_dev, const void* rec_dev, int64_t parts, float eps,
+                                const void* ws_dev, const void* s_dev, const void* c_dev, void* y_dev, int64_t M, int64_t N,
+                                int64_t K, int act) {
+  if (!rec_dev || parts <= 0 || parts > K) return CODETR_E_BADARG;
+  PpLn ln;
+  ln.rec = static_cast<const float*>(rec_dev); ln.s = static_cast<const float*>(s_dev); ln.c = static_cast<const float*>(c_dev);
+  ln.parts = (int)parts; ln.eps = eps;
+  return launch_pp<HalfT>(static_cast<hipStream_t>(stream), x_dev, ws_dev, nullptr, nullptr, y_dev, M, N, K, act, 0, ln);
+}
+
+int codetr_linear_pp_lnfold_bf16(void* stream, const void* x_dev, const void* rec_dev, int64_t parts, float eps,
+                                 const void* ws_dev, const void* s_dev, const void* c_dev, void* y_dev, int64_t M, int64_t N,
+                                 int64_t K, int act) {
+  if (!rec_dev || parts <= 0 || parts > K) return CODETR_E_BADARG;
+  PpLn ln;
+  ln.rec = static_cast<const float*>(rec_dev); ln.s = static_cast<const float*>(s_dev); ln.c = static_cast<const float*>(c_dev);
+  ln.parts = (int)parts; ln.eps = eps;
+  return launch_pp<BFloatT>(static_cast<hipStream_t>(stream), x_dev, ws_dev, nullptr, nullptr, y_dev, M, N, K, act, 0, ln);
+}
+
+int codetr_linear_pp_stats_f16(void* stream, const void* x_dev, const void* w_dev, const void* bias_dev,
+                               const void* residual_dev, void* y_dev, void* rec_out_dev, int64_t M, int64_t N, int64_t K) {
+  if (!rec_out_dev) return CODETR_E_BADARG;
+  PpLn ln;
+  ln.rec_out = static_cast<float*>(rec_out_dev);
+  return launch_pp<HalfT>(static_cast<hipStream_t>(stream), x_dev, w_dev, bias_dev, residual_dev, y_dev, M, N, K, 0, 0, ln);
+}
+
+int codetr_linear_pp_stats_bf16(void* stream, const void* x_dev, const void* w_dev, const void* bias_dev,
+                                const void* residual_dev, void* y_dev, void* rec_out_dev, int64_t M, int64_t N, int64_t K) {
+  if (!rec_out_dev) return CODETR_E_BADARG;
+  PpLn ln;
+  ln.rec_out = static_cast<float*>(rec_out_dev);
+  return launch_pp<BFloatT>(static_cast<hipStream_t>(stream), x_dev, w_dev, bias_dev, residual_dev, y_dev, M, N, K, 0, 0, ln);
+}
+#else
+int codetr_linear_pp_lnfold_f16(void*, const void*, const void*, int64_t, float, const void*, const void*, const void*, void*,
+                                int64_t, int64_t, int64_t, int) { return CODETR_E_UNSUPPORTED; }
+int codetr_linear_pp_lnfold_bf16(void*, const void*, const void*, int64_t, float, const void*, const void*, const void*, void*,
+                                 int64_t, int64_t, int64_t, int) { return CODETR_E_UNSUPPORTED; }
+int codetr_linear_pp_stats_f16(void*, const void*, const void*, const void*, const void*, void*, void*, int64_t, int64_t,
+                               int64_t) { return CODETR_E_UNSUPPORTED; }
+int codetr_linear_pp_stats_bf16(void*, const void*, const void*, const void*, const void*, void*, void*, int64_t, int64_t,
+                                int64_t) { return CODETR_E_UNSUPPORTED; }
+#endif
+
+}
diff --git a/co-detr-tensorrt_amd/csrc/layernorm.hip b/co-detr-tensorrt_amd/csrc/layernorm.hip
--- a/co-detr-tensorrt_amd/csrc/layernorm.hip
+++ b/co-detr-tensorrt_amd/csrc/layernorm.hip
@@ -113,6 +113,63 @@
       }
     }
   }
+}
+
+template <class T, int G, int NCH>
+__global__ __launch_bounds__(kThreads) void row_stats_kernel(const short* __restrict__ x, float2* __restrict__ rec,
+                                                             int64_t rows, int C) {
+  constexpr int ROWS_PER_BLOCK = kThreads / G;
+  const int sub = threadIdx.x % G, rloc = threadIdx.x / G, nchunks = C >> 3;
+  for (int64_t row = (int64_t)blockIdx.x * ROWS_PER_BLOCK + rloc; row < rows; row += (int64_t)gridDim.x * ROWS_PER_BLOCK) {
+    s16x8 v[NCH];
+    float s = 0.f;
+#pragma unroll
+    for (int c = 0; c < NCH; ++c) {
+      const int ch = sub + c * G;
+      if (ch < nchunks) {
+        v[c] = *reinterpret_cast<const s16x8*>(x + row * C + ch * 8);
+#pragma unroll
+        for (int e = 0; e < 8; ++e) s += T::up(v[c][e]);
+      }
+    }
+    const float mean = group_sum<G>(s) / (float)C;
+    float q = 0.f;
+#pragma unroll
+    for (int c = 0; c < NCH; ++c) {
+      if (sub + c * G < nchunks) {
+#pragma unroll
+        for (int e = 0; e < 8; ++e) {
+          const float d = T::up(v[c][e]) - mean;
+          q = fmaf(d, d, q);
+        }
+      }
+    }
+    q = group_sum<G>(q);
+    if (sub == 0) rec[row] = float2{mean, q};
+  }
+}
+
+template <class T, int G, int NCH>
+int launch_stats_cfg(hipStream_t st, const void* x, void* rec, int64_t rows, int C) {
+  constexpr int RPB = kThreads / G;
+  int64_t blocks = (rows + RPB - 1) / RPB;
+  if (blocks > 256 * 16) blocks = 256 * 16;
+  hipLaunchKernelGGL((row_stats_kernel<T, G, NCH>), dim3((unsigned)blocks), dim3(kThreads), 0, st,
+                     static_cast<const short*>(x), static_cast<float2*>(rec), rows, C);
+  const hipError_t err = hipGetLastError();
+  return err == hipSuccess ? 0 : (int)err;
+}
+
+template <class T>
+int launch_stats(hipStream_t st, const void* x, void* rec, int64_t rows, int64_t C) {
+  if (!x || !rec || rows <= 0 || C <= 0) return CODETR_E_BADARG;
+  if (C % 8 != 0 || C > 2048) return CODETR_E_UNSUPPORTED;
+  const int nch = (int)(C / 8);
+  if (nch <= 32) return launch_stats_cfg<T, 32, 1>(st, x, rec, rows, (int)C);
+  if (nch <= 64) return launch_stats_cfg<T, 64, 1>(st, x, rec, rows, (int)C);
+  if (nch <= 128) return launch_stats_cfg<T, 64, 2>(st, x, rec, rows, (int)C);
+  if (nch <= 192) return launch_stats_cfg<T, 64, 3>(st, x, rec, rows, (int)C);
+  return launch_stats_cfg<T, 64, 4>(st, x, rec, rows, (int)C);
 }
 
 template <class T, int G, int NCH, bool MERGE = false>
@@ -175,6 +232,14 @@
   return launch<LnBf16>(static_cast<hipStream_t>(stream), x_dev, gamma_dev, beta_dev, y_dev, rows, C, eps);
 }
 
+int codetr_row_stats_f16(void* stream, const void* x_dev, void* rec_dev, int64_t rows, int64_t C) {
+  return launch_stats<LnHalf>(static_cast<hipStream_t>(stream), x_dev, rec_dev, rows, C);
+}
+
+int codetr_row_stats_bf16(void* stream, const void* x_dev, void* rec_dev, int64_t rows, int64_t C) {
+  return launch_stats<LnBf16>(static_cast<hipStream_t>(stream), x_dev, rec_dev, rows, C);
+}
+
 int codetr_patch_merge_layernorm_f16(void* stream, const void* x_dev, const void* gamma_dev, const void* beta_dev,
                                      void* y_dev, int64_t B, int64_t H, int64_t W, int64_t C, float eps) {
   return launch_merge<LnHalf>(static_cast<hipStream_t>(stream), x_dev, gamma_dev, beta_dev, y_dev, B, H, W, C, eps);
diff --git a/co-detr-tensorrt_amd/csrc/ln_fold.h b/co-detr-tensorrt_amd/csrc/ln_fold.h
--- /dev/null
+++ b/co-detr-tensorrt_amd/csrc/ln_fold.h
@@ -0,0 +1,41 @@
+#pragma once
+#include "device_prims.h"
+
+namespace {
+
+__device__ __forceinline__ float row16_sum(float v) {
+  v += dpp_f<kXor1>(v);
+  v += dpp_f<kXor2>(v);
+  v += dpp_f<0x141>(v);
+  v += dpp_f<0x140>(v);
+  return v;
+}
+
+__device__ __forceinline__ float2 ln_row_stats(const float2* rec, int parts, float cnt, float eps) {
+  float n = 0.f, mean = 0.f, m2 = 0.f;
+  for (int p0 = 0; p0 < parts; p0 += 12) {
+    const int np = parts - p0 < 12 ? parts - p0 : 12;
+    float2 t[12];
+#pragma unroll
+    for (int u = 0; u < 12; ++u) t[u] = rec[p0 + (u < np ? u : np - 1)];
+    float sm = 0.f;
+#pragma unroll
+    for (int u = 0; u < 12; ++u) sm += u < np ? t[u].x : 0.f;
+    const float mc = sm / (float)np;
+    float q = 0.f, d2 = 0.f;
+#pragma unroll
+    for (int u = 0; u < 12; ++u) {
+      const float d = t[u].x - mc;
+      q += u < np ? t[u].y : 0.f;
+      d2 = u < np ? fmaf(d, d, d2) : d2;
+    }
+    const float nc = cnt * (float)np, m2c = fmaf(cnt, d2, q);
+    const float tot = n + nc, delta = mc - mean;
+    mean = fmaf(delta, nc / tot, mean);
+    m2 += m2c + delta * delta * (n * nc / tot);
+    n = tot;
+  }
+  return float2{mean, 1.0f / sqrtf(m2 / n + eps)};
+}
+
+}
diff --git a/include/codetr_hip.h b/include/codetr_hip.h
--- a/include/codetr_hip.h
+++ b/include/codetr_hip.h
@@ -12,7 +12,7 @@
 #define CODETR_E_TOO_LARGE (-3)
 #define CODETR_E_UNSUPPORTED (-4)
 
-#define CODETR_HIP_ABI_VERSION 53
+#define CODETR_HIP_ABI_VERSION 54
 int codetr_hip_abi_version(void);
 const char *codetr_hip_strerror(int code);
 
@@ -224,6 +224,19 @@
 int codetr_linear_pp_bf16(void *stream, const void *x_dev, const void *w_dev, const void *bias_dev,
                           const void *residual_dev, void *y_dev, int64_t M, int64_t N, int64_t K, int act, int flags);
 
+int codetr_linear_pp_stats_f16(void *stream, const void *x_dev, const void *w_dev, const void *bias_dev,
+                               const void *residual_dev, void *y_dev, void *rec_out_dev, int64_t M, int64_t N, int64_t K);
+int codetr_linear_pp_stats_bf16(void *stream, const void *x_dev, const void *w_dev, const void *bias_dev,
+                                const void *residual_dev, void *y_dev, void *rec_out_dev, int64_t M, int64_t N, int64_t K);
+int codetr_row_stats_f16(void *stream, const void *x_dev, void *rec_dev, int64_t rows, int64_t C);
+int codetr_row_stats_bf16(void *stream, const void *x_dev, void *rec_dev, int64_t rows, int64_t C);
+int codetr_linear_pp_lnfold_f16(void *stream, const void *x_dev, const void *rec_dev, int64_t parts, float eps,
+                                const void *ws_dev, const void *s_dev, const void *c_dev, void *y_dev, int64_t M,
+                                int64_t N, int64_t K, int act);
+int codetr_linear_pp_lnfold_bf16(void *stream, const void *x_dev, const void *rec_dev, int64_t parts, float eps,
+                                 const void *ws_dev, const void *s_dev, const void *c_dev, void *y_dev, int64_t M,
+                                 int64_t N, int64_t K, int act);
+
 int codetr_mask_pyramid(void *stream, const void *img_mask_dev, int64_t B, int64_t H_img, int64_t W_img,
                         int num_levels, const int64_t *level_shapes_host, void *mask_flat_dev, float *ycum_dev,
                         float *xcum_dev, float *valid_counts_dev, int mask_elem_bytes);
diff --git a/runner/dispatch_gen.inc b/runner/dispatch_gen.inc
--- a/runner/dispatch_gen.inc
+++ b/runner/dispatch_gen.inc
@@ -1,4 +1,4 @@
-static const int kPlanAbi = 53;
+static const int kPlanAbi = 54;
 static int call_codetr_msda_forward_f16(void* fn, const Arg* a) { typedef int (*F)(const void*, const void*, const void*, const void*, const void*, const void*, long long, long long, int, int, int, long long, int, long long, const void*); return ((F)fn)((const void*)a[0].p, (const void*)a[1].p, (const void*)a[2].p, (const void*)a[3].p, (const void*)a[4].p, (const void*)a[5].p, (long long)a[6].i, (long long)a[7].i, (int)a[8].i, (int)a[9].i, (int)a[10].i, (long long)a[11].i, (int)a[12].i, (long long)a[13].i, (const void*)a[14].p); }
 static int call_codetr_msda_forward_bf16(void* fn, const Arg* a) { typedef int (*F)(const void*, const void*, const void*, const void*, const void*, const void*, long long, long long, int, int, int, long long, int, long long, const void*); return ((F)fn)((const void*)a[0].p, (const void*)a[1].p, (const void*)a[2].p, (const void*)a[3].p, (const void*)a[4].p, (const void*)a[5].p, (long long)a[6].i, (long long)a[7].i, (int)a[8].i, (int)a[9].i, (int)a[10].i, (long long)a[11].i, (int)a[12].i, (long long)a[13].i, (const void*)a[14].p); }
 static int call_codetr_msda_forward_f32(void* fn, const Arg* a) { typedef int (*F)(const void*, const void*, const void*, const void*, const void*, const void*, long long, long long, int, int, int, long long, int, long long, const void*); return ((F)fn)((const void*)a[0].p, (const void*)a[1].p, (const void*)a[2].p, (const void*)a[3].p, (const void*)a[4].p, (const void*)a[5].p, (long long)a[6].i, (long long)a[7].i, (int)a[8].i, (int)a[9].i, (int)a[10].i, (long long)a[11].i, (int)a[12].i, (long long)a[13].i, (const void*)a[14].p); }
@@ -78,6 +78,12 @@
 static int call_codetr_swin_mlp_bf16(void* fn, const Arg* a) { typedef int (*F)(const void*, const void*, const void*, const void*, float, const void*, const void*, const void*, const void*, const void*, long long, long long); return ((F)fn)((const void*)a[0].p, (const void*)a[1].p, (const void*)a[2].p, (const void*)a[3].p, (float)a[4].f, (const void*)a[5].p, (const void*)a[6].p, (const void*)a[7].p, (const void*)a[8].p, (const void*)a[9].p, (long long)a[10].i, (long long)a[11].i); }
 static int call_codetr_linear_pp_f16(void* fn, const Arg* a) { typedef int (*F)(const void*, const void*, const void*, const void*, const void*, const void*, long long, long long, long long, int, int); return ((F)fn)((const void*)a[0].p, (const void*)a[1].p, (const void*)a[2].p, (const void*)a[3].p, (const void*)a[4].p, (const void*)a[5].p, (long long)a[6].i, (long long)a[7].i, (long long)a[8].i, (int)a[9].i, (int)a[10].i); }
 static int call_codetr_linear_pp_bf16(void* fn, const Arg* a) { typedef int (*F)(const void*, const void*, const void*, const void*, const void*, const void*, long long, long long, long long, int, int); return ((F)fn)((const void*)a[0].p, (const void*)a[1].p, (const void*)a[2].p, (const void*)a[3].p, (const void*)a[4].p, (const void*)a[5].p, (long long)a[6].i, (long long)a[7].i, (long long)a[8].i, (int)a[9].i, (int)a[10].i); }
+static int call_codetr_linear_pp_stats_f16(void* fn, const Arg* a) { typedef int (*F)(const void*, const void*, const void*, const void*, const void*, const void*, const void*, long long, long long, long long); return ((F)fn)((const void*)a[0].p, (const void*)a[1].p, (const void*)a[2].p, (const void*)a[3].p, (const void*)a[4].p, (const void*)a[5].p, (const void*)a[6].p, (long long)a[7].i, (long long)a[8].i, (long long)a[9].i); }
+static int call_codetr_linear_pp_stats_bf16(void* fn, const Arg* a) { typedef int (*F)(const void*, const void*, const void*, const void*, const void*, const void*, const void*, long long, long long, long long); return ((F)fn)((const void*)a[0].p, (const void*)a[1].p, (const void*)a[2].p, (const void*)a[3].p, (const void*)a[4].p, (const void*)a[5].p, (const void*)a[6].p, (long long)a[7].i, (long long)a[8].i, (long long)a[9].i); }
+static int call_codetr_row_stats_f16(void* fn, const Arg* a) { typedef int (*F)(const void*, const void*, const void*, long long, long long); return ((F)fn)((const void*)a[0].p, (const void*)a[1].p, (const void*)a[2].p, (long long)a[3].i, (long long)a[4].i); }
+static int call_codetr_row_stats_bf16(void* fn, const Arg* a) { typedef int (*F)(const void*, const void*, const void*, long long, long long); return ((F)fn)((const void*)a[0].p, (const void*)a[1].p, (const void*)a[2].p, (long long)a[3].i, (long long)a[4].i); }
+static int call_codetr_linear_pp_lnfold_f16(void* fn, const Arg* a) { typedef int (*F)(const void*, const void*, const void*, long long, float, const void*, const void*, const void*, const void*, long long, long long, long long, int); return ((F)fn)((const void*)a[0].p, (const void*)a[1].p, (const void*)a[2].p, (long long)a[3].i, (float)a[4].f, (const void*)a[5].p, (const void*)a[6].p, (const void*)a[7].p, (const void*)a[8].p, (long long)a[9].i, (long long)a[10].i, (long long)a[11].i, (int)a[12].i); }
+static int call_codetr_linear_pp_lnfold_bf16(void* fn, const Arg* a) { typedef int (*F)(const void*, const void*, const void*, long long, float, const void*, const void*, const void*, const void*, long long, long long, long long, int); return ((F)fn)((const void*)a[0].p, (const void*)a[1].p, (const void*)a[2].p, (long long)a[3].i, (float)a[4].f, (const void*)a[5].p, (const void*)a[6].p, (const void*)a[7].p, (const void*)a[8].p, (long long)a[9].i, (long long)a[10].i, (long long)a[11].i, (int)a[12].i); }
 static int call_codetr_linear_sk_bf16(void* fn, const Arg* a) { typedef int (*F)(const void*, const void*, const void*, const void*, const void*, const void*, long long, long long, long long, int, const void*, long long, int); return ((F)fn)((const void*)a[0].p, (const void*)a[1].p, (const void*)a[2].p, (const void*)a[3].p, (const void*)a[4].p, (const void*)a[5].p, (long long)a[6].i, (long long)a[7].i, (long long)a[8].i, (int)a[9].i, (const void*)a[10].p, (long long)a[11].i, (int)a[12].i); }
 static int call_codetr_decoder_layer_f16(void* fn, const Arg* a) { typedef int (*F)(const void*, const void*, const void*, const void*, const void*, const void*, const void*, const void*, const void*, const void*, const void*, const void*, const void*, const void*, const void*, const void*, const void*, const void*, long long, long long, long long, int, int, int, float, float); return ((F)fn)((const void*)a[0].p, (const void*)a[1].p, (const void*)a[2].p, (const void*)a[3].p, (const void*)a[4].p, (const void*)a[5].p, (const void*)a[6].p, (const void*)a[7].p, (const void*)a[8].p, (const void*)a[9].p, (const void*)a[10].p, (const void*)a[11].p, (const void*)a[12].p, (const void*)a[13].p, (const void*)a[14].p, (const void*)a[15].p, (const void*)a[16].p, (const void*)a[17].p, (long long)a[18].i, (long long)a[19].i, (long long)a[20].i, (int)a[21].i, (int)a[22].i, (int)a[23].i, (float)a[24].f, (float)a[25].f); }
 static int call_codetr_decoder_layer_bf16(void* fn, const Arg* a) { typedef int (*F)(const void*, const void*, const void*, const void*, const void*, const void*, const void*, const void*, const void*, const void*, const void*, const void*, const void*, const void*, const void*, const void*, const void*, const void*, long long, long long, long long, int, int, int, float, float); return ((F)fn)((const void*)a[0].p, (const void*)a[1].p, (const void*)a[2].p, (const void*)a[3].p, (const void*)a[4].p, (const void*)a[5].p, (const void*)a[6].p, (const void*)a[7].p, (const void*)a[8].p, (const void*)a[9].p, (const void*)a[10].p, (const void*)a[11].p, (const void*)a[12].p, (const void*)a[13].p, (const void*)a[14].p, (const void*)a[15].p, (const void*)a[16].p, (const void*)a[17].p, (long long)a[18].i, (long long)a[19].i, (long long)a[20].i, (int)a[21].i, (int)a[22].i, (int)a[23].i, (float)a[24].f, (float)a[25].f); }
@@ -179,6 +185,12 @@
   {"codetr_swin_mlp_bf16", 12, call_codetr_swin_mlp_bf16},
   {"codetr_linear_pp_f16", 11, call_codetr_linear_pp_f16},
   {"codetr_linear_pp_bf16", 11, call_codetr_linear_pp_bf16},
+  {"codetr_linear_pp_stats_f16", 10, call_codetr_linear_pp_stats_f16},
+  {"codetr_linear_pp_stats_bf16", 10, call_codetr_linear_pp_stats_bf16},
+  {"codetr_row_stats_f16", 5, call_codetr_row_stats_f16},
+  {"codetr_row_stats_bf16", 5, call_codetr_row_stats_bf16},
+  {"codetr_linear_pp_lnfold_f16", 13, call_codetr_linear_pp_lnfold_f16},
+  {"codetr_linear_pp_lnfold_bf16", 13, call_codetr_linear_pp_lnfold_bf16},
   {"codetr_linear_sk_bf16", 13, call_codetr_linear_sk_bf16},
   {"codetr_decoder_layer_f16", 26, call_codetr_decoder_layer_f16},
   {"codetr_decoder_layer_bf16", 26, call_codetr_decoder_layer_bf16},
```

Result: no change. 99.52, median of 3 (-0.1%).
